# steineggerlab/folddisco

Hardware: AMD Instinct MI355X
Metric: structures/sec indexed (higher is better)
Workload: dtype f32+u32; 1 GPU; Swiss-Prot scale: 542000 synthetic AFDB-shaped structures (175035960 residues, 17705019118 postings, 26085150307 value bytes) index build, PDBTrRosetta default; 1 rank(s), contiguous id ranges, per rank 1 build call(s) of <= 542000 structures: one resident index, no merge; structures=542000, structures_per_gpu=542000, residues=175035960, postings=17705019118, parallelism=shard-by-structure x1, build_calls_per_rank=1

## Files before the change

### folddisco_amd/_lib.py

```python
from __future__ import annotations

import ctypes as C
import os

HERE = os.path.dirname(os.path.abspath(__file__))
LIB_PATH = os.path.join(HERE, "libfdgpu.so")

u8p = C.POINTER(C.c_uint8)
u32p = C.POINTER(C.c_uint32)
u64p = C.POINTER(C.c_uint64)
f32p = C.POINTER(C.c_float)
VP = C.c_void_p


class BatchDesc(C.Structure):
    _fields_ = [("n_struct", C.c_uint64), ("res_off", u64p), ("n_xyz", f32p), ("ca_xyz", f32p), ("cb_xyz", f32p),
                ("aa", u8p), ("cb_valid", u8p)]


class HashParams(C.Structure):
    _fields_ = [("nbin_dist", C.c_uint32), ("nbin_angle", C.c_uint32), ("dist_cutoff", C.c_float), ("hash_type", C.c_uint32),
                ("n_multiple_bins", C.c_uint32), ("multiple_bins", (C.c_uint32 * 2) * 8)]

    def __init__(self, nbin_dist=0, nbin_angle=0, dist_cutoff=20.0, hash_type=3, multiple_bins=None):
        super().__init__(int(nbin_dist), int(nbin_angle), float(dist_cutoff), int(hash_type))
        mb = list(multiple_bins or [])
        if len(mb) > 8:
            raise ValueError("at most 8 (dist, angle) bin pairs")
        self.n_multiple_bins = len(mb)
        for k, (d, a) in enumerate(mb):
            self.multiple_bins[k][0] = int(d)
            self.multiple_bins[k][1] = int(a)


def parse_multiple_bins(s):
    out = []
    for item in (s or "").split(","):
        parts = item.strip().split("-")
        if len(parts) == 2:
            try:
                out.append((int(parts[0]), int(parts[1])))
            except ValueError:
                pass
    return out


HASH_TYPE_NAMES = {0: "PDBMotif", 1: "PDBMotifSinCos", 2: "TrRosetta", 3: "PDBTrRosetta", 4: "PointPairFeature", 5: "TertiaryInteraction",
                   6: "Hybrid", 7: "FolddiscoAngle", 8: "FolddiscoDist"}
_HASH_TYPE_ALIASES = {"pyscomotif": 0, "orig_pdb": 0, "pdb": 1, "trrosetta": 2, "tr": 2, "pdbtr": 3, "default": 3, "folddisco": 3, "ppf": 4,
                      "tertiary": 5, "3di": 5, "hybrid": 6, "angle": 7, "folddisco_angle": 7, "distance": 8, "dist": 8, "folddisco_dist": 8}


def hash_type_index(name) -> int:
    if isinstance(name, int):
        return name
    s = str(name)
    if s.isdigit() and int(s) in HASH_TYPE_NAMES:
        return int(s)
    for k, v in HASH_TYPE_NAMES.items():
        if v == s:
            return k
    if s in _HASH_TYPE_ALIASES:
        return _HASH_TYPE_ALIASES[s]
    raise ValueError(f"unknown hash type {name!r}")


class CountRec(C.Structure):
    _fields_ = [("nid", C.c_uint32), ("total_match_count", C.c_uint32), ("node_count", C.c_uint32),
                ("edge_count", C.c_uint32), ("idf", C.c_float)]


class PairRec(C.Structure):
    _fields_ = [("cand", C.c_uint32), ("i", C.c_uint32), ("j", C.c_uint32), ("hash", C.c_uint32)]


class CandRec(C.Structure):
    _fields_ = [("cand", C.c_uint32), ("qi", C.c_uint32), ("i", C.c_uint32), ("j", C.c_uint32)]


class MatchQuery(C.Structure):
    _fields_ = [("hashes", u32p), ("n_hashes", C.c_uint64), ("aad_aa1", u8p), ("aad_aa2", u8p), ("aad_dist", f32p),
                ("aad_qi", u32p), ("n_aad", C.c_uint64), ("ca_distance_cutoff", C.c_float), ("use_aa_prefilter", C.c_int)]


class QueryMap(C.Structure):
    _fields_ = [("n", C.c_uint64), ("hash", u32p), ("qi", u32p), ("qj", u32p), ("is_primary", u8p), ("idf", f32p),
                ("n_indices", C.c_uint64), ("indices", u32p),
                ("n_aad", C.c_uint64), ("aad_aa1", u8p), ("aad_aa2", u8p), ("aad_dist", f32p), ("aad_qi", u32p), ("primary_hash", u32p),
                ("post_len", u64p), ("post_seg", u32p), ("post_index_uid", C.c_uint64), ("post_kidx", C.POINTER(C.c_longlong)),
                ("arena_bytes", C.c_uint64)]


class MatchRec(C.Structure):
    _fields_ = [("cand", C.c_uint32), ("same", C.c_uint32), ("idf", C.c_float), ("rmsd", C.c_float), ("rmsd_from_hash", C.c_float),
                ("rot", C.c_float * 9), ("tran", C.c_float * 3), ("metrics", C.c_float * 5),
                ("rot_from_hash", C.c_float * 9), ("tran_from_hash", C.c_float * 3), ("metrics_from_hash", C.c_float * 5)]


class FoldcompAtom(C.Structure):
    _fields_ = [("x", C.c_float), ("y", C.c_float), ("z", C.c_float), ("b", C.c_float), ("name", C.c_char * 4), ("res", C.c_char * 3),
                ("chain", C.c_uint8), ("rser", C.c_uint64)]


class VerifyReportC(C.Structure):
    _fields_ = [("ok", C.c_uint32), ("first_mask", C.c_uint32), ("n_bad", C.c_uint64), ("class_count", C.c_uint64 * 9), ("first_slot", C.c_uint64),
                ("first_offset", C.c_uint64), ("first_hash", C.c_uint32), ("list_stage", C.c_uint32), ("n_lists", C.c_uint64), ("n_postings", C.c_uint64),
                ("max_id", C.c_uint64), ("max_list_bytes", C.c_uint64)]


class Parsed(C.Structure):
    _fields_ = [("n_struct", C.c_uint64), ("n_res", C.c_uint64), ("res_off", u64p), ("n_xyz", f32p), ("ca_xyz", f32p), ("cb_xyz", f32p),
                ("aa", u8p), ("cb_valid", u8p), ("chain", u8p), ("resname_std", u8p), ("serial", u64p), ("bfac", f32p),
                ("resname", C.POINTER(C.c_char)), ("nres_raw", u64p), ("plddt", f32p), ("ok", u8p), ("first_chain", u8p)]


SYMBOLS = [
    ("fdgpu_create", C.c_int, [C.c_int, C.POINTER(VP)]),
    ("fdgpu_destroy", None, [VP]),
    ("fdgpu_set_stream", C.c_int, [VP, VP]),
    ("fdgpu_synchronize", C.c_int, [VP]),
    ("fdgpu_release_workspaces", C.c_int, [VP]),
    ("fdgpu_last_error", C.c_char_p, [VP]),
    ("fdgpu_free", None, [VP]),
    ("fdgpu_version", C.c_char_p, []),
    ("fdgpu_batch_upload", C.c_int, [VP, C.POINTER(BatchDesc), C.POINTER(VP)]),
    ("fdgpu_batch_wrap_device", C.c_int, [VP, C.POINTER(BatchDesc), C.c_uint64, C.POINTER(VP)]),
    ("fdgpu_batch_destroy", None, [VP]),
    ("fdgpu_batch_num_structures", C.c_uint64, [VP]),
    ("fdgpu_batch_num_residues", C.c_uint64, [VP]),
    ("fdgpu_batch_select", C.c_int, [VP, VP, u32p, C.c_uint64, C.POINTER(VP)]),
    ("fdgpu_batch_concat", C.c_int, [VP, C.POINTER(VP), C.c_uint64, C.POINTER(VP)]),
    ("fdgpu_batch_export", C.c_int, [VP, VP, C.POINTER(BatchDesc)]),
    ("fdgpu_hash_batch", C.c_int, [VP, VP, C.POINTER(HashParams), C.c_int, C.POINTER(u32p), C.POINTER(u64p)]),
    ("fdgpu_index_build", C.c_int, [VP, VP, C.POINTER(HashParams), C.c_uint64, C.POINTER(VP)]),
    ("fdgpu_index_export", C.c_int, [VP, VP, C.POINTER(u8p), u64p, C.POINTER(u32p), C.POINTER(u64p), u64p]),
    ("fdgpu_index_load", C.c_int, [VP, u32p, u64p, C.c_uint64, u8p, C.c_uint64, C.c_uint64, C.POINTER(VP)]),
    ("fdgpu_index_destroy", None, [VP]),
    ("fdgpu_index_num_hashes", C.c_uint64, [VP]),
    ("fdgpu_index_value_len", C.c_uint64, [VP]),
    ("fdgpu_index_num_postings", C.c_uint64, [VP]),
    ("fdgpu_index_num_structures", C.c_uint64, [VP]),
    ("fdgpu_index_save", C.c_int, [VP, VP, C.c_char_p]),
    ("fdgpu_posting_lengths", C.c_int, [VP, VP, u32p, C.c_uint64, u64p]),
    ("fdgpu_count_query", C.c_int, [VP, VP, u32p, u32p, u32p, f32p, C.c_uint64, f32p, C.POINTER(C.POINTER(CountRec)), u64p]),
    ("fdgpu_count_query_batch", C.c_int, [VP, VP, C.c_uint64, u64p, u32p, u32p, u32p, f32p, f32p, C.POINTER(C.POINTER(CountRec)), C.POINTER(u64p)]),
    ("fdgpu_spec_fallbacks", C.c_int, [VP, u64p]),
    ("fdgpu_parse_structures", C.c_int, [C.POINTER(C.c_char_p), C.c_uint64, C.c_uint32, C.c_uint64, C.POINTER(C.POINTER(Parsed))]),
    ("fdgpu_parsed_free", None, [C.POINTER(Parsed)]),
    ("fdgpu_foldcomp_decode", C.c_int, [C.c_char_p, C.c_uint64, C.POINTER(C.POINTER(FoldcompAtom)), u64p]),
    ("fdgpu_foldcomp_db_list", C.c_int, [C.c_char_p, C.POINTER(u64p), C.POINTER(C.c_void_p), u64p]),
    ("fdgpu_parse_foldcomp_db", C.c_int, [C.c_char_p, u64p, C.c_uint64, C.c_uint32, C.c_uint64, C.POINTER(C.POINTER(Parsed))]),
    ("fdgpu_get_entries", C.c_int, [VP, VP, u32p, C.c_uint64, C.POINTER(u32p), C.POINTER(u64p)]),
    ("fdgpu_count_query_batch_top", C.c_int, [VP, VP, C.c_uint64, u64p, u32p, u32p, u32p, f32p, f32p, C.c_uint32, C.POINTER(C.POINTER(CountRec)), C.POINTER(u64p)]),
    ("fdgpu_index_set_penalty", C.c_int, [VP, VP, f32p]),
    ("fdgpu_count_query_maps_top", C.c_int, [VP, VP, C.c_uint64, C.c_void_p, f32p, C.c_float, C.c_uint32, C.POINTER(C.POINTER(CountRec)), C.POINTER(u64p)]),
    ("fdgpu_match_pairs", C.c_int, [VP, VP, u8p, u32p, C.c_uint64, C.POINTER(MatchQuery), C.POINTER(HashParams),
                                    C.POINTER(C.POINTER(PairRec)), u64p, C.POINTER(C.POINTER(CandRec)), u64p]),
    ("fdgpu_kabsch_batch", C.c_int, [VP, f32p, f32p, u64p, C.c_uint64, f32p, f32p, f32p]),
    ("fdgpu_lms_qcp_batch", C.c_int, [VP, f32p, f32p, u64p, C.c_uint64, f32p, f32p, f32p, u32p, u32p]),
    ("fdgpu_last_timings", C.c_int, [VP, C.POINTER(C.c_char_p), f32p, u64p, C.c_int]),
    ("fdgpu_enable_timing", C.c_int, [VP, C.c_int]),
    ("fdgpu_pair_features", C.c_int, [VP, VP, C.c_uint64, u32p, u32p, C.c_uint64, C.POINTER(HashParams), f32p, u8p]),
    ("fdgpu_hash_features", C.c_int, [VP, f32p, C.c_uint64, C.POINTER(HashParams), u32p]),
    ("fdgpu_make_query_map_batch", C.c_int, [VP, VP, C.c_uint64, u32p, u64p, u32p, C.POINTER(u8p), u32p, f32p, C.c_uint64, f32p, C.c_uint64,
                                              C.POINTER(HashParams), VP, C.c_float, C.POINTER(C.POINTER(QueryMap))]),
    ("fdgpu_make_query_map", C.c_int, [VP, VP, u32p, C.c_uint64, C.POINTER(u8p), u32p, f32p, C.c_uint64, f32p, C.c_uint64,
                                       C.POINTER(HashParams), VP, C.c_float, C.POINTER(C.POINTER(QueryMap))]),
    ("fdgpu_query_map_free", None, [C.POINTER(QueryMap)]),
    ("fdgpu_retrieve_batch", C.c_int, [VP, VP, u8p, C.c_uint64, u32p, u64p, C.POINTER(C.POINTER(QueryMap)), VP, u32p, C.POINTER(HashParams),
                                        C.c_float, C.c_uint32, C.c_uint32, C.POINTER(C.POINTER(MatchRec)), C.POINTER(u64p), C.POINTER(C.POINTER(C.c_int32)),
                                        C.POINTER(u64p)]),
    ("fdgpu_query_batch", C.c_int, [VP, VP, VP, u8p, VP, C.c_uint64, u32p, u64p, u32p, C.POINTER(u8p), u32p, f32p, C.c_uint64, f32p, C.c_uint64,
                                    C.POINTER(HashParams), C.c_float, f32p, C.c_uint32, C.c_uint32, C.c_float, C.c_uint32, C.POINTER(C.POINTER(QueryMap)),
                                    C.POINTER(C.POINTER(CountRec)), C.POINTER(u64p), C.POINTER(C.POINTER(MatchRec)), C.POINTER(u64p),
                                    C.POINTER(C.POINTER(C.c_int32)), C.POINTER(u64p)]),
    ("fdgpu_query_batch_submit", C.c_int, [VP, VP, VP, u8p, VP, C.c_uint64, u32p, u64p, u32p, C.POINTER(u8p), u32p, f32p, C.c_uint64, f32p, C.c_uint64,
                                           C.POINTER(HashParams), C.c_float, f32p, C.c_uint32, C.c_uint32, C.c_float, C.c_uint32, C.POINTER(VP)]),
    ("fdgpu_query_batch_wait", C.c_int, [VP, VP, C.POINTER(C.POINTER(QueryMap)), C.POINTER(C.POINTER(CountRec)), C.POINTER(u64p), C.POINTER(C.POINTER(MatchRec)),
                                         C.POINTER(u64p), C.POINTER(C.POINTER(C.c_int32)), C.POINTER(u64p)]),
    ("fdgpu_query_lanes", C.c_int, [VP, C.c_uint32]),
    ("fdgpu_trim", None, []),
    ("fdgpu_reserve_staging", C.c_int, [VP]),
    ("fdgpu_write_lookup", C.c_int, [C.c_char_p, C.c_char_p, C.c_uint64, u64p, f32p, u64p]),
    ("fdgpu_format_f32_display", C.c_int, [f32p, C.c_uint64, C.c_char_p]),
    ("fdgpu_retrieve", C.c_int, [VP, VP, u8p, u32p, C.c_uint64, C.POINTER(QueryMap), VP, C.POINTER(HashParams), C.c_float, C.c_uint32, C.c_uint32,
                                 C.POINTER(C.POINTER(MatchRec)), u64p, C.POINTER(C.POINTER(C.c_int32))]),
    ("fdgpu_matches_free", None, [C.POINTER(MatchRec), C.POINTER(C.c_int32)]),
    ("fdgpu_merge_subindices", C.c_int, [C.c_uint64, C.POINTER(u8p), C.POINTER(u32p), C.POINTER(u64p), u64p, C.POINTER(u8p), u64p,
                                         C.POINTER(u32p), C.POINTER(u64p), u64p]),
    ("fdgpu_index_merge", C.c_int, [VP, C.POINTER(VP), C.c_uint64, C.POINTER(VP)]),
    ("fdgpu_index_remove", C.c_int, [VP, VP, u8p, C.c_uint64, C.POINTER(VP)]),
    ("fdgpu_index_split", C.c_int, [VP, VP, C.c_uint32, u64p, C.POINTER(VP)]),
    ("fdgpu_split_host", C.c_int, [u32p, u64p, C.c_uint64, u8p, C.c_uint64, C.c_uint64, C.c_uint32, u64p, C.c_uint32, C.POINTER(u8p), u64p,
                                   C.POINTER(u32p), C.POINTER(u64p), u64p]),
    ("fdgpu_index_rebase", C.c_int, [VP, VP, C.c_uint64, C.POINTER(VP)]),
    ("fdgpu_rebase_host", C.c_int, [u32p, u64p, C.c_uint64, u8p, C.c_uint64, C.c_uint64, C.c_uint64, C.c_uint64, C.c_uint32, C.POINTER(u8p), u64p,
                                    C.POINTER(u32p), C.POINTER(u64p)]),
    ("fdgpu_index_permute", C.c_int, [VP, VP, u32p, C.c_uint64, C.POINTER(VP)]),
    ("fdgpu_permute_host", C.c_int, [u32p, u64p, C.c_uint64, u8p, C.c_uint64, C.c_uint64, u32p, C.c_uint64, C.c_uint32, C.POINTER(u8p), u64p,
                                     C.POINTER(u32p), C.POINTER(u64p)]),
    ("fdgpu_index_rows", C.c_int, [VP, VP, C.c_uint64, C.c_uint64, C.POINTER(u32p), C.POINTER(u64p)]),
    ("fdgpu_rows_host", C.c_int, [u32p, u64p, C.c_uint64, u8p, C.c_uint64, C.c_uint64, C.c_uint64, C.c_uint64, C.c_uint64, C.c_uint32, C.POINTER(u32p),
                                  C.POINTER(u64p)]),
    ("fdgpu_index_signatures", C.c_int, [VP, VP, C.c_uint64, C.c_uint64, C.c_uint64, C.POINTER(VP)]),
    ("fdgpu_signatures_host", C.c_int, [u32p, u64p, C.c_uint64, u8p, C.c_uint64, C.c_uint64, C.c_uint64, C.c_uint64, C.c_uint64, C.c_uint32, C.POINTER(VP)]),
    ("fdgpu_signature_pairs", C.c_int, [VP, VP, C.c_uint64, VP, C.c_uint64, C.c_uint32, C.c_uint64, C.POINTER(VP), u64p]),
    ("fdgpu_signature_pairs_host", C.c_int, [VP, C.c_uint64, VP, C.c_uint64, C.c_uint32, C.c_uint64, C.c_uint32, C.POINTER(VP), u64p]),
    ("fdgpu_signature_neighbors", C.c_int, [VP, VP, C.c_uint64, VP, C.c_uint64, VP, C.c_uint32, C.c_uint32, C.POINTER(VP)]),
    ("fdgpu_signature_neighbors_host", C.c_int, [VP, C.c_uint64, VP, C.c_uint64, VP, C.c_uint32, C.c_uint32, C.c_uint32, C.POINTER(VP)]),
    ("fdgpu_signature_clusters", C.c_int, [VP, VP, C.c_uint64, VP, C.c_uint32, C.POINTER(VP)]),
    ("fdgpu_signature_clusters_host", C.c_int, [VP, C.c_uint64, VP, C.c_uint32, C.c_uint32, C.POINTER(VP)]),
    ("fdgpu_index_rowset", C.c_int, [VP, VP, u32p, C.c_uint64, C.c_uint64, C.c_uint64, C.POINTER(VP), u64p]),
    ("fdgpu_rowset_info", C.c_int, [VP, u64p, u64p]),
    ("fdgpu_rowset_lengths", C.c_int, [VP, C.POINTER(u32p)]),
    ("fdgpu_rowset_export", C.c_int, [VP, VP, C.POINTER(u32p), C.POINTER(u64p)]),
    ("fdgpu_rowset_intersect", C.c_int, [VP, VP, VP, u32p, u32p, C.c_uint64, C.POINTER(u32p)]),
    ("fdgpu_rowset_destroy", None, [VP]),
    ("fdgpu_rows_intersect_host", C.c_int, [u32p, u64p, C.c_uint64, u32p, u64p, C.c_uint64, u32p, u32p, C.c_uint64, C.c_uint32, C.POINTER(u32p)]),
    ("fdgpu_index_verify", C.c_int, [VP, VP, C.POINTER(VerifyReportC)]),
    ("fdgpu_verify_host", C.c_int, [u32p, u64p, C.c_uint64, u8p, C.c_uint64, C.c_uint64, C.c_uint64, C.c_uint32, C.POINTER(VerifyReportC)]),
    ("fdgpu_posting_bytes", C.c_int, [VP, VP, u32p, C.c_uint64, u64p]),
    ("fdgpu_index_set_first_id", C.c_int, [VP, C.c_uint64]),
    ("fdgpu_host_libm_matches", C.c_int, [VP]),
    ("fdgpu_metrics_batch", C.c_int, [VP, f32p, f32p, u64p, C.c_uint64, f32p, f32p, f32p]),
    ("fdgpu_hash_batch_rows", C.c_int, [VP, VP, C.POINTER(HashParams), C.POINTER(u32p), C.POINTER(u32p), C.POINTER(u64p)]),
    ("fdgpu_hypergeom_enrichment", C.c_int, [u64p, u64p, C.c_uint64, C.c_uint64, C.c_uint64, C.c_uint32, C.POINTER(C.c_double)]),
    ("fdgpu_comm_unique_id", C.c_int, [u8p]),
    ("fdgpu_comm_init", C.c_int, [VP, u8p, C.c_int, C.c_int, C.POINTER(VP)]),
    ("fdgpu_comm_destroy", None, [VP]),
    ("fdgpu_comm_rank", C.c_int, [VP]),
    ("fdgpu_comm_world", C.c_int, [VP]),
    ("fdgpu_allreduce_lengths", C.c_int, [VP, VP, u64p, C.c_uint64]),
    ("fdgpu_sharded_count_query", C.c_int, [VP, VP, VP, C.c_uint64, u64p, u32p, u32p, u32p, f32p, C.c_uint64, C.c_uint32,
                                            C.POINTER(C.POINTER(CountRec)), C.POINTER(u64p)]),
    ("fdgpu_comm_stats", C.c_int, [VP, u64p, u64p]),
    ("fdgpu_index_range_bounds", C.c_int, [VP, VP, C.c_uint32, u32p]),
    ("fdgpu_index_slice", C.c_int, [VP, VP, C.c_uint64, C.c_uint64, C.POINTER(VP)]),
    ("fdgpu_comm_single_index", C.c_int, [VP, VP, VP, C.POINTER(VP), u64p, u64p, u64p, u64p]),
    ("fdgpu_index_save_part", C.c_int, [VP, VP, C.c_char_p, C.c_uint64, C.c_uint64, C.c_uint64, C.c_uint64, C.c_int, C.c_int]),
    ("fdgpu_sharded_count_query_maps", C.c_int, [VP, VP, VP, C.c_uint64, C.c_void_p, f32p, C.c_uint64, C.c_uint32,
                                                 C.POINTER(C.POINTER(CountRec)), C.POINTER(u64p)]),
    ("fdgpu_sharded_retrieve", C.c_int, [VP, VP, VP, C.c_uint64, u8p, C.c_uint64, u32p, u64p, C.POINTER(C.POINTER(QueryMap)), VP, u32p,
                                         C.POINTER(HashParams), C.c_float, C.c_uint32, C.c_uint32, C.POINTER(C.POINTER(MatchRec)), C.POINTER(u64p),
                                         C.POINTER(C.POINTER(C.c_int32)), C.POINTER(u64p)]),
    ("fdgpu_query_maps_lengths", C.c_int, [VP, VP, C.c_uint64, C.c_void_p, u64p]),
    ("fdgpu_count_query_maps_top_global", C.c_int, [VP, VP, C.c_uint64, C.c_void_p, u64p, f32p, C.c_float, C.c_uint32,
                                                    C.POINTER(C.POINTER(CountRec)), C.POINTER(u64p)]),
    ("fdgpu_comm_message_bytes", C.c_uint64, [C.c_uint64, C.c_uint32]),
    ("fdgpu_debug_merge_gathered", C.c_int, [VP, C.c_uint32, C.c_uint64, C.c_uint32, u8p, C.POINTER(C.POINTER(CountRec)), C.POINTER(u64p)]),
    ("fdgpu_debug_libm", C.c_int, [VP, C.c_int, f32p, f32p, f32p, C.c_uint64]),
    ("fdgpu_debug_last_count_path", C.c_int, [VP, u32p]),
    ("fdgpu_debug_last_retrieve_path", C.c_int, [VP, u32p]),
    ("fdgpu_debug_last_query_map_path", C.c_int, [VP, u32p]),
    ("fdgpu_debug_qm_pairs", C.c_int, [C.c_uint64, u32p, u64p, u32p, u64p, C.POINTER(u32p), C.POINTER(u32p), u64p]),
    ("fdgpu_debug_qm_fields", C.c_int, [C.c_uint32, C.POINTER(C.c_int32)]),
    ("fdgpu_debug_qm_expand", C.c_int, [f32p, u8p, u32p, u32p, C.c_uint64, C.c_uint64, u32p, C.c_uint64, C.POINTER(u8p), u32p, C.c_uint32, f32p, C.c_uint64, f32p,
                                        C.c_uint64, C.POINTER(f32p), C.POINTER(u32p), u64p]),
    ("fdgpu_debug_qm_first_insertions", C.c_int, [u32p, C.c_uint64, C.c_uint32, C.c_uint64, C.c_uint64, C.POINTER(u32p), u64p]),
    ("fdgpu_debug_qm_arena", C.c_int, [C.c_uint64, C.c_uint64, C.c_uint64, C.c_uint32, u64p]),
    ("fdgpu_debug_qm_fill", C.c_int, [u32p, C.c_uint64, u32p, C.c_uint64, C.c_uint32, C.c_uint64, u32p, u32p, C.c_uint64, u32p, u32p, C.c_uint64, f32p, u32p, u64p, u32p,
                                      C.POINTER(C.c_longlong), C.c_uint64, u32p, C.c_uint64, u8p, u8p, f32p, u32p, C.c_uint64, C.c_uint32, C.POINTER(C.POINTER(QueryMap))]),
    ("fdgpu_debug_encode_stream", C.c_int, [VP, u32p, u32p, C.c_uint64, C.POINTER(VP)]),
    ("fdgpu_debug_encode_stream_b24", C.c_int, [VP, u32p, u32p, C.c_uint64, C.c_uint64, C.POINTER(VP)]),
    ("fdgpu_ingest_stats", None, [C.POINTER(C.c_double), C.c_int]),
    ("fdgpu_debug_gunzip", C.c_int, [u8p, C.c_uint64, C.POINTER(u8p), u64p]),
    ("fdgpu_debug_host_components", C.c_int, [u32p, u32p, C.c_uint64, C.c_uint32, C.POINTER(u32p), C.POINTER(u64p), u64p]),
    ("fdgpu_debug_hash_is_symmetric", C.c_int, [C.c_uint32, u32p, C.c_uint64, u8p]),
    ("fdgpu_debug_host_retrieve_slot", C.c_int, [u32p, u32p, u32p, C.c_uint64, u32p, u32p, u32p, C.c_uint64, C.c_uint32, C.POINTER(QueryMap), C.c_uint32, C.c_uint32,
                                                 C.c_uint32, C.c_uint32, u64p, C.POINTER(f32p), C.POINTER(u32p), C.POINTER(C.POINTER(C.c_int32))]),
    ("fdgpu_debug_match_tables", C.c_int, [C.c_uint64, C.POINTER(MatchQuery), u32p, u64p, u64p, C.c_uint64, C.c_uint32, C.c_uint32, C.c_uint32, C.POINTER(u32p), u64p, u64p,
                                           C.POINTER(C.c_char_p)]),
    ("fdgpu_debug_merge_retrieved", C.c_int, [VP, C.c_uint32, C.c_uint64, u64p, C.POINTER(C.POINTER(MatchRec)), C.POINTER(C.POINTER(C.c_int32)), u64p,
                                              C.POINTER(C.POINTER(MatchRec)), C.POINTER(u64p), C.POINTER(C.POINTER(C.c_int32)), C.POINTER(u64p)]),
]

_lib = None


def load() -> C.CDLL:
    global _lib
    if _lib is not None:
        return _lib
    if not os.path.exists(LIB_PATH):
        raise ImportError(
            f"{LIB_PATH} is missing: build it with `python -m folddisco_amd.build` (hipcc, gfx950). "
            "folddisco_amd has no CPU fallback.")
    try:
        import torch
    except Exception:
        pass
    L = C.CDLL(LIB_PATH)
    for name, res, args in SYMBOLS:
        fn = getattr(L, name)
        fn.restype = res
        fn.argtypes = args
    _lib = L
    return L


def owned_view(lib, ptr, nbytes, dtype):
    import weakref
    import numpy as _np
    addr = C.cast(ptr, C.c_void_p).value
    if not nbytes or not addr:
        if addr:
            lib.fdgpu_free(C.c_void_p(addr))
        return _np.zeros(0, _np.uint8).view(dtype)
    buf = (C.c_uint8 * nbytes).from_address(addr)
    weakref.finalize(buf, lib.fdgpu_free, C.c_void_p(addr))
    return _np.frombuffer(buf, dtype=_np.uint8).view(dtype)
```

### folddisco_amd/csrc/fd_api_build.hip

```cpp
#include <stdlib.h>
#include <algorithm>
#include <memory>
#include "fd_api_common.h"

struct ib_free { void operator()(void *p) const { free(p); } };
typedef std::unique_ptr<uint32_t, ib_free> ib_u32_ptr;
typedef std::unique_ptr<uint64_t, ib_free> ib_u64_ptr;

static int row_count_and_scan(fdgpu_ctx *c, const fdgpu_batch *b, const fd_hash_consts &C, float dist_cutoff, uint64_t *P, const char *stage = nullptr) {
    const uint64_t R = b->n_res;
    hipStream_t st = c->stream;
    HIPCHK(c, c->ws[WS_MISC0].ensure((R + 1) * 4));
    HIPCHK(c, c->ws[WS_MISC1].ensure((R + 2) * 8));
    HIPCHK(c, c->ws[WS_SCANTMP].ensure(fd_scan_tmp_elems(std::max<uint64_t>(b->n_struct, R)) * 8 + 64));
    HIPCHK(c, c->ws[WS_TOTAL].ensure(64));
    HIPCHK(c, hipMemsetAsync(c->ws[WS_MISC0].p, 0, (R + 1) * 4, st));
    {
        StageTimer t(stage ? c : nullptr, stage, R * 37);
        fd_launch_row_count(b->view(), C, c->ws[WS_MISC0].as<uint32_t>(), dist_cutoff, st);
        fd_exclusive_scan<uint32_t>(c->ws[WS_MISC0].as<uint32_t>(), R, c->ws[WS_MISC1].as<uint64_t>(), c->ws[WS_SCANTMP].as<uint64_t>(),
                                    c->ws[WS_TOTAL].as<uint64_t>(), st);
    }
    HIPCHK(c, hipGetLastError());
    return d2h_u64(c, c->ws[WS_TOTAL].as<uint64_t>(), P);
}

static int scan_counts(fdgpu_ctx *c, uint64_t n, uint64_t *P) {
    {
        StageTimer t(c, "segment_scan", n * 12);
        fd_exclusive_scan<uint32_t>(c->ws[WS_COUNTS].as<uint32_t>(), n, c->ws[WS_SEGOFF].as<uint64_t>(), c->ws[WS_SCANTMP].as<uint64_t>(),
                                    c->ws[WS_TOTAL].as<uint64_t>(), c->stream);
    }
    HIPCHK(c, hipGetLastError());
    return d2h_u64(c, c->ws[WS_TOTAL].as<uint64_t>(), P);
}
static int count_and_scan(fdgpu_ctx *c, const fdgpu_batch *b, const fd_hash_consts &C, uint64_t *P, bool unordered = false) {
    uint64_t S = b->n_struct;
    HIPCHK(c, c->ws[WS_COUNTS].ensure((S + 1) * 4));
    HIPCHK(c, c->ws[WS_CURSOR].ensure((S + 1) * 4));
    HIPCHK(c, c->ws[WS_SEGOFF].ensure((S + 2) * 8));
    HIPCHK(c, c->ws[WS_SCANTMP].ensure(fd_scan_tmp_elems(std::max<uint64_t>(S, b->n_res)) * 8 + 64));
    HIPCHK(c, c->ws[WS_TOTAL].ensure(64));
    HIPCHK(c, hipMemsetAsync(c->ws[WS_COUNTS].p, 0, (S + 1) * 4, c->stream));
    HIPCHK(c, hipMemsetAsync(c->ws[WS_CURSOR].p, 0, (S + 1) * 4, c->stream));
    {
        StageTimer t(c, "pair_count", b->n_res * 13);
        if (unordered) fd_launch_pair_count2(b->view(), C, c->ws[WS_COUNTS].as<uint32_t>(), c->stream);
        else fd_launch_pair_count(b->view(), C, c->ws[WS_COUNTS].as<uint32_t>(), c->stream);
    }
    return scan_counts(c, S, P);
}

struct ib_keys { uint32_t *ka, *kb; void *ia, *ib; };
static int reserve_keys(fdgpu_ctx *c, uint64_t P, uint64_t max_keys, const char *too_many, size_t id_bytes, ib_keys &K) {
    if (P >= max_keys) FAIL(c, FDGPU_ERANGE, too_many);
    size_t kb = std::max<uint64_t>(P, 1) * 4, ib = std::max<uint64_t>(P, 1) * id_bytes + 16;
    if (kb > c->ws[WS_KEYS_A].cap + ((size_t)1 << 30) || kb > c->ws[WS_KEYS_B].cap + ((size_t)1 << 30)) c->pool_drop();
    HIPCHK(c, c->ws[WS_KEYS_A].ensure(kb));
    HIPCHK(c, c->ws[WS_IDS_A].ensure(ib));
    HIPCHK(c, c->ws[WS_KEYS_B].ensure(kb));
    HIPCHK(c, c->ws[WS_IDS_B].ensure(ib));
    HIPCHK(c, c->ws[WS_GHIST].ensure((size_t)256 * std::max<uint32_t>(fd_rs_num_tiles(P), 1) * 4));
    HIPCHK(c, c->ws[WS_TOT].ensure((256 + (size_t)(fd_rs_num_tiles(P) / 128 + 2) * 256) * 8));
    K.ka = c->ws[WS_KEYS_A].as<uint32_t>(); K.kb = c->ws[WS_KEYS_B].as<uint32_t>();
    K.ia = c->ws[WS_IDS_A].p; K.ib = c->ws[WS_IDS_B].p;
    return FDGPU_OK;
}

extern "C" int fdgpu_hash_batch(fdgpu_ctx *c, const fdgpu_batch *b, const fd_hash_params *p, int sort_dedup, uint32_t **hashes,
                                uint64_t **hash_off) { FD_LOCK(c);
    if (!c || !b || !p || !hashes || !hash_off) return FDGPU_EINVAL;
    *hashes = nullptr; *hash_off = nullptr;
    if (p->n_multiple_bins) FAIL(c, FDGPU_EINVAL, "hash_batch: multiple_bins is honoured by the index build and the query calls only");
    if (!fd_hash_type_supported(p->hash_type)) FAIL(c, FDGPU_EINVAL, "hash_type: only the encodings over the (d_CA, d_CB, theta, tau1, tau2) descriptor are built (0, 1, 3, 7, 8)");
    reset_timings(c);
    fd_hash_consts C = make_consts(p);
    uint64_t S = b->n_struct, R = b->n_res;
    ib_u64_ptr h_off((uint64_t *)malloc((S + 1) * 8));
    if (!h_off) return FDGPU_ENOMEM;
    hipStream_t st = c->stream;
    int rc;
    if (!sort_dedup) {
        uint64_t P = 0;
        if ((rc = row_count_and_scan(c, b, C, p->dist_cutoff, &P))) return rc;
        HIPCHK(c, c->ws[WS_KEYS_A].ensure(std::max<uint64_t>(P, 1) * 4));
        fd_launch_row_emit(b->view(), C, c->ws[WS_MISC1].as<uint64_t>(), c->ws[WS_KEYS_A].as<uint32_t>(), p->dist_cutoff, nullptr, 0u, st);
        HIPCHK(c, hipGetLastError());
        ib_u32_ptr h((uint32_t *)malloc(std::max<uint64_t>(P, 1) * 4));
        std::vector<uint64_t> row_off(R + 1);
        if (!h) return FDGPU_ENOMEM;
        HIPCHK(c, hipMemcpyAsync(h.get(), c->ws[WS_KEYS_A].p, P * 4, hipMemcpyDeviceToHost, st));
        HIPCHK(c, hipMemcpyAsync(row_off.data(), c->ws[WS_MISC1].p, (R + 1) * 8, hipMemcpyDeviceToHost, st));
        HIPCHK(c, hipStreamSynchronize(st));
        for (uint64_t s = 0; s <= S; ++s) h_off.get()[s] = row_off[b->h_res_off[s]];
        *hashes = h.release(); *hash_off = h_off.release();
        return FDGPU_OK;
    }
    if (fd_own_descriptor(p->hash_type)) FAIL(c, FDGPU_EINVAL, "hash_batch: this encoding is served in the reference's raw order only (sort_dedup = 0)");
    uint64_t P = 0;
    if ((rc = count_and_scan(c, b, C, &P))) return rc;
    ib_keys K;
    if ((rc = reserve_keys(c, P, 0xffffffffull, "more than 2^32 residue pairs in one batch; split the batch", 4, K))) return rc;
    uint32_t *ka = K.ka, *ia = (uint32_t *)K.ia, *kb = K.kb, *ib = (uint32_t *)K.ib;
    fd_launch_pair_emit(b->view(), C, c->ws[WS_SEGOFF].as<uint64_t>(), c->ws[WS_CURSOR].as<uint32_t>(), ka, ia, 0u, st);
    int cur = sort_pairs(c, ka, ia, kb, ib, P, 32);
    uint32_t *k1 = cur ? kb : ka, *i1 = cur ? ib : ia, *k2 = cur ? ka : kb, *i2 = cur ? ia : ib;
    int id_bits = 1;
    while (id_bits < 32 && (1ull << id_bits) < std::max<uint64_t>(S, 2)) ++id_bits;
    int cur2 = sort_pairs(c, i1, k1, i2, k2, P, id_bits);
    uint32_t *ids_s = cur2 ? i2 : i1, *keys_s = cur2 ? k2 : k1, *spare = cur2 ? k1 : k2;
    HIPCHK(c, c->ws[WS_MISC0].ensure(std::max<uint64_t>(P, 1)));
    HIPCHK(c, c->ws[WS_MISC1].ensure((P + 2) * 8));
    HIPCHK(c, c->ws[WS_SCANTMP].ensure(fd_scan_tmp_elems(std::max<uint64_t>(P, S)) * 8 + 64));
    fd_launch_uniq_flags(keys_s, ids_s, P, c->ws[WS_MISC0].as<uint8_t>(), st);
    fd_exclusive_scan<uint8_t>(c->ws[WS_MISC0].as<uint8_t>(), P, c->ws[WS_MISC1].as<uint64_t>(), c->ws[WS_SCANTMP].as<uint64_t>(),
                               c->ws[WS_TOTAL].as<uint64_t>(), st);
    fd_launch_compact(keys_s, c->ws[WS_MISC0].as<uint8_t>(), c->ws[WS_MISC1].as<uint64_t>(), P, spare, st);
    HIPCHK(c, c->ws[WS_MISC2].ensure((S + 2) * 8));
    fd_launch_gather_u64(c->ws[WS_MISC1].as<uint64_t>(), c->ws[WS_SEGOFF].as<uint64_t>(), S + 1, c->ws[WS_MISC2].as<uint64_t>(), st);
    HIPCHK(c, hipGetLastError());
    uint64_t U = 0;
    if ((rc = d2h_u64(c, c->ws[WS_TOTAL].as<uint64_t>(), &U))) return rc;
    ib_u32_ptr h((uint32_t *)malloc(std::max<uint64_t>(U, 1) * 4));
    if (!h) return FDGPU_ENOMEM;
    HIPCHK(c, hipMemcpyAsync(h.get(), spare, U * 4, hipMemcpyDeviceToHost, st));
    HIPCHK(c, hipMemcpyAsync(h_off.get(), c->ws[WS_MISC2].p, (S + 1) * 8, hipMemcpyDeviceToHost, st));
    HIPCHK(c, hipStreamSynchronize(st));
    *hashes = h.release(); *hash_off = h_off.release();
    return FDGPU_OK;
}

extern "C" int fdgpu_hash_batch_rows(fdgpu_ctx *c, const fdgpu_batch *b, const fd_hash_params *p, uint32_t **hashes, uint32_t **partner, uint64_t **row_off) { FD_LOCK(c);
    if (!c || !b || !p || !hashes || !partner || !row_off) return FDGPU_EINVAL;
    *hashes = nullptr; *partner = nullptr; *row_off = nullptr;
    if (p->n_multiple_bins) FAIL(c, FDGPU_EINVAL, "hash_batch_rows: multiple_bins is honoured by the index build and the query calls only");
    if (!fd_hash_type_supported(p->hash_type)) FAIL(c, FDGPU_EINVAL, "hash_type: unknown encoding");
    reset_timings(c);
    const fd_hash_consts C = make_consts(p);
    const uint64_t R = b->n_res;
    hipStream_t st = c->stream;
    uint64_t P = 0;
    int rc = row_count_and_scan(c, b, C, p->dist_cutoff, &P);
    if (rc) return rc;
    HIPCHK(c, c->ws[WS_KEYS_A].ensure(std::max<uint64_t>(P, 1) * 4));
    HIPCHK(c, c->ws[WS_IDS_A].ensure(std::max<uint64_t>(P, 1) * 4));
    fd_launch_row_emit(b->view(), C, c->ws[WS_MISC1].as<uint64_t>(), c->ws[WS_KEYS_A].as<uint32_t>(), p->dist_cutoff, c->ws[WS_IDS_A].as<uint32_t>(), 0u, st, 1);
    HIPCHK(c, hipGetLastError());
    ib_u32_ptr h((uint32_t *)malloc(std::max<uint64_t>(P, 1) * 4)), pj((uint32_t *)malloc(std::max<uint64_t>(P, 1) * 4));
    ib_u64_ptr ro((uint64_t *)malloc((R + 1) * 8));
    if (!h || !pj || !ro) return FDGPU_ENOMEM;
    hipError_t e = hipMemcpyAsync(h.get(), c->ws[WS_KEYS_A].p, P * 4, hipMemcpyDeviceToHost, st);
    if (e == hipSuccess) e = hipMemcpyAsync(pj.get(), c->ws[WS_IDS_A].p, P * 4, hipMemcpyDeviceToHost, st);
    if (e == hipSuccess) e = hipMemcpyAsync(ro.get(), c->ws[WS_MISC1].p, (R + 1) * 8, hipMemcpyDeviceToHost, st);
    if (e == hipSuccess) e = hipStreamSynchronize(st);
    if (e != hipSuccess) { c->err = std::string("hash_batch_rows: ") + hipGetErrorString(e); return FDGPU_EHIP; }
    *hashes = h.release(); *partner = pj.release(); *row_off = ro.release();
    return FDGPU_OK;
}

#define FDGPU_RETRY_WIDE 1000
enum {
    IB_W_TOTALS = 0, IB_W_VALUE_BYTES = 0, IB_W_HASHES = 1, IB_W_POSTINGS = 2,
    IB_W_WIDE = 3,
    IB_W_SORT_OVERFLOW = 4,
    IB_W_READ = 5,
    IB_W_BUCKET_STARTS = 8,
};
static uint64_t *ib_word(fdgpu_ctx *c, int w) { return c->ws[WS_MISC3].as<uint64_t>() + w; }
static int ib_clear_words(fdgpu_ctx *c) {
    HIPCHK(c, c->ws[WS_MISC3].ensure(512));
    HIPCHK(c, hipMemsetAsync(c->ws[WS_MISC3].p, 0, IB_W_BUCKET_STARTS * 8, c->stream));
    return FDGPU_OK;
}
static int encode_sorted_stream(fdgpu_ctx *c, const uint32_t *ks, const void *is, int codec, uint64_t first_id, uint64_t P, uint64_t S, uint64_t seg_stride, fdgpu_index **out) {
    hipStream_t st = c->stream;
    const bool el6 = codec != 0;
    const uint32_t nt = std::max<uint32_t>(fd_enc_num_tiles(P), 1);
    for (int s : {WS_TILE_B, WS_TILE_H, WS_TILE_P}) HIPCHK(c, c->ws[s].ensure((size_t)(nt + 1) * 4));
    for (int s : {WS_TILE_BO, WS_TILE_HO, WS_TILE_PO}) HIPCHK(c, c->ws[s].ensure((size_t)(nt + 2) * 8));
    HIPCHK(c, c->ws[WS_SCANTMP].ensure(fd_scan_tmp_elems(std::max<uint64_t>(nt, S)) * 8 + 64));
    uint32_t *tile_bytes = c->ws[WS_TILE_B].as<uint32_t>(), *tile_hashes = c->ws[WS_TILE_H].as<uint32_t>(), *tile_posts = c->ws[WS_TILE_P].as<uint32_t>();
    uint64_t *bytes_off = c->ws[WS_TILE_BO].as<uint64_t>(), *hashes_off = c->ws[WS_TILE_HO].as<uint64_t>(), *posts_off = c->ws[WS_TILE_PO].as<uint64_t>();
    uint64_t *scan_tmp = c->ws[WS_SCANTMP].as<uint64_t>();
    const uint64_t *seg = c->ws[WS_SEGOFF].as<uint64_t>();
    uint64_t tot[IB_W_READ] = {0, 0, 0, 0, 0};
    const uint64_t nt_eff = P ? fd_enc_num_tiles(P) : 0;
    {
        StageTimer t(c, "encode_sizes", P * (el6 ? 6 : 8));
        for (uint32_t *tile : {tile_bytes, tile_hashes, tile_posts}) HIPCHK(c, hipMemsetAsync(tile, 0, (size_t)(nt + 1) * 4, st));
        fd_launch_enc_sizes(ks, is, codec, (uint32_t)first_id, P, tile_bytes, tile_hashes, tile_posts, seg, seg_stride, ib_word(c, IB_W_BUCKET_STARTS), st);
        fd_exclusive_scan<uint32_t>(tile_bytes, nt_eff, bytes_off, scan_tmp, ib_word(c, IB_W_VALUE_BYTES), st);
        fd_exclusive_scan<uint32_t>(tile_hashes, nt_eff, hashes_off, scan_tmp, ib_word(c, IB_W_HASHES), st);
        fd_exclusive_scan<uint32_t>(tile_posts, nt_eff, posts_off, scan_tmp, ib_word(c, IB_W_POSTINGS), st);
    }
    HIPCHK(c, hipGetLastError());
    HIPCHK(c, hipMemcpyAsync(tot, ib_word(c, IB_W_TOTALS), sizeof tot, hipMemcpyDeviceToHost, st));
    HIPCHK(c, hipStreamSynchronize(st));
    if (tot[IB_W_SORT_OVERFLOW]) FAIL(c, FDGPU_ERANGE, "index build: one (residue-pair bucket, key digit) group holds 2^32 keys or more; build the shard in several calls and merge");
    if (el6 && tot[IB_W_WIDE]) return FDGPU_RETRY_WIDE;
    fdgpu_index *ix = nullptr;
    const int rc = fd_index_new(c, true, tot[IB_W_HASHES], tot[IB_W_VALUE_BYTES], true, &ix);
    if (rc) return rc;
    ix->n_postings = tot[IB_W_POSTINGS]; ix->n_structures = S; ix->first_id = first_id;
    {
        StageTimer t(c, "encode_write", P * (el6 ? 6 : 8) + ix->value_len + ix->n_hashes * 12);
        fd_launch_enc_write(ks, is, codec, (uint32_t)first_id, P, bytes_off, hashes_off, ix->value, ix->hashes, ix->offsets, ix->last_ids, ib_word(c, IB_W_TOTALS), ix->n_hashes,
                            ib_word(c, IB_W_BUCKET_STARTS), st);
    }
    const hipError_t e = hipGetLastError();
    if (e != hipSuccess) { c->err = std::string("encode launch: ") + hipGetErrorString(e); fdgpu_index_destroy(ix); return FDGPU_EHIP; }
    *out = ix;
    return FDGPU_OK;
}

enum ib_kind { IB_OWN, IB_STRUCTURE_MAJOR, IB_MSD };
static const uint32_t IB_BUCKETS = 40;
struct ib_form {
    ib_kind kind; bool el6; int codec;
    uint32_t n_cfg; uint64_t seg_stride;
    uint64_t max_keys; const char *too_many;
};
static int ib_choose_form(fdgpu_ctx *c, const fdgpu_batch *b, const fd_hash_params *p, uint64_t first_id, bool force32, ib_form &F) {
    if (!fd_hash_type_supported(p->hash_type)) FAIL(c, FDGPU_EINVAL, "hash_type: only the encodings over the (d_CA, d_CB, theta, tau1, tau2) descriptor are built (0, 1, 3, 7, 8)");
    reset_timings(c);
    const uint64_t S = b->n_struct;
    if (first_id + S > 0xffffffffull) FAIL(c, FDGPU_ERANGE, "structure ids exceed 32 bits");
    if (!fd_multiple_bins_valid(p)) FAIL(c, FDGPU_EINVAL, "multiple_bins: at most 8 (dist, angle) bin pairs, no zero counts");
    F.n_cfg = fd_num_bin_configs(p);
    const bool own = fd_own_descriptor(p->hash_type);
    if (own && F.n_cfg > 1) FAIL(c, FDGPU_EINVAL, "multiple_bins is built for the encodings over the PDBTrRosetta descriptor only");
    const bool ids16 = !own && !force32 && S <= (1ull << 18);
    const bool msd_env = [] { const char *e = getenv("FDGPU_MSD"); return !(e && e[0] == '0'); }();
    const bool msd = msd_env && !own && !force32 && S <= (1ull << 24) && F.n_cfg == 1 && p->hash_type == FDGPU_HASH_PDBTR && S > 0;
    F.kind = own ? IB_OWN : msd ? IB_MSD : IB_STRUCTURE_MAJOR;
    F.el6 = ids16 || msd;
    F.codec = msd ? 2 : ids16 ? 1 : 0;
    F.seg_stride = msd ? b->n_work : 0;
    F.max_keys = msd ? 1ull << 35 : 0xffffffffull;
    F.too_many = msd ? "more than 2^35 residue pairs in one build call; split the shard" : "more than 2^32 residue pairs in one build call; split the shard";
    return FDGPU_OK;
}
static void ib_frames(fdgpu_ctx *c, const fdgpu_batch *b) {
    StageTimer t(c, "frames", b->n_res * (37 + sizeof(fd_frame)));
    fd_launch_frames(b->view(), b->n_res, c->ws[WS_FRAMES].p, c->stream);
}
static int ib_count_msd(fdgpu_ctx *c, const fdgpu_batch *b, const fd_hash_consts &C, fd_batch_view &V, uint64_t *P1) {
    hipStream_t st = c->stream;
    const uint64_t R1 = std::max<uint64_t>(b->n_res, 1), NS = (uint64_t)IB_BUCKETS * b->n_work;
    HIPCHK(c, c->ws[WS_CA_PERM].ensure(R1 * 12));
    HIPCHK(c, c->ws[WS_OK_PERM].ensure(R1));
    HIPCHK(c, c->ws[WS_AA_PERM].ensure(R1));
    HIPCHK(c, c->ws[WS_SRC_PERM].ensure(R1 * 4));
    V = b->view();
    {
        StageTimer t(c, "frames", b->n_res * (2 + 14 + 18));
        fd_launch_frames_perm(V, c->ws[WS_CA_PERM].as<float>(), c->ws[WS_OK_PERM].as<uint8_t>(), c->ws[WS_AA_PERM].as<uint8_t>(), c->ws[WS_SRC_PERM].as<uint32_t>(),
                              C.wide_flag, st);
    }
    V.ca_xyz = c->ws[WS_CA_PERM].as<float>(); V.hash_ok = c->ws[WS_OK_PERM].as<uint8_t>(); V.aa = c->ws[WS_AA_PERM].as<uint8_t>();
    V.n_xyz = nullptr; V.cb_xyz = nullptr;
    HIPCHK(c, c->ws[WS_COUNTS].ensure((NS + 1) * 4));
    HIPCHK(c, c->ws[WS_SEGOFF].ensure((NS + 2) * 8));
    HIPCHK(c, c->ws[WS_SCANTMP].ensure(fd_scan_tmp_elems(std::max<uint64_t>(NS, b->n_res)) * 8 + 64));
    HIPCHK(c, c->ws[WS_TOTAL].ensure(64));
    {
        StageTimer t(c, "pair_count", b->n_res * (14 + 28 + sizeof(fd_frame)) + NS * 4);
        fd_launch_pair_count_msd(V, C, b->n_xyz, b->cb_xyz, c->ws[WS_SRC_PERM].as<uint32_t>(), c->ws[WS_FRAMES].p, c->ws[WS_COUNTS].as<uint32_t>(), st);
    }
    int rc = scan_counts(c, NS, P1);
    uint64_t odd = 0;
    if (!rc) rc = d2h_u64(c, (const uint64_t *)C.wide_flag, &odd);
    return !rc && odd ? FDGPU_RETRY_WIDE : rc;
}
static int ib_reserve_keys(fdgpu_ctx *c, const ib_form &F, uint64_t P, ib_keys &K) { return reserve_keys(c, P, F.max_keys, F.too_many, F.el6 ? 2 : 4, K); }
static void ib_emit_rows(fdgpu_ctx *c, const fdgpu_batch *b, const fd_hash_params *p, const fd_hash_consts &C, const ib_keys &K, uint64_t P, uint64_t first_id) {
    StageTimer t(c, "pair_emit", b->n_res * 37 + P * 8);
    fd_launch_row_emit(b->view(), C, c->ws[WS_MISC1].as<uint64_t>(), K.ka, p->dist_cutoff, (uint32_t *)K.ia, (uint32_t)first_id, c->stream);
}
static void ib_emit_msd(fdgpu_ctx *c, const fdgpu_batch *b, const fd_batch_view &V, const fd_hash_consts &C, const ib_keys &K, uint64_t P) {
    StageTimer t(c, "pair_emit", b->n_res * 37 + P * 6);
    fd_launch_pair_emit_msd(V, c->ws[WS_FRAMES].p, C, c->ws[WS_SEGOFF].as<uint64_t>(), K.ka, (uint16_t *)K.ia, c->stream);
}
static int ib_emit_structure_major(fdgpu_ctx *c, const fdgpu_batch *b, const fd_hash_params *p, const ib_form &F, const fd_hash_consts &C, const ib_keys &K, uint64_t P,
                                   uint64_t first_id) {
    StageTimer t(c, "pair_emit", b->n_res * 37 + P * (F.el6 ? 6 : 8));
    for (uint32_t k = 0; k < F.n_cfg; ++k) {
        fd_hash_consts Ck = fd_make_consts_cfg(p, k);
        Ck.spec_miss = C.spec_miss; Ck.wide_flag = C.wide_flag; Ck.seg_mul = F.n_cfg; Ck.seg_cfg = k;
        if (k) HIPCHK(c, hipMemsetAsync(c->ws[WS_CURSOR].p, 0, (b->n_struct + 1) * 4, c->stream));
        fd_launch_pair_emit2(b->view(), c->ws[WS_FRAMES].p, Ck, c->ws[WS_SEGOFF].as<uint64_t>(), c->ws[WS_CURSOR].as<uint32_t>(), K.ka, K.ia, F.el6, (uint32_t)first_id,
                             c->stream);
    }
    return FDGPU_OK;
}
static int ib_sort(fdgpu_ctx *c, const ib_form &F, const ib_keys &K, uint64_t P) {
    if (F.el6) return fd_radix_sort_pairs16(K.ka, (uint16_t *)K.ia, K.kb, (uint16_t *)K.ib, P, 32, c->ws[WS_GHIST].as<uint32_t>(), c->ws[WS_TOT].as<uint64_t>(), c->stream, c);
    return sort_pairs(c, K.ka, (uint32_t *)K.ia, K.kb, (uint32_t *)K.ib, P, 32);
}
static int ib_sort_msd(fdgpu_ctx *c, const fdgpu_batch *b, const ib_keys &K, uint64_t P, int *cur) {
    static const fd_rs_digit digits[3] = {{0, 24}, {1, 0}, {1, 8}};
    HIPCHK(c, c->ws[WS_GHIST].ensure((size_t)256 * fd_rs_seg_num_tiles(P, IB_BUCKETS) * 4));
    HIPCHK(c, c->ws[WS_TOT].ensure(fd_rs_seg_tot_words(P, IB_BUCKETS) * 8));
    HIPCHK(c, c->ws[WS_SEG_TAB].ensure(fd_rs_seg_tab_bytes(P, IB_BUCKETS)));
    *cur = fd_radix_sort_pairs16_seg(K.ka, (uint16_t *)K.ia, K.kb, (uint16_t *)K.ib, P, c->ws[WS_SEGOFF].as<uint64_t>(), b->n_work, IB_BUCKETS, digits, 3,
                                     c->ws[WS_GHIST].as<uint32_t>(), c->ws[WS_TOT].as<uint64_t>(), c->ws[WS_SEG_TAB].p, c->stream, c,
                                     (unsigned long long *)ib_word(c, IB_W_SORT_OVERFLOW));
    return FDGPU_OK;
}

static int index_build_impl(fdgpu_ctx *c, const fdgpu_batch *b, const fd_hash_params *p, uint64_t first_id, fdgpu_index **out, bool force32) {
    if (!c || !b || !p || !out) return FDGPU_EINVAL;
    *out = nullptr;
    ib_form F;
    int rc = ib_choose_form(c, b, p, first_id, force32, F);
    if (rc) return rc;
    HIPCHK(c, c->ws[WS_FRAMES].ensure(std::max<uint64_t>(b->n_res, 1) * sizeof(fd_frame)));
    if ((rc = ib_clear_words(c))) return rc;
    fd_hash_consts C = fd_make_consts_cfg(p, 0);
    C.spec_miss = c->spec_miss;
    C.wide_flag = (unsigned long long *)ib_word(c, IB_W_WIDE);
    uint64_t P = 0;
    ib_keys K;
    fd_batch_view V;
    int cur = 0;
    switch (F.kind) {
    case IB_OWN:
        ib_frames(c, b);
        if ((rc = row_count_and_scan(c, b, C, p->dist_cutoff, &P, "pair_count")) || (rc = ib_reserve_keys(c, F, P, K))) return rc;
        ib_emit_rows(c, b, p, C, K, P, first_id);
        cur = ib_sort(c, F, K, P);
        break;
    case IB_STRUCTURE_MAJOR:
        ib_frames(c, b);
        if ((rc = count_and_scan(c, b, C, &P, true))) return rc;
        P *= F.n_cfg;
        if ((rc = ib_reserve_keys(c, F, P, K)) || (rc = ib_emit_structure_major(c, b, p, F, C, K, P, first_id))) return rc;
        cur = ib_sort(c, F, K, P);
        break;
    case IB_MSD:
        if ((rc = ib_count_msd(c, b, C, V, &P)) || (rc = ib_reserve_keys(c, F, P, K))) return rc;
        ib_emit_msd(c, b, V, C, K, P);
        if ((rc = ib_sort_msd(c, b, K, P, &cur))) return rc;
        break;
    }
    return encode_sorted_stream(c, cur ? K.kb : K.ka, cur ? K.ib : K.ia, F.codec, first_id, P, b->n_struct, F.seg_stride, out);
}

extern "C" int fdgpu_index_build(fdgpu_ctx *c, const fdgpu_batch *b, const fd_hash_params *p, uint64_t first_id, fdgpu_index **out) { FD_LOCK(c);
    const char *e32 = getenv("FDGPU_IDS32");
    int rc = index_build_impl(c, b, p, first_id, out, e32 && e32[0] == '1');
    if (rc == FDGPU_RETRY_WIDE) rc = index_build_impl(c, b, p, first_id, out, true);
    return rc;
}

static int debug_upload_stream(fdgpu_ctx *c, const uint32_t *keys, const void *ids, size_t id_bytes, uint64_t n) {
    reset_timings(c);
    const int rc = ib_clear_words(c);
    if (rc) return rc;
    HIPCHK(c, c->ws[WS_KEYS_A].ensure(std::max<uint64_t>(n, 1) * 4));
    HIPCHK(c, c->ws[WS_IDS_A].ensure(std::max<uint64_t>(n, 1) * id_bytes));
    if (n) {
        HIPCHK(c, hipMemcpyAsync(c->ws[WS_KEYS_A].p, keys, n * 4, hipMemcpyHostToDevice, c->stream));
        HIPCHK(c, hipMemcpyAsync(c->ws[WS_IDS_A].p, ids, n * id_bytes, hipMemcpyHostToDevice, c->stream));
    }
    return FDGPU_OK;
}
extern "C" int fdgpu_debug_encode_stream(fdgpu_ctx *c, const uint32_t *hashes, const uint32_t *ids, uint64_t n, fdgpu_index **out) { FD_LOCK(c);
    if (!c || !out || (n && (!hashes || !ids))) return FDGPU_EINVAL;
    *out = nullptr;
    if (n >= 0xffffffffull) FAIL(c, FDGPU_ERANGE, "encode_stream: 2^32 elements or more");
    uint64_t S = 0;
    for (uint64_t p = 0; p < n; ++p) {
        if (p && (hashes[p - 1] > hashes[p] || (hashes[p - 1] == hashes[p] && ids[p - 1] > ids[p]))) FAIL(c, FDGPU_EINVAL, "encode_stream: the stream is not sorted by (hash, id)");
        S = std::max<uint64_t>(S, (uint64_t)ids[p] + 1);
    }
    const int rc = debug_upload_stream(c, hashes, ids, 4, n);
    if (rc) return rc;
    return encode_sorted_stream(c, c->ws[WS_KEYS_A].as<uint32_t>(), c->ws[WS_IDS_A].p, 0, 0, n, S, 0, out);
}
extern "C" int fdgpu_debug_encode_stream_b24(fdgpu_ctx *c, const uint32_t *hashes, const uint32_t *local_ids, uint64_t n, uint64_t first_id, fdgpu_index **out) { FD_LOCK(c);
    if (!out || (n && (!hashes || !local_ids))) return FDGPU_EINVAL;
    *out = nullptr;
    const uint32_t NB = IB_BUCKETS;
    uint64_t S = 0;
    const char *why = n >= 0xffffffffull ? "encode_stream_b24: 2^32 elements or more" : nullptr;
    for (uint64_t p = 0; p < n && !why; ++p) {
        const uint32_t h = hashes[p], id = local_ids[p];
        if (h >= (1u << 30) || (h >> 24) >= NB) why = "encode_stream_b24: a hash of 2^30 or more, or in a bucket (hash >> 24) of 40 or more";
        else if (id >= (1u << 24)) why = "encode_stream_b24: a local id of 2^24 or more";
        else if (p && (hashes[p - 1] > h || (hashes[p - 1] == h && local_ids[p - 1] > id))) why = "encode_stream_b24: the stream is not sorted by (hash, id)";
        S = std::max<uint64_t>(S, (uint64_t)id + 1);
    }
    if (!why && first_id + S > 0xffffffffull) why = "encode_stream_b24: structure ids exceed 32 bits";
    if (why) { if (c) c->err = why; return FDGPU_EINVAL; }
    if (!c) return FDGPU_OK;
    std::vector<uint32_t> k32(std::max<uint64_t>(n, 1));
    std::vector<uint16_t> v16(std::max<uint64_t>(n, 1));
    std::vector<uint64_t> seg(NB + 2, 0);
    for (uint64_t p = 0; p < n; ++p) {
        const uint32_t h = hashes[p];
        k32[p] = (h & 0xffu) << 24 | local_ids[p];
        v16[p] = (uint16_t)(h >> 8);
        ++seg[(h >> 24) + 1];
    }
    for (uint32_t b = 0; b < NB; ++b) seg[b + 1] += seg[b];
    const int rc = debug_upload_stream(c, k32.data(), v16.data(), 2, n);
    if (rc) return rc;
    HIPCHK(c, c->ws[WS_SEGOFF].ensure((NB + 2) * 8));
    HIPCHK(c, hipMemcpyAsync(c->ws[WS_SEGOFF].p, seg.data(), (NB + 1) * 8, hipMemcpyHostToDevice, c->stream));
    HIPCHK(c, hipStreamSynchronize(c->stream));
    return encode_sorted_stream(c, c->ws[WS_KEYS_A].as<uint32_t>(), c->ws[WS_IDS_A].p, 2, first_id, n, S, 1, out);
}
```

### folddisco_amd/csrc/fd_device.h

```cpp
#pragma once
#include <hip/hip_runtime.h>
#include <stdint.h>
#include "fd_geom.h"

#define FD_WAVE 64

struct fd_batch_view {
    const float *n_xyz, *ca_xyz, *cb_xyz;
    const uint8_t *aa;
    const uint8_t *hash_ok;
    const uint32_t *res_off;
    const uint32_t *wi_struct;
    const uint32_t *wi_i0;
    uint32_t n_struct;
    uint32_t n_work;
};

struct fd_hash_consts {
    uint32_t seg_mul, seg_cfg;
    fd_quant q;
    float d2_max;
    int use_tab;
    unsigned long long *spec_miss;
    unsigned long long *wide_flag;
};

__device__ __forceinline__ fd_v3 fd_load3(const float *p, uint32_t r) {
    const float *q = p + 3ull * r;
    return {q[0], q[1], q[2]};
}

__device__ __forceinline__ uint32_t fd_xcd_remap(uint32_t b, uint32_t n) {
    uint32_t per = (n + 7u) / 8u;
    uint32_t w = (b & 7u) * per + (b >> 3);
    return w;
}

__device__ __forceinline__ void fd_wave_lds_fence() {
    __builtin_amdgcn_fence(__ATOMIC_ACQ_REL, "wavefront");
    __builtin_amdgcn_wave_barrier();
}

__device__ __forceinline__ uint32_t fd_lane() { return __builtin_amdgcn_mbcnt_hi(~0u, __builtin_amdgcn_mbcnt_lo(~0u, 0u)); }
__device__ __forceinline__ uint32_t fd_mbcnt(uint64_t m) {
    return __builtin_amdgcn_mbcnt_hi((uint32_t)(m >> 32), __builtin_amdgcn_mbcnt_lo((uint32_t)m, 0u));
}
```

### folddisco_amd/csrc/fdgpu_api.hip

```cpp
#include <math.h>
#include <stdio.h>
#include <stdlib.h>
#include <string.h>
#include <algorithm>
#include <chrono>
#include <sys/mman.h>
#include <atomic>
#include <thread>
#include "fdgpu_internal.h"
#include <fcntl.h>
#include <unistd.h>
#include <cerrno>
#include <cstring>

#include "fd_api_common.h"
#include "fd_postings.h"

__global__ void k_uniq_flags(const uint32_t *__restrict__ keys, const uint32_t *__restrict__ ids, uint64_t n, uint8_t *__restrict__ flags) {
    uint64_t p = (uint64_t)blockIdx.x * blockDim.x + threadIdx.x;
    if (p < n) flags[p] = (p == 0 || keys[p] != keys[p - 1] || ids[p] != ids[p - 1]) ? 1 : 0;
}
__global__ void k_compact(const uint32_t *__restrict__ keys, const uint8_t *__restrict__ flags, const uint64_t *__restrict__ pos, uint64_t n,
                          uint32_t *__restrict__ out) {
    uint64_t p = (uint64_t)blockIdx.x * blockDim.x + threadIdx.x;
    if (p < n && flags[p]) out[pos[p]] = keys[p];
}
__global__ void k_gather_u64(const uint64_t *__restrict__ src, const uint64_t *__restrict__ idx, uint64_t n, uint64_t *__restrict__ dst) {
    uint64_t p = (uint64_t)blockIdx.x * blockDim.x + threadIdx.x;
    if (p < n) dst[p] = src[idx[p]];
}
void fd_launch_uniq_flags(const uint32_t *keys, const uint32_t *ids, uint64_t n, uint8_t *flags, hipStream_t st) {
    if (n) hipLaunchKernelGGL(k_uniq_flags, dim3((unsigned)((n + 255) / 256)), dim3(256), 0, st, keys, ids, n, flags);
}
void fd_launch_compact(const uint32_t *keys, const uint8_t *flags, const uint64_t *pos, uint64_t n, uint32_t *out, hipStream_t st) {
    if (n) hipLaunchKernelGGL(k_compact, dim3((unsigned)((n + 255) / 256)), dim3(256), 0, st, keys, flags, pos, n, out);
}
void fd_launch_gather_u64(const uint64_t *src, const uint64_t *idx, uint64_t n, uint64_t *dst, hipStream_t st) {
    if (n) hipLaunchKernelGGL(k_gather_u64, dim3((unsigned)((n + 255) / 256)), dim3(256), 0, st, src, idx, n, dst);
}

__global__ __launch_bounds__(256) void k_count_postings(const uint8_t *__restrict__ value, uint64_t n, unsigned long long *__restrict__ out) {
    unsigned long long acc = 0;
    for (uint64_t p = ((uint64_t)blockIdx.x * 256 + threadIdx.x) * 16; p < n; p += (uint64_t)gridDim.x * 256 * 16)
        for (uint64_t k = p; k < n && k < p + 16; ++k) acc += !(value[k] & 0x80u);
    for (int o = 32; o > 0; o >>= 1) acc += __shfl_down(acc, o);
    if ((threadIdx.x & 63) == 0 && acc) atomicAdd(out, acc);
}
hipError_t fd_count_postings(fdgpu_ctx *c, const uint8_t *value, uint64_t n, uint64_t *out) {
    unsigned long long np = 0;
    hipError_t e = hipSuccess;
    if (n) {
        e = c->ws[WS_TOTAL].ensure(64);
        if (e == hipSuccess) e = hipMemsetAsync(c->ws[WS_TOTAL].p, 0, 8, c->stream);
        if (e == hipSuccess) { hipLaunchKernelGGL(k_count_postings, dim3(2048), dim3(256), 0, c->stream, value, n, c->ws[WS_TOTAL].as<unsigned long long>()); e = hipGetLastError(); }
        if (e == hipSuccess) e = hipMemcpyAsync(&np, c->ws[WS_TOTAL].p, 8, hipMemcpyDeviceToHost, c->stream);
    }
    if (e == hipSuccess) e = hipStreamSynchronize(c->stream);
    *out = np;
    return e;
}

extern "C" const char *fdgpu_version(void) { return "folddisco_amd 0.1 (gfx950)"; }

static int fd_selfcheck(fdgpu_ctx *c) {
    const char *e = getenv("FDGPU_SELFCHECK");
    if (e && e[0] == '0') return FDGPU_OK;
    fd_hash_params p;
    memset(&p, 0, sizeof p);
    p.dist_cutoff = 20.0f; p.hash_type = FDGPU_HASH_PDBTR;
    const fd_hash_consts C = make_consts(&p);
    uint32_t *d = nullptr, h[24];
    HIPCHK(c, hipMalloc((void **)&d, sizeof h));
    fd_launch_selfcheck(C.q, d, c->stream);
    hipError_t he = hipGetLastError();
    if (he == hipSuccess) he = hipMemcpyAsync(h, d, sizeof h, hipMemcpyDeviceToHost, c->stream);
    if (he == hipSuccess) he = hipStreamSynchronize(c->stream);
    (void)hipFree(d);
    if (he != hipSuccess) { c->err = std::string("self-check launch: ") + hipGetErrorString(he); return FDGPU_EHIP; }
    static const uint32_t want[6] = {109329223u, 116878724u, 271858548u, 284511716u, 506948936u, 512052558u};
    for (int k = 0; k < 24; ++k)
        if (h[k] != want[k % 6]) {
            char b[256];
            snprintf(b, sizeof b, "self-check failed: 4CHA triad hash %d (%s evaluation) is %u, the reference's literal is %u (controller/graph.rs:71-79)", k % 6,
                     k < 6 ? "generic" : k < 12 ? "table" : k < 18 ? "speculative" : "speculative + squared-distance table", h[k], want[k % 6]);
            c->err = b;
            return FDGPU_EHIP;
        }
    int ok = 1;
    auto same = [](float a, float b) { uint32_t x, y; memcpy(&x, &a, 4); memcpy(&y, &b, 4); return x == y || (a != a && b != b); };
    for (int k = 1; k < FD_THETA_NSEG && ok; ++k) {
        float t;
        memcpy(&t, &fd_theta_thr_bits[k], 4);
        for (int u = -64; u <= 64 && ok; ++u) {
            uint32_t bits = fd_theta_thr_bits[k] + (uint32_t)u;
            float x;
            memcpy(&x, &bits, 4);
            if (!(x >= -1.0f && x <= 1.0f)) continue;
            const float a = acosf(x);
            ok = same(fd_acosf(x), a) && same(fd_sinf(a), sinf(a)) && same(fd_cosf(a), cosf(a));
        }
    }
    for (int m = 0; m < 4 && ok; ++m)
        for (int k = 1; k < FD_TOR_MAXSEG && ok; ++k)
            for (int u = -64; u <= 64 && ok; ++u) {
                uint32_t bits = fd_tor_thr_bits[m][k] + (uint32_t)u;
                float r;
                memcpy(&r, &bits, 4);
                if (!(r == r) || r > 3.0e38f) continue;
                const float y = (m & 1) ? -r : r, x = (m & 2) ? -1.0f : 1.0f;
                const float a = -atan2f(y, x);
                ok = same(-fd_atan2f(y, x), a) && same(fd_sinf(a), sinf(a)) && same(fd_cosf(a), cosf(a));
            }
    c->host_libm_matches = ok;
    if (!ok) {
        static bool warned = false;
        if (!warned) {
            warned = true;
            fprintf(stderr, "[fdgpu] warning: this host's libm (sinf/cosf/acosf/atan2f) differs from the glibc 2.35 generation the device arithmetic restates; a "
                            "reference build on this host can hash residue pairs at bin edges differently (rerun tools/gen_bin_tables.c + tools/check_libm.c)\n");
        }
    }
    return FDGPU_OK;
}
extern "C" int fdgpu_host_libm_matches(const fdgpu_ctx *c) { return c ? c->host_libm_matches : -1; }

static std::atomic<int> fd_live_contexts{0};
extern "C" void fdgpu_trim(void);
extern "C" int fdgpu_create(int device, fdgpu_ctx **out) {
    if (!out) return FDGPU_EINVAL;
    *out = nullptr;
    fdgpu_ctx *c = new (std::nothrow) fdgpu_ctx();
    if (!c) return FDGPU_ENOMEM;
    c->device = device;
    int n = 0;
    hipError_t e = hipGetDeviceCount(&n);
    if (e != hipSuccess || n <= 0 || device < 0 || device >= n) {
        c->err = e != hipSuccess ? std::string("hipGetDeviceCount: ") + hipGetErrorString(e) : "no such HIP device";
        *out = c;
        return FDGPU_EHIP;
    }
    if ((e = hipSetDevice(device)) != hipSuccess || (e = hipStreamCreate(&c->stream)) != hipSuccess) {
        c->err = std::string("hipSetDevice/hipStreamCreate: ") + hipGetErrorString(e);
        *out = c;
        return FDGPU_EHIP;
    }
    c->own_stream = true;
    c->counted = true;
    fd_live_contexts.fetch_add(1);
    if (hipMalloc((void **)&c->spec_miss, 8) == hipSuccess) (void)hipMemset(c->spec_miss, 0, 8);
    else c->spec_miss = nullptr;
    *out = c;
    return fd_selfcheck(c);
}
extern "C" int fdgpu_spec_fallbacks(fdgpu_ctx *c, uint64_t *out) { FD_LOCK(c);
    if (!c || !out) return FDGPU_EINVAL;
    *out = 0;
    if (!c->spec_miss) return FDGPU_OK;
    HIPCHK(c, hipStreamSynchronize(c->stream));
    HIPCHK(c, hipMemcpy(out, c->spec_miss, 8, hipMemcpyDeviceToHost));
    HIPCHK(c, hipMemset(c->spec_miss, 0, 8));
    return FDGPU_OK;
}
extern "C" void fdgpu_destroy(fdgpu_ctx *c) {
    if (!c) return;
    fd_lanes_destroy(c);
    if (c->spec_miss) (void)hipFree(c->spec_miss);
    for (auto &b : c->ws) b.release();
    for (auto &b : c->pool) (void)hipFree(b.p);
    for (auto e : c->event_pool) (void)hipEventDestroy(e);
    for (int k = 0; k < 16; ++k) { if (c->pin[k]) (void)hipHostFree(c->pin[k]); if (c->pin_ev[k]) (void)hipEventDestroy(c->pin_ev[k]); }
    for (int k = 0; k < FD_HP_SLOTS; ++k) if (c->hbuf[k]) (void)hipHostFree(c->hbuf[k]);
    if (c->side_stream) (void)hipStreamDestroy(c->side_stream);
    if (c->own_stream && c->stream) (void)hipStreamDestroy(c->stream);
    const bool last = c->counted && fd_live_contexts.fetch_sub(1) == 1;
    delete c;
    if (last) fdgpu_trim();
}
extern "C" int fdgpu_release_workspaces(fdgpu_ctx *c) { FD_LOCK(c);
    if (!c) return FDGPU_EINVAL;
    HIPCHK(c, hipStreamSynchronize(c->stream));
    for (auto &b : c->ws) b.release();
    c->pool_drop();
    (void)hipGetLastError();
    return FDGPU_OK;
}
extern "C" int fdgpu_set_stream(fdgpu_ctx *c, void *s) { FD_LOCK(c);
    if (!c) return FDGPU_EINVAL;
    if (c->own_stream && c->stream) { (void)hipStreamSynchronize(c->stream); (void)hipStreamDestroy(c->stream); c->own_stream = false; }
    if (s) { c->stream = (hipStream_t)s; return FDGPU_OK; }
    HIPCHK(c, hipStreamCreate(&c->stream));
    c->own_stream = true;
    return FDGPU_OK;
}
extern "C" int fdgpu_synchronize(fdgpu_ctx *c) { FD_LOCK(c);
    if (!c) return FDGPU_EINVAL;
    HIPCHK(c, hipStreamSynchronize(c->stream));
    return FDGPU_OK;
}
extern "C" const char *fdgpu_last_error(const fdgpu_ctx *c) { return c ? c->err.c_str() : "null context"; }
#include <mutex>
#include <unordered_map>
namespace {
struct fd_out_blk { size_t cap; bool pinned; };
struct fd_out_pool {
    std::mutex mu;
    std::unordered_map<void *, fd_out_blk> live;
    std::vector<std::pair<fd_out_blk, void *>> idle;
    size_t idle_bytes = 0;
};
fd_out_pool &out_pool() { static fd_out_pool *p = new fd_out_pool(); return *p; }
const size_t FD_OUT_POOL_MIN = (size_t)64 << 10;
size_t fd_out_pool_cap() {
    static const size_t cap = [] { const char *e = getenv("FDGPU_OUT_POOL_MB"); return e ? (size_t)std::max(0L, atol(e)) << 20 : (size_t)256 << 20; }();
    return cap;
}
}
extern "C" void fdgpu_trim(void) {
    fd_out_pool &P = out_pool();
    std::vector<std::pair<fd_out_blk, void *>> drop;
    {
        std::lock_guard<std::mutex> lk(P.mu);
        drop.swap(P.idle);
        P.idle_bytes = 0;
    }
    for (auto &b : drop) { if (b.first.pinned) (void)hipHostFree(b.second); else free(b.second); }
}
void *fd_out_alloc(size_t bytes, bool pinned) {
    if (bytes < FD_OUT_POOL_MIN) return malloc(bytes ? bytes : 1);
    fd_out_pool &P = out_pool();
    {
        std::lock_guard<std::mutex> lk(P.mu);
        size_t best = (size_t)-1;
        for (size_t k = 0; k < P.idle.size(); ++k)
            if (P.idle[k].first.pinned == pinned && P.idle[k].first.cap >= bytes && P.idle[k].first.cap <= 2 * bytes + (1u << 20) &&
                (best == (size_t)-1 || P.idle[k].first.cap < P.idle[best].first.cap)) best = k;
        if (best != (size_t)-1) {
            void *p = P.idle[best].second;
            const fd_out_blk b = P.idle[best].first;
            P.idle.erase(P.idle.begin() + best);
            P.idle_bytes -= b.cap;
            P.live[p] = b;
            return p;
        }
    }
    const size_t cap = bytes + bytes / 4;
    void *p = nullptr;
    bool got_pinned = false;
    if (pinned && hipHostMalloc(&p, cap, hipHostMallocPortable) == hipSuccess && p) got_pinned = true;
    else { (void)hipGetLastError(); p = malloc(cap); }
    if (!p) return nullptr;
    std::lock_guard<std::mutex> lk(P.mu);
    P.live[p] = fd_out_blk{cap, got_pinned};
    return p;
}
extern "C" void fdgpu_free(void *p) {
    if (!p) return;
    fd_out_pool &P = out_pool();
    fd_out_blk b;
    {
        std::lock_guard<std::mutex> lk(P.mu);
        auto it = P.live.find(p);
        if (it == P.live.end()) { free(p); return; }
        b = it->second;
        P.live.erase(it);
        if (P.idle_bytes + b.cap <= fd_out_pool_cap()) { P.idle.emplace_back(b, p); P.idle_bytes += b.cap; return; }
    }
    if (b.pinned) (void)hipHostFree(p); else free(p);
}
extern "C" int fdgpu_enable_timing(fdgpu_ctx *c, int on) { FD_LOCK(c); if (!c) return FDGPU_EINVAL; c->timing = on != 0; return FDGPU_OK; }
extern "C" int fdgpu_last_timings(const fdgpu_ctx *c, const char **names, float *ms, uint64_t *bytes, int cap) { FD_LOCK(c);
    if (!c) return FDGPU_EINVAL;
    int n = 0;
    for (auto &t : c->timings) {
        if (n >= cap) break;
        float m = 0.f;
        if (hipEventElapsedTime(&m, t.ev0, t.ev1) != hipSuccess) m = -1.f;
        if (names) names[n] = t.name;
        if (ms) ms[n] = m;
        if (bytes) bytes[n] = t.bytes;
        ++n;
    }
    return n;
}

int fd_build_work_items(fdgpu_ctx *c, fdgpu_batch *b, bool with_hash_ok) {
    std::vector<uint32_t> ws, wi;
    std::vector<uint32_t> ro(b->n_struct + 1);
    for (uint64_t s = 0; s <= b->n_struct; ++s) ro[s] = (uint32_t)b->h_res_off[s];
    for (uint64_t s = 0; s < b->n_struct; ++s) {
        uint64_t R = b->h_res_off[s + 1] - b->h_res_off[s];
        if (R > 65535) FAIL(c, FDGPU_ERANGE, "structure with more than 65535 residues (reference max_residue, controller/mod.rs:40)");
        for (uint64_t t = 0; t < R; t += FD_WAVE) { ws.push_back((uint32_t)s); wi.push_back((uint32_t)(b->h_res_off[s] + t)); }
    }
    if (ws.size() > 0xfffffff0ull) FAIL(c, FDGPU_ERANGE, "too many tiles in one batch");
    b->n_work = (uint32_t)ws.size();
    HIPCHK(c, hipMalloc((void **)&b->res_off, ro.size() * 4));
    HIPCHK(c, hipMalloc((void **)&b->wi_struct, std::max<size_t>(ws.size(), 1) * 4));
    HIPCHK(c, hipMalloc((void **)&b->wi_i0, std::max<size_t>(wi.size(), 1) * 4));
    HIPCHK(c, hipMemcpyAsync(b->res_off, ro.data(), ro.size() * 4, hipMemcpyHostToDevice, c->stream));
    if (!ws.empty()) {
        HIPCHK(c, hipMemcpyAsync(b->wi_struct, ws.data(), ws.size() * 4, hipMemcpyHostToDevice, c->stream));
        HIPCHK(c, hipMemcpyAsync(b->wi_i0, wi.data(), wi.size() * 4, hipMemcpyHostToDevice, c->stream));
    }
    HIPCHK(c, hipMalloc((void **)&b->hash_ok, std::max<uint64_t>(b->n_res, 1)));
    if (with_hash_ok) fd_launch_hash_ok(b->aa, b->cb_valid, b->hash_ok, b->n_res, c->stream);
    HIPCHK(c, hipGetLastError());
    HIPCHK(c, hipStreamSynchronize(c->stream));
    return FDGPU_OK;
}

extern "C" int fdgpu_batch_upload(fdgpu_ctx *c, const fd_batch_desc *h, fdgpu_batch **out) { FD_LOCK(c);
    if (!c || !h || !out || !h->res_off || (h->n_struct && (!h->n_xyz || !h->ca_xyz || !h->cb_xyz || !h->aa))) return FDGPU_EINVAL;
    *out = nullptr;
    if (h->n_struct >= 0xffffffffull) FAIL(c, FDGPU_ERANGE, "too many structures in one batch");
    uint64_t R = h->res_off[h->n_struct];
    if (R >= 0xffffffffull) FAIL(c, FDGPU_ERANGE, "more than 2^32 residues in one batch");
    fdgpu_batch *b = new (std::nothrow) fdgpu_batch();
    if (!b) return FDGPU_ENOMEM;
    b->ctx = c; b->owns = true; b->n_struct = h->n_struct; b->n_res = R;
    b->h_res_off.assign(h->res_off, h->res_off + h->n_struct + 1);
    size_t rb = std::max<uint64_t>(R, 1);
    int rc = FDGPU_OK;
    auto up = [&](void **d, const void *src, size_t bytes) -> int {
        HIPCHK(c, hipMalloc(d, std::max<size_t>(bytes, 4)));
        if (bytes) HIPCHK(c, hipMemcpyAsync(*d, src, bytes, hipMemcpyHostToDevice, c->stream));
        return FDGPU_OK;
    };
    if ((rc = up((void **)&b->n_xyz, h->n_xyz, R * 12)) || (rc = up((void **)&b->ca_xyz, h->ca_xyz, R * 12)) ||
        (rc = up((void **)&b->cb_xyz, h->cb_xyz, R * 12)) || (rc = up((void **)&b->aa, h->aa, R))) { fdgpu_batch_destroy(b); return rc; }
    if (h->cb_valid && (rc = up((void **)&b->cb_valid, h->cb_valid, R))) { fdgpu_batch_destroy(b); return rc; }
    (void)rb;
    if ((rc = fd_build_work_items(c, b))) { fdgpu_batch_destroy(b); return rc; }
    *out = b;
    return FDGPU_OK;
}

extern "C" int fdgpu_batch_wrap_device(fdgpu_ctx *c, const fd_batch_desc *d, uint64_t total_residues, fdgpu_batch **out) { FD_LOCK(c);
    if (!c || !d || !out || !d->res_off) return FDGPU_EINVAL;
    *out = nullptr;
    fdgpu_batch *b = new (std::nothrow) fdgpu_batch();
    if (!b) return FDGPU_ENOMEM;
    b->ctx = c; b->owns = false; b->n_struct = d->n_struct; b->n_res = total_residues;
    b->n_xyz = (float *)d->n_xyz; b->ca_xyz = (float *)d->ca_xyz; b->cb_xyz = (float *)d->cb_xyz;
    b->aa = (uint8_t *)d->aa; b->cb_valid = (uint8_t *)d->cb_valid;
    b->h_res_off.resize(d->n_struct + 1);
    hipError_t e = hipMemcpy(b->h_res_off.data(), d->res_off, (d->n_struct + 1) * 8, hipMemcpyDeviceToHost);
    if (e != hipSuccess) { c->err = std::string("wrap_device: ") + hipGetErrorString(e); delete b; return FDGPU_EHIP; }
    if (b->h_res_off[d->n_struct] != total_residues) { c->err = "wrap_device: res_off[n] != total_residues"; delete b; return FDGPU_EINVAL; }
    int rc = fd_build_work_items(c, b);
    if (rc) { fdgpu_batch_destroy(b); return rc; }
    *out = b;
    return FDGPU_OK;
}

extern "C" void fdgpu_batch_destroy(fdgpu_batch *b) {
    if (!b) return;
    if (b->owns) { (void)hipFree(b->n_xyz); (void)hipFree(b->ca_xyz); (void)hipFree(b->cb_xyz); (void)hipFree(b->aa); (void)hipFree(b->cb_valid); }
    (void)hipFree(b->hash_ok); (void)hipFree(b->res_off); (void)hipFree(b->wi_struct); (void)hipFree(b->wi_i0);
    delete b;
}
extern "C" uint64_t fdgpu_batch_num_structures(const fdgpu_batch *b) { return b ? b->n_struct : 0; }
extern "C" uint64_t fdgpu_batch_num_residues(const fdgpu_batch *b) { return b ? b->n_res : 0; }

bool fd_hash_type_supported(uint32_t t) { return t <= 8u; }
fd_hash_consts make_consts_bins(const fd_hash_params *p, uint32_t nbd_req, uint32_t nba_req, bool either_zero_defaults) {
    const uint32_t type = p->hash_type;
    uint32_t cap_d = 16, def_d = 16, cap_a = 4, def_a = 4;
    if (type == FD_HASH_PDBMOTIF) { cap_d = 32; def_d = 18; cap_a = 32; def_a = 9; }
    else if (type == FD_HASH_PDBMOTIF_SINCOS) { cap_d = 16; def_d = 8; cap_a = 16; def_a = 3; }
    else if (type == FD_HASH_FD_ANGLE) { cap_d = 8; def_d = 8; cap_a = 32; def_a = 32; }
    else if (type == FD_HASH_FD_DIST) { cap_d = 32; def_d = 32; cap_a = 16; def_a = 16; }
    else if (type == FD_HASH_TRROSETTA) { cap_d = 8; def_d = 8; cap_a = 4; def_a = 3; }
    else if (type == FD_HASH_PPF || type == FD_HASH_TERTIARY) { cap_d = 16; def_d = 8; cap_a = 8; def_a = 3; }
    else if (type == FD_HASH_HYBRID) { cap_d = 16; def_d = 16; cap_a = 4; def_a = 4; }
    const bool dflt = either_zero_defaults && (nbd_req == 0 || nba_req == 0);
    float nd = (dflt || nbd_req == 0) ? (float)def_d : (nbd_req > cap_d ? (float)cap_d : (float)nbd_req);
    float na = (dflt || nba_req == 0) ? (float)def_a : (nba_req > cap_a ? (float)cap_a : (float)nba_req);
    fd_hash_consts C;
    C.seg_mul = 1; C.seg_cfg = 0;
    const float PI_F = 3.14159274f;
    float a_min = -1.0f, a_max = 1.0f;
    if (type == FD_HASH_PDBMOTIF) { a_min = 0.0f; a_max = 180.0f; }
    else if (type == FD_HASH_FD_ANGLE || type == FD_HASH_FD_DIST) { a_min = -PI_F; a_max = PI_F; }
    volatile float cont_d = (20.0f - 2.0f) / (nd - 1.0f);
    volatile float cont_a = (a_max - a_min) / (na - 1.0f);
    float n180 = type == FD_HASH_FD_ANGLE ? fminf(na, 32.0f) : fminf(na, 8.0f);
    volatile float cont_t = (PI_F - 0.0f) / (n180 - 1.0f);
    C.q.dist_disc = 1.0f / cont_d;
    C.q.ang_disc = 1.0f / cont_a;
    C.q.ang2_disc = 1.0f / cont_t;
    C.q.type = type;
    float cut = p->dist_cutoff;
    float d2 = cut * cut;
    while (sqrtf(d2) > cut) d2 = nextafterf(d2, 0.0f);
    while (sqrtf(nextafterf(d2, INFINITY)) <= cut) d2 = nextafterf(d2, INFINITY);
    C.d2_max = d2;
    const char *ex = getenv("FDGPU_EXACT");
    const bool exact_only = ex && ex[0] == '1';
    C.use_tab = (type == FD_HASH_PDBTR && na == 4.0f) ? (exact_only ? 1 : 2) : 0;
    const char *dt = getenv("FDGPU_DTAB");
    if (C.use_tab == 2 && nd == 16.0f && !(dt && dt[0] == '0')) C.use_tab = 3;
    C.spec_miss = nullptr;
    return C;
}

fd_hash_consts make_consts(const fd_hash_params *p) { return make_consts_bins(p, p->nbin_dist, p->nbin_angle, true); }
fd_hash_consts fd_make_consts(const fd_hash_params *p) { return make_consts(p); }
uint32_t fd_num_bin_configs(const fd_hash_params *p) { return p->n_multiple_bins ? p->n_multiple_bins : 1u; }
fd_hash_consts fd_make_consts_cfg(const fd_hash_params *p, uint32_t k) {
    if (!p->n_multiple_bins) return make_consts(p);
    return make_consts_bins(p, p->multiple_bins[k][0], p->multiple_bins[k][1], false);
}
bool fd_multiple_bins_valid(const fd_hash_params *p) {
    if (p->n_multiple_bins > FDGPU_MAX_MULTIPLE_BINS) return false;
    for (uint32_t k = 0; k < p->n_multiple_bins; ++k)
        if (p->multiple_bins[k][0] == 0 || p->multiple_bins[k][1] == 0) return false;
    return true;
}

int d2h_u64(fdgpu_ctx *c, const uint64_t *dev, uint64_t *host) {
    HIPCHK(c, hipMemcpyAsync(host, dev, 8, hipMemcpyDeviceToHost, c->stream));
    HIPCHK(c, hipStreamSynchronize(c->stream));
    return FDGPU_OK;
}

int sort_pairs(fdgpu_ctx *c, uint32_t *ka, uint32_t *va, uint32_t *kb, uint32_t *vb, uint64_t n, int key_bits) {
    return fd_radix_sort_pairs(ka, va, kb, vb, n, key_bits, c->ws[WS_GHIST].as<uint32_t>(), c->ws[WS_TOT].as<uint64_t>(), c->stream, c);
}

hipError_t fd_index_block(fdgpu_ctx *pool, size_t bytes, void **p, size_t *cap) {
    if (!pool) return hipMalloc(p, bytes);
    hipError_t e;
    *p = pool->pool_alloc(bytes, &e);
    *cap = pool->last_cap;
    return e;
}
int fd_index_new(fdgpu_ctx *c, bool pooled, uint64_t H, uint64_t value_len, bool with_last, fdgpu_index **out) {
    *out = nullptr;
    fdgpu_index *ix = new (std::nothrow) fdgpu_index();
    if (!ix) FAIL(c, FDGPU_ENOMEM, "index alloc: out of memory");
    ix->ctx = pooled ? c : nullptr; ix->n_hashes = H;
    hipError_t e = hipSuccess;
    if (value_len != FD_VALUE_LATER) { ix->value_len = value_len; e = fd_index_block(ix->ctx, value_len + FD_VALUE_SLACK, (void **)&ix->value, &ix->cap_value); }
    if (e == hipSuccess) e = fd_index_block(ix->ctx, std::max<uint64_t>(H, 1) * 4, (void **)&ix->hashes, &ix->cap_hashes);
    if (e == hipSuccess) e = fd_index_block(ix->ctx, (H + 1) * 8, (void **)&ix->offsets, &ix->cap_offsets);
    if (e == hipSuccess && with_last) e = fd_index_block(ix->ctx, std::max<uint64_t>(H, 1) * 4, (void **)&ix->last_ids, &ix->cap_last);
    if (e != hipSuccess) { c->err = std::string("index alloc: ") + hipGetErrorString(e); fdgpu_index_destroy(ix); return FDGPU_EHIP; }
    *out = ix;
    return FDGPU_OK;
}
__global__ void k_ix_order(const uint8_t *__restrict__ sel, const uint8_t *__restrict__ is_long, const uint64_t *__restrict__ sel_pre,
                           const uint64_t *__restrict__ long_pre, uint64_t H, uint32_t *__restrict__ order, uint32_t *__restrict__ place) {
    const uint64_t t = (uint64_t)blockIdx.x * blockDim.x + threadIdx.x;
    if (t >= H || (sel && !sel[t])) return;
    const uint64_t n_long = long_pre[H];
    const uint64_t g = is_long[t] ? long_pre[t] : n_long + ((sel ? sel_pre[t] : t) - long_pre[t]);
    order[g] = (uint32_t)t;
    if (place) place[t] = (uint32_t)g;
}
void fd_order_long_first(const uint8_t *sel, const uint8_t *is_long, uint64_t H, uint64_t *sel_pre, uint64_t *long_pre, uint64_t *scan_tmp,
                         uint64_t *total_dev, uint32_t *order, uint32_t *place, hipStream_t st) {
    if (sel) fd_exclusive_scan<uint8_t>(sel, H, sel_pre, scan_tmp, total_dev, st);
    fd_exclusive_scan<uint8_t>(is_long, H, long_pre, scan_tmp, total_dev, st);
    hipLaunchKernelGGL(k_ix_order, dim3(fd_grid(H, 256)), dim3(256), 0, st, sel, is_long, sel_pre, long_pre, H, order, place);
}
extern "C" void fdgpu_index_destroy(fdgpu_index *ix) {
    if (!ix) return;
    FD_LOCK(ix->ctx);
    if (ix->ctx) {
        ix->ctx->pool_free(ix->hashes, ix->cap_hashes); ix->ctx->pool_free(ix->offsets, ix->cap_offsets); ix->ctx->pool_free(ix->value, ix->cap_value);
    } else { (void)hipFree(ix->hashes); (void)hipFree(ix->offsets); (void)hipFree(ix->value); }
    if (ix->ctx && ix->cap_last) ix->ctx->pool_free(ix->last_ids, ix->cap_last);
    else (void)hipFree(ix->last_ids);
    if (ix->penalty) (void)hipFree(ix->penalty);
    if (ix->lens) (void)hipFree(ix->lens);
    if (ix->ck_meta) (void)hipFree(ix->ck_meta);
    if (ix->ck_ent) (void)hipFree(ix->ck_ent);
    delete ix;
}
extern "C" int fdgpu_index_set_first_id(fdgpu_index *ix, uint64_t first_id) { if (!ix || first_id + ix->n_structures > 0xffffffffull) return FDGPU_EINVAL; ix->first_id = first_id; return FDGPU_OK; }
extern "C" uint64_t fdgpu_index_num_hashes(const fdgpu_index *ix) { return ix ? ix->n_hashes : 0; }
extern "C" uint64_t fdgpu_index_value_len(const fdgpu_index *ix) { return ix ? ix->value_len : 0; }
extern "C" uint64_t fdgpu_index_num_postings(const fdgpu_index *ix) { return ix ? ix->n_postings : 0; }
extern "C" uint64_t fdgpu_index_num_structures(const fdgpu_index *ix) { return ix ? ix->n_structures : 0; }

#define FD_PIN_SLOTS 16
#define FD_PIN_BYTES ((size_t)16 << 20)
hipError_t fd_d2h_big(fdgpu_ctx *c, void *dst, const void *src, size_t bytes) {
    if (bytes < 4 * FD_PIN_BYTES) return bytes ? hipMemcpyAsync(dst, src, bytes, hipMemcpyDeviceToHost, c->stream) : hipSuccess;
    for (int k = 0; k < FD_PIN_SLOTS; ++k) {
        hipError_t e = hipSuccess;
        if (!c->pin[k]) e = hipHostMalloc(&c->pin[k], FD_PIN_BYTES, hipHostMallocDefault);
        if (e == hipSuccess && !c->pin_ev[k]) e = hipEventCreateWithFlags(&c->pin_ev[k], hipEventDisableTiming);
        if (e != hipSuccess) return hipMemcpyAsync(dst, src, bytes, hipMemcpyDeviceToHost, c->stream);
    }
    {
        const uintptr_t a = ((uintptr_t)dst + 0x1fffff) & ~(uintptr_t)0x1fffff, b = ((uintptr_t)dst + bytes) & ~(uintptr_t)0x1fffff;
        if (b > a) (void)madvise((void *)a, b - a, MADV_HUGEPAGE);
    }
    const size_t n_chunks = (bytes + FD_PIN_BYTES - 1) / FD_PIN_BYTES;
    std::vector<std::thread> drain(FD_PIN_SLOTS);
    hipError_t err = hipSuccess;
    const int dev = c->device;
    for (size_t i = 0; i < n_chunks && err == hipSuccess; ++i) {
        const int k = (int)(i % FD_PIN_SLOTS);
        if (drain[k].joinable()) drain[k].join();
        const size_t off = i * FD_PIN_BYTES, n = std::min(FD_PIN_BYTES, bytes - off);
        err = hipMemcpyAsync(c->pin[k], (const uint8_t *)src + off, n, hipMemcpyDeviceToHost, c->stream);
        if (err == hipSuccess) err = hipEventRecord(c->pin_ev[k], c->stream);
        if (err != hipSuccess) break;
        void *pin = c->pin[k];
        hipEvent_t ev = c->pin_ev[k];
        drain[k] = std::thread([=]() { (void)hipSetDevice(dev); (void)hipEventSynchronize(ev); memcpy((uint8_t *)dst + off, pin, n); });
    }
    for (auto &t : drain) if (t.joinable()) t.join();
    return err;
}

extern "C" int fdgpu_index_export(fdgpu_ctx *c, const fdgpu_index *ix, uint8_t **value, uint64_t *value_len, uint32_t **hashes,
                                  uint64_t **offsets, uint64_t *n_hashes) { FD_LOCK(c);
    if (!c || !ix || !value || !value_len || !hashes || !offsets || !n_hashes) return FDGPU_EINVAL;
    uint8_t *v = (uint8_t *)malloc(std::max<uint64_t>(ix->value_len, 1));
    uint32_t *h = (uint32_t *)malloc(std::max<uint64_t>(ix->n_hashes, 1) * 4);
    uint64_t *o = (uint64_t *)malloc((ix->n_hashes + 1) * 8);
    if (!v || !h || !o) { free(v); free(h); free(o); return FDGPU_ENOMEM; }
    hipError_t e = fd_d2h_big(c, v, ix->value, ix->value_len);
    if (e == hipSuccess) e = fd_d2h_big(c, h, ix->hashes, ix->n_hashes * 4);
    if (e == hipSuccess) e = fd_d2h_big(c, o, ix->offsets, (ix->n_hashes + 1) * 8);
    if (e == hipSuccess) e = hipStreamSynchronize(c->stream);
    if (e != hipSuccess) { free(v); free(h); free(o); c->err = std::string("index export: ") + hipGetErrorString(e); return FDGPU_EHIP; }
    *value = v; *value_len = ix->value_len; *hashes = h; *offsets = o; *n_hashes = ix->n_hashes;
    return FDGPU_OK;
}

extern "C" int fdgpu_index_load(fdgpu_ctx *c, const uint32_t *hashes, const uint64_t *offsets, uint64_t H, const uint8_t *value,
                                uint64_t vlen, uint64_t n_structures, fdgpu_index **out) { FD_LOCK(c);
    if (!c || !out || (H && (!hashes || !offsets)) || (vlen && !value)) return FDGPU_EINVAL;
    *out = nullptr;
    fdgpu_index *ix = nullptr;
    int rc = fd_index_new(c, false, H, vlen, false, &ix);
    if (rc) return rc;
    ix->n_structures = n_structures;
    hipError_t e = hipSuccess;
    uint64_t zero = 0;
    if ((vlen && (e = hipMemcpyAsync(ix->value, value, vlen, hipMemcpyHostToDevice, c->stream)) != hipSuccess) ||
        (H && (e = hipMemcpyAsync(ix->hashes, hashes, H * 4, hipMemcpyHostToDevice, c->stream)) != hipSuccess) ||
        (e = hipMemcpyAsync(ix->offsets, H ? offsets : &zero, (H + 1) * 8, hipMemcpyHostToDevice, c->stream)) != hipSuccess ||
        (e = hipStreamSynchronize(c->stream)) != hipSuccess) {
        c->err = std::string("index load: ") + hipGetErrorString(e);
        fdgpu_index_destroy(ix);
        return FDGPU_EHIP;
    }
    if ((e = fd_count_postings(c, ix->value, vlen, &ix->n_postings)) != hipSuccess) {
        (void)hipGetLastError();
        c->err = std::string("index load: counting the postings: ") + hipGetErrorString(e);
        fdgpu_index_destroy(ix);
        return FDGPU_EHIP;
    }
    *out = ix;
    return FDGPU_OK;
}

hipError_t fd_d2h_to_file(fdgpu_ctx *c, int fd, uint64_t file_off, const void *src, size_t bytes, std::atomic<int> *io_err) {
    if (!bytes) return hipSuccess;
    for (int k = 0; k < FD_PIN_SLOTS; ++k) {
        hipError_t e = hipSuccess;
        if (!c->pin[k]) e = hipHostMalloc(&c->pin[k], FD_PIN_BYTES, hipHostMallocDefault);
        if (e == hipSuccess && !c->pin_ev[k]) e = hipEventCreateWithFlags(&c->pin_ev[k], hipEventDisableTiming);
        if (e != hipSuccess) return e;
    }
    const size_t n_chunks = (bytes + FD_PIN_BYTES - 1) / FD_PIN_BYTES;
    std::vector<std::thread> drain(FD_PIN_SLOTS);
    hipError_t err = hipSuccess;
    const int dev = c->device;
    for (size_t i = 0; i < n_chunks && err == hipSuccess; ++i) {
        const int k = (int)(i % FD_PIN_SLOTS);
        if (drain[k].joinable()) drain[k].join();
        const size_t off = i * FD_PIN_BYTES, n = std::min(FD_PIN_BYTES, bytes - off);
        err = hipMemcpyAsync(c->pin[k], (const uint8_t *)src + off, n, hipMemcpyDeviceToHost, c->stream);
        if (err == hipSuccess) err = hipEventRecord(c->pin_ev[k], c->stream);
        if (err != hipSuccess) break;
        const uint8_t *pin = (const uint8_t *)c->pin[k];
        hipEvent_t ev = c->pin_ev[k];
        drain[k] = std::thread([=]() {
            (void)hipSetDevice(dev);
            if (hipEventSynchronize(ev) != hipSuccess) { int z = 0; io_err->compare_exchange_strong(z, EIO); return; }
            size_t done = 0;
            while (done < n) {
                const ssize_t w = pwrite(fd, pin + done, n - done, (off_t)(file_off + off + done));
                if (w < 0) { if (errno == EINTR) continue; int z = 0; io_err->compare_exchange_strong(z, errno ? errno : EIO); return; }
                done += (size_t)w;
            }
        });
    }
    for (auto &t : drain) if (t.joinable()) t.join();
    return err;
}

extern "C" int fdgpu_reserve_staging(fdgpu_ctx *c) { FD_LOCK(c);
    if (!c) return FDGPU_EINVAL;
    for (int k = 0; k < FD_PIN_SLOTS; ++k) {
        if (!c->pin[k]) HIPCHK(c, hipHostMalloc(&c->pin[k], FD_PIN_BYTES, hipHostMallocDefault));
        if (!c->pin_ev[k]) HIPCHK(c, hipEventCreateWithFlags(&c->pin_ev[k], hipEventDisableTiming));
    }
    return FDGPU_OK;
}

extern "C" int fdgpu_index_save(fdgpu_ctx *c, const fdgpu_index *ix, const char *prefix) { FD_LOCK(c);
    if (!c || !ix || !prefix) return FDGPU_EINVAL;
    const std::string p(prefix);
    const uint64_t H = ix->n_hashes;
    std::atomic<int> io_err{0};
    hipError_t e = hipSuccess;
    const int fv = open(p.c_str(), O_WRONLY | O_CREAT | O_TRUNC, 0644);
    const int fo = fv >= 0 ? open((p + ".offset").c_str(), O_WRONLY | O_CREAT | O_TRUNC, 0644) : -1;
    if (fv < 0 || fo < 0) { if (fv >= 0) close(fv); FAIL(c, FDGPU_EINVAL, "index save: cannot write " + p); }
    if (pwrite(fo, &H, 8, 0) != 8) io_err = errno ? errno : EIO;
    const bool trace = getenv("FDGPU_TRACE") != nullptr;
    const auto t0 = std::chrono::steady_clock::now();
    auto ms = [&]() { return std::chrono::duration<double, std::milli>(std::chrono::steady_clock::now() - t0).count(); };
    if (trace) {
        for (int k = 0; k < FD_PIN_SLOTS && e == hipSuccess; ++k) if (!c->pin[k]) e = hipHostMalloc(&c->pin[k], FD_PIN_BYTES, hipHostMallocDefault);
        fprintf(stderr, "[index_save] staging slots page-locked at %.3f ms\n", ms());
    }
    if (e == hipSuccess) e = fd_d2h_to_file(c, fv, 0, ix->value, ix->value_len, &io_err);
    if (trace) fprintf(stderr, "[index_save] %llu value bytes streamed at %.3f ms\n", (unsigned long long)ix->value_len, ms());
    if (e == hipSuccess) e = fd_d2h_to_file(c, fo, 8, ix->hashes, H * 4, &io_err);
    if (e == hipSuccess) e = fd_d2h_to_file(c, fo, 8 + H * 4, ix->offsets, (H + 1) * 8, &io_err);
    if (e == hipSuccess) e = hipStreamSynchronize(c->stream);
    if (trace) fprintf(stderr, "[index_save] offset file streamed at %.3f ms\n", ms());
    if (close(fv) != 0 && !io_err) io_err = errno ? errno : EIO;
    if (close(fo) != 0 && !io_err) io_err = errno ? errno : EIO;
    if (trace) fprintf(stderr, "[index_save] files closed at %.3f ms\n", ms());
    if (e != hipSuccess) { c->err = std::string("index save: ") + hipGetErrorString(e); return FDGPU_EHIP; }
    if (io_err) FAIL(c, FDGPU_EINVAL, "index save: cannot write " + p + " (" + strerror(io_err) + ")");
    return FDGPU_OK;
}

__global__ void k_debug_libm(int op, const float *__restrict__ a, const float *__restrict__ b, float *__restrict__ out, uint64_t n) {
    uint64_t k = (uint64_t)blockIdx.x * blockDim.x + threadIdx.x;
    if (k >= n) return;
    float x = a[k], s, c;
    switch (op) {
        case 0: fdd_sincosf(x, &s, &c); out[k] = s; break;
        case 1: fdd_sincosf(x, &s, &c); out[k] = c; break;
        case 2: out[k] = fdd_acosf(x); break;
        case 3: out[k] = fdd_atanf(x); break;
        default: out[k] = fdd_atan2f(x, b[k]); break;
    }
}
extern "C" int fdgpu_debug_libm(fdgpu_ctx *c, int op, const float *a, const float *b, float *out, uint64_t n) { FD_LOCK(c);
    if (!c || !a || !out || (op == 4 && !b) || op < 0 || op > 4) return FDGPU_EINVAL;
    if (!n) return FDGPU_OK;
    hipStream_t st = c->stream;
    HIPCHK(c, c->ws[WS_MISC0].ensure(n * 4));
    HIPCHK(c, c->ws[WS_MISC1].ensure(n * 4));
    HIPCHK(c, c->ws[WS_MISC2].ensure(n * 4));
    HIPCHK(c, hipMemcpyAsync(c->ws[WS_MISC0].p, a, n * 4, hipMemcpyHostToDevice, st));
    if (b) HIPCHK(c, hipMemcpyAsync(c->ws[WS_MISC1].p, b, n * 4, hipMemcpyHostToDevice, st));
    hipLaunchKernelGGL(k_debug_libm, dim3((unsigned)((n + 255) / 256)), dim3(256), 0, st, op, c->ws[WS_MISC0].as<float>(),
                       c->ws[WS_MISC1].as<float>(), c->ws[WS_MISC2].as<float>(), n);
    HIPCHK(c, hipGetLastError());
    HIPCHK(c, hipMemcpyAsync(out, c->ws[WS_MISC2].p, n * 4, hipMemcpyDeviceToHost, st));
    HIPCHK(c, hipStreamSynchronize(st));
    return FDGPU_OK;
}
```

### folddisco_amd/csrc/fdgpu_internal.h

```cpp
#pragma once
#include <hip/hip_runtime.h>
#include <stdint.h>
#include <functional>
#include <mutex>
#include <string>
#include <vector>
#include "../../include/fdgpu.h"
#include "../../include/fdgpu_debug.h"
#include "fd_device.h"
#include "fd_geom_other.h"
#include "fd_retrieve_host.h"

#include "fd_host_pool.h"
#include "fd_match_tables.h"

struct fd_devbuf {
    void *p = nullptr;
    size_t cap = 0;
    hipError_t ensure(size_t bytes) {
        if (bytes <= cap) return hipSuccess;
        size_t want = bytes + (bytes < ((size_t)4 << 30) ? bytes / 16 : (size_t)0) + 256;
        if (cap && cap < (64u << 20) && want < cap + cap / 2) want = cap + cap / 2;
        if (p) { hipError_t e = hipFree(p); p = nullptr; cap = 0; if (e != hipSuccess) return e; }
        hipError_t e = hipMalloc(&p, want);
        if (e != hipSuccess) { p = nullptr; return e; }
        cap = want;
        return hipSuccess;
    }
    void release() { if (p) (void)hipFree(p); p = nullptr; cap = 0; }
    template <typename T> T *as() const { return reinterpret_cast<T *>(p); }
};

struct fd_timing_entry { const char *name; hipEvent_t ev0, ev1; uint64_t bytes; };

enum {
    WS_COUNTS, WS_CURSOR, WS_SEGOFF, WS_SCANTMP, WS_TOTAL, WS_KEYS_A, WS_IDS_A, WS_KEYS_B, WS_IDS_B, WS_GHIST, WS_TOT,
    WS_TILE_B, WS_TILE_H, WS_TILE_P, WS_TILE_BO, WS_TILE_HO , WS_TILE_PO, WS_MISC0, WS_MISC1, WS_MISC2, WS_MISC3, WS_MISC4, WS_MISC5, WS_FRAMES,
    WS_CQ_KIDX, WS_CQ_NSEG, WS_CQ_WSTART, WS_CQ_SEGSUM, WS_CQ_TOPN,
    WS_QT_RANGES, WS_QT_COMPACT, WS_QT_COUNT, WS_QT_AUX, WS_RS_PLAN, WS_RS_REC, WS_RS_RECRES, WS_QT_PARTIAL, WS_QT_SURV, WS_QT_ROWBITS, WS_QT_STREAM, WS_QT_STAB, WS_QT_PIECEP, WS_QT_WIN, WS_QT_HEAD, WS_RS_SPLIT, WS_MP_QSET,
    WS_CA_PERM, WS_OK_PERM, WS_AA_PERM, WS_SRC_PERM , WS_SEG_TAB,
    WS_RS_TAB, WS_RS_SEG, WS_RS_OUT, WS_RS_RES, WS_RS_KX, WS_RS_KY, WS_RS_KOFF, WS_RS_SOL, WS_RS_CNT, WS_RS_GQ, WS_MP_ACT, WS_MP_Q,
    WS_SG_TAB , WS_SG_TAB_B, WS_SG_PAIRS, WS_SG_CURSOR,
    WS_SG_NB_PART , WS_SG_NB_OUT ,
    WS_SG_CL_TAB , WS_SG_CL_REPS ,
    WS_SG_CL_OUT , WS_SG_CL_PART , WS_SG_CL_COUNT ,
    WS_COUNT
};

enum fd_hp_slot {
    FD_HP_SCAN_A,
    FD_HP_SCAN_B,
    FD_HP_LAND,
    FD_HP_UP,
    FD_HP_FEAT,
    FD_HP_PAIRS,
    FD_HP_SLOTS
};

struct fdgpu_ctx {
    int device = 0;
    hipStream_t stream = nullptr;
    bool own_stream = false;
    std::string err;
    uint32_t last_retrieve_path = 0;
    uint32_t last_count_path = 0;
    uint32_t last_query_map_path = 0;
    fd_devbuf ws[WS_COUNT];
    bool timing = false;
    mutable std::recursive_mutex mu;
    int host_libm_matches = -1;
    unsigned long long *spec_miss = nullptr;
    std::vector<fd_timing_entry> timings;
    std::vector<hipEvent_t> event_pool;
    size_t event_used = 0;
    hipStream_t side_stream = nullptr;
    void *hbuf[FD_HP_SLOTS] = {};
    size_t hbuf_cap[FD_HP_SLOTS] = {};
    void *host_pinned(fd_hp_slot k, size_t bytes) {
        if (hbuf_cap[k] >= bytes) return hbuf[k];
        if (hbuf[k]) (void)hipHostFree(hbuf[k]);
        hbuf[k] = nullptr; hbuf_cap[k] = 0;
        const size_t want = bytes + bytes / 4 + 4096;
        if (hipHostMalloc(&hbuf[k], want, hipHostMallocDefault) != hipSuccess) { hbuf[k] = nullptr; return nullptr; }
        hbuf_cap[k] = want;
        return hbuf[k];
    }
    void *pin[16] = {};
    hipEvent_t pin_ev[16] = {};
    struct pooled { void *p; size_t cap; };
    std::vector<pooled> pool;
    void *pool_alloc(size_t bytes, hipError_t *err) {
        *err = hipSuccess;
        size_t best = (size_t)-1;
        for (size_t k = 0; k < pool.size(); ++k)
            if (pool[k].cap >= bytes && pool[k].cap <= bytes + bytes / 4 + 4096 && (best == (size_t)-1 || pool[k].cap < pool[best].cap)) best = k;
        if (best != (size_t)-1) { void *p = pool[best].p; last_cap = pool[best].cap; pool.erase(pool.begin() + best); return p; }
        void *p = nullptr;
        size_t want = bytes + bytes / 32 + 256;
        *err = hipMalloc(&p, want);
        if (*err != hipSuccess) {
            pool_drop();
            (void)hipGetLastError();
            *err = hipMalloc(&p, want);
            if (*err != hipSuccess) return nullptr;
        }
        last_cap = want;
        return p;
    }
    void pool_drop() { for (auto &b : pool) (void)hipFree(b.p); pool.clear(); }
    void pool_free(void *p, size_t cap) {
        if (!p) return;
        if (pool.size() >= 96) { (void)hipFree(p); return; }
        pool.push_back({p, cap});
    }
    size_t last_cap = 0;
    bool counted = false;
    const void *mp_bintab_at = nullptr; size_t mp_bintab_cap = 0;
    fd_host_pool host_pool;
    bool is_lane = false;
    unsigned small_par(unsigned n) const { return is_lane ? 1u : std::min(n, std::max(1u, std::thread::hardware_concurrency())); }
    void *lanes = nullptr;
};
void fd_lanes_destroy(fdgpu_ctx *c);

static inline hipEvent_t fd_next_event(fdgpu_ctx *c) {
    if (c->event_used == c->event_pool.size()) {
        hipEvent_t e;
        if (hipEventCreate(&e) != hipSuccess) return nullptr;
        c->event_pool.push_back(e);
    }
    return c->event_pool[c->event_used++];
}
struct StageTimer {
    fdgpu_ctx *c;
    size_t idx = (size_t)-1;
    StageTimer(fdgpu_ctx *ctx, const char *name, uint64_t bytes) : c(ctx) {
        if (!c || !c->timing) return;
        fd_timing_entry t;
        t.name = name; t.bytes = bytes; t.ev0 = fd_next_event(c); t.ev1 = fd_next_event(c);
        if (!t.ev0 || !t.ev1) return;
        (void)hipEventRecord(t.ev0, c->stream);
        c->timings.push_back(t);
        idx = c->timings.size() - 1;
    }
    ~StageTimer() { if (idx != (size_t)-1) (void)hipEventRecord(c->timings[idx].ev1, c->stream); }
};

#define FD_LOCK(c) std::unique_lock<std::recursive_mutex> _fd_lk; if (c) { _fd_lk = std::unique_lock<std::recursive_mutex>((c)->mu); (void)hipSetDevice((c)->device); }

struct fdgpu_batch {
    fdgpu_ctx *ctx = nullptr;
    bool owns = false;
    uint64_t n_struct = 0, n_res = 0;
    uint32_t n_work = 0;
    float *n_xyz = nullptr, *ca_xyz = nullptr, *cb_xyz = nullptr;
    uint8_t *aa = nullptr, *cb_valid = nullptr, *hash_ok = nullptr;
    uint32_t *res_off = nullptr, *wi_struct = nullptr, *wi_i0 = nullptr;
    std::vector<uint64_t> h_res_off;
    fd_batch_view view() const {
        fd_batch_view v;
        v.n_xyz = n_xyz; v.ca_xyz = ca_xyz; v.cb_xyz = cb_xyz; v.aa = aa; v.hash_ok = hash_ok; v.res_off = res_off;
        v.wi_struct = wi_struct; v.wi_i0 = wi_i0; v.n_struct = (uint32_t)n_struct; v.n_work = n_work;
        return v;
    }
};

int fd_build_work_items(fdgpu_ctx *c, fdgpu_batch *b, bool with_hash_ok = true);

#include <atomic>
static inline uint64_t fd_next_index_uid() { static std::atomic<uint64_t> n{1}; return n.fetch_add(1); }
struct fdgpu_index {
    fdgpu_ctx *ctx = nullptr;
    uint64_t n_hashes = 0, value_len = 0, n_postings = 0, n_structures = 0, first_id = 0;
    uint32_t *hashes = nullptr;
    uint64_t *offsets = nullptr;
    uint8_t *value = nullptr;
    mutable uint32_t *last_ids = nullptr;
    size_t cap_hashes = 0, cap_offsets = 0, cap_value = 0, cap_last = 0;
    mutable uint32_t *lens = nullptr;
    mutable std::mutex lens_mu;
    uint64_t uid = fd_next_index_uid();
    float *penalty = nullptr;
    mutable unsigned long long *ck_meta = nullptr;
    mutable void *ck_ent = nullptr;
    mutable uint64_t ck_n = 0, ck_first = 0, ck_S = 0;
    mutable bool ck_failed = false;
    mutable uint32_t ck_fail_skips = 0;
};

#define FD_VALUE_LATER (~0ull)
int fd_index_new(fdgpu_ctx *c, bool pooled, uint64_t H, uint64_t value_len, bool with_last, fdgpu_index **out);
hipError_t fd_index_block(fdgpu_ctx *pool, size_t bytes, void **p, size_t *cap);
int fd_index_last_ids(fdgpu_ctx *c, const fdgpu_index *ix);
hipError_t fd_count_postings(fdgpu_ctx *c, const uint8_t *value, uint64_t n, uint64_t *out);
static inline unsigned fd_grid(uint64_t n, uint64_t per) { return (unsigned)((n + per - 1) / per); }

#define FD_IXERR_DAMAGED 1u
#define FD_IXERR_LONG 2u
#define FD_LONG_LIST_BYTES 16384u
void fd_order_long_first(const uint8_t *sel, const uint8_t *is_long, uint64_t H, uint64_t *sel_pre, uint64_t *long_pre, uint64_t *scan_tmp,
                         uint64_t *total_dev, uint32_t *order, uint32_t *place, hipStream_t st);
static inline int fd_index_last_ids_staged(fdgpu_ctx *c, const fdgpu_index *ix, const char *stage) {
    if (ix->last_ids || !ix->n_hashes) return FDGPU_OK;
    StageTimer t(c, stage, ix->value_len + ix->n_hashes * 12);
    return fd_index_last_ids(c, ix);
}
struct fd_rows_dev { const uint32_t *val; const uint64_t *row_off; uint64_t n; };
int fd_rows_device(fdgpu_ctx *c, const fdgpu_index *ix, uint64_t id_lo, uint64_t id_hi, const char *what, fd_rows_dev *out);
static inline int fd_index_op_failed(fdgpu_ctx *c, int rc, fdgpu_index *const *made, size_t n = 1) {
    (void)hipStreamSynchronize(c->stream);
    for (size_t k = 0; k < n; ++k) fdgpu_index_destroy(made[k]);
    return rc;
}

struct fd_cq_dev_out {
    bool got = false, overflow = false; const void *recs = nullptr; const void *state = nullptr; uint32_t top_n = 0, cap = 0;
    std::vector<uint32_t> counts;
    const std::function<void()> *while_running = nullptr;
    uint32_t head_n = 0;
    const fd_count_rec *head = nullptr;
};
int fd_count_query_batch_impl(fdgpu_ctx *c, const fdgpu_index *ix, uint64_t n_queries, const uint64_t *q_off, const uint32_t *q_hash,
                              const uint32_t *q_node, const uint32_t *q_edge_j, const float *q_idf, const float *penalty, uint32_t top_n,
                              fd_count_rec **out, uint64_t **out_off, bool allow_dense, fd_cq_dev_out *dev, int64_t known_segments = -1,
                              const long long *known_kidx = nullptr, const uint64_t *known_len = nullptr);
int fd_posting_lengths_dev(fdgpu_ctx *c, const fdgpu_index *ix, const uint32_t *q_hash, uint64_t nq, uint64_t **dev_lengths);
uint64_t fd_maps_hashes(uint64_t n_queries, const fd_query_map *const *qms, std::vector<uint32_t> &h);
int fd_count_query_maps_len(fdgpu_ctx *c, const fdgpu_index *ix, uint64_t n_queries, const fd_query_map *const *qms, const uint64_t *len,
                            const uint64_t *primary_len, const float *penalty, float total_structures, uint32_t top_n, fd_count_rec **out,
                            uint64_t **out_off, fd_cq_dev_out *dev, const uint32_t *seg = nullptr, const long long *kidx = nullptr, bool allow_dense = true);
int fd_posting_lengths_segs(fdgpu_ctx *c, const fdgpu_index *ix, const uint32_t *q_hash, uint64_t nq, uint64_t *lengths, uint32_t *segs, long long *kidx = nullptr,
                            const uint8_t **land_out = nullptr);
int fd_count_query_maps_top_impl(fdgpu_ctx *c, const fdgpu_index *ix, uint64_t n_queries, const fd_query_map *const *qms, const float *penalty, float total_structures,
                                 uint32_t top_n, fd_count_rec **out, uint64_t **out_off, fd_cq_dev_out *dev, bool allow_dense = true);

struct fd_rb_dev_out { bool got = false; const void *recs = nullptr; const int32_t *residues = nullptr; uint64_t n_recs = 0, n_res = 0; };
int fd_retrieve_batch_dev(fdgpu_ctx *c, const fdgpu_batch *db, const uint8_t *resname_std, uint64_t n_queries, const uint32_t *cand, const uint64_t *cand_off,
                          const fd_query_map *const *qms, const fdgpu_batch *qb, const uint32_t *q_struct, const fd_hash_params *p, float ca_distance_cutoff,
                          uint32_t node_count, uint32_t partial_fit, fd_match_rec **matches, uint64_t **match_off, int32_t **residues, uint64_t **res_off, fd_rb_dev_out *dev);
hipError_t fd_d2h_to_file(fdgpu_ctx *c, int fd, uint64_t file_off, const void *src, size_t bytes, std::atomic<int> *io_err);
hipError_t fd_d2h_big(fdgpu_ctx *c, void *dst, const void *src, size_t bytes);
void *fd_out_alloc(size_t bytes, bool pinned = false);

void fd_launch_selfcheck(const fd_quant &q, uint32_t *out, hipStream_t st);
void fd_launch_hash_ok(const uint8_t *aa, const uint8_t *cb_valid, uint8_t *ok, uint64_t n, hipStream_t st);
void fd_launch_pair_count(const fd_batch_view &B, const fd_hash_consts &C, uint32_t *counts, hipStream_t st);
void fd_launch_pair_emit(const fd_batch_view &B, const fd_hash_consts &C, const uint64_t *seg_off, uint32_t *cursor, uint32_t *keys,
                         uint32_t *ids, uint32_t first_id, hipStream_t st);
void fd_launch_frames(const fd_batch_view &B, uint64_t n_res, void *frames, hipStream_t st);
void fd_launch_pair_count2(const fd_batch_view &B, const fd_hash_consts &C, uint32_t *counts, hipStream_t st);
void fd_launch_pair_emit2(const fd_batch_view &B, const void *frames, const fd_hash_consts &C, const uint64_t *seg_off, uint32_t *cursor,
                          uint32_t *keys, void *ids, bool ids16, uint32_t first_id, hipStream_t st);
int fd_radix_sort_pairs16(uint32_t *keys_a, uint16_t *vals_a, uint32_t *keys_b, uint16_t *vals_b, uint64_t n, int key_bits, uint32_t *ghist,
                          uint64_t *tot, hipStream_t st, fdgpu_ctx *timing_ctx = nullptr);
void fd_launch_frames_perm(const fd_batch_view &B, float *ca_perm, uint8_t *ok_perm, uint8_t *aa_perm, uint32_t *src_perm, unsigned long long *wide_flag, hipStream_t st);
void fd_launch_pair_count_msd(const fd_batch_view &B, const fd_hash_consts &C, const float *n_xyz, const float *cb_xyz, const uint32_t *src_perm, void *frames,
                              uint32_t *counts, hipStream_t st);
void fd_launch_pair_emit_msd(const fd_batch_view &B, const void *frames, const fd_hash_consts &C, const uint64_t *seg_off, uint32_t *keys,
                             uint16_t *ids, hipStream_t st);
uint32_t fd_rs_seg_num_tiles(uint64_t n, uint32_t n_seg);
uint64_t fd_rs_seg_tot_words(uint64_t n, uint32_t n_seg);
size_t fd_rs_seg_tab_bytes(uint64_t n, uint32_t n_seg);
struct fd_rs_digit { uint32_t plane, shift; };
int fd_radix_sort_pairs16_seg(uint32_t *keys_a, uint16_t *vals_a, uint32_t *keys_b, uint16_t *vals_b, uint64_t n, const uint64_t *seg_off, uint64_t stride,
                              uint32_t n_seg, const fd_rs_digit *digits, int passes, uint32_t *ghist, uint64_t *tot, void *seg_tab, hipStream_t st, fdgpu_ctx *timing_ctx = nullptr,
                              unsigned long long *overflow = nullptr);
void fd_launch_row_count(const fd_batch_view &B, const fd_hash_consts &C, uint32_t *row_cnt, float cutoff, hipStream_t st);
void fd_launch_row_emit(const fd_batch_view &B, const fd_hash_consts &C, const uint64_t *row_off, uint32_t *keys, float cutoff, uint32_t *ids,
                        uint32_t first_id, hipStream_t st, int ids_partner = 0);
template <typename TIn>
void fd_exclusive_scan(const TIn *in, uint64_t n, uint64_t *out, uint64_t *chunk_tmp, uint64_t *total_dev, hipStream_t st);
uint64_t fd_scan_tmp_elems(uint64_t n);
uint32_t fd_rs_num_tiles(uint64_t n);
int fd_radix_sort_pairs(uint32_t *keys_a, uint32_t *vals_a, uint32_t *keys_b, uint32_t *vals_b, uint64_t n, int key_bits, uint32_t *ghist,
                        uint64_t *tot, hipStream_t st, fdgpu_ctx *timing_ctx = nullptr);
uint32_t fd_enc_num_tiles(uint64_t n);
void fd_launch_enc_sizes(const uint32_t *keys, const void *ids, int codec, uint32_t first_id, uint64_t n, uint32_t *tb, uint32_t *th, uint32_t *tp,
                         const uint64_t *seg_off, uint64_t S, uint64_t *bo, hipStream_t st);
void fd_launch_enc_write(const uint32_t *keys, const void *ids, int codec, uint32_t first_id, uint64_t n, const uint64_t *tbo, const uint64_t *tho,
                         uint8_t *value, uint32_t *hashes, uint64_t *offsets, uint32_t *last_ids, const uint64_t *total_bytes_dev, uint64_t H,
                         const uint64_t *bo, hipStream_t st);
void fd_launch_uniq_flags(const uint32_t *keys, const uint32_t *ids, uint64_t n, uint8_t *flags, hipStream_t st);
void fd_launch_compact(const uint32_t *keys, const uint8_t *flags, const uint64_t *pos, uint64_t n, uint32_t *out, hipStream_t st);
void fd_launch_gather_u64(const uint64_t *src, const uint64_t *idx, uint64_t n, uint64_t *dst, hipStream_t st);

struct cq_args {
    const uint32_t *hashes; const uint64_t *offsets; const uint8_t *value; uint64_t H;
    const uint32_t *q_hash; uint64_t nq;
    uint32_t *hash_bits;
    const unsigned long long *row_meta;
    uint32_t *match;
    unsigned long long *idf;
    int packed;
    uint32_t words; uint32_t first_id; uint32_t S;
};

#define QT_CELL_LOG2 11
#define QT_BINS 2048
#define QT_MAX_ROWS 1024
#define QT_MAXB 16
struct qt_state { uint32_t thr_bin, above, thr_key, count; };
struct qt_aux { uint32_t need_l2, shift2, edge, pad; };
struct qt_args {
    const uint8_t *value; const uint64_t *offsets;
    const unsigned long long *ck_meta; const uint2 *ck_ent;
    const long long *kidx;
    const unsigned long long *row_meta;
    const uint64_t *q_rows;
    const float *penalty;
    uint32_t nq, n_queries, S, first_id, NT, NC, tile_log2, plan_log2;
    uint4 *ranges;
    uint32_t *c_nid, *c_key;
    uint32_t *ccount;
    uint32_t *ghist;
    qt_state *state; qt_aux *aux;
    void *out; uint32_t cap;
    void *stream_ids; uint16_t *stream_row;
    uint2 *stream_tab;
    uint32_t *stream_used; uint32_t stream_cap;
    uint4 *pieces;
    uint32_t *piece_p;
    uint32_t *win;
    uint4 *heads;
    uint32_t win_per_row, top_n;
    uint32_t max_rows;
    const uint64_t *slices; uint32_t n_slices;
    unsigned long long *partial;
    uint32_t *g_bm, *g_rank, *g_tcount, *g_nid;
    uint32_t *g_rowbits; uint32_t g_wpr;
    const uint32_t *g_eend, *g_nend;
};
void fd_launch_ck_count(const uint64_t *offsets, uint64_t H, uint32_t NC, uint32_t *cnt, hipStream_t st);
void fd_launch_ck_fill(const uint64_t *offsets, const uint8_t *value, uint64_t H, uint32_t NC, uint32_t S, uint32_t first_id, const uint64_t *ent_off,
                       unsigned long long *meta, void *ent, hipStream_t st);
void fd_launch_qt_plan(const qt_args &A, hipStream_t st);
void fd_launch_qt_score(const qt_args &A, hipStream_t st);
void fd_launch_qt_big_score(const qt_args &A, hipStream_t st);
void fd_launch_qt_big_select(const qt_args &A, uint32_t top_n, void *sorted, hipStream_t st);
void fd_launch_qt_select(const qt_args &A, uint32_t top_n, void *sorted, hipStream_t st);
#define QT_WIN_CONT 0x80000000u
void fd_launch_qt_layout(const qt_args &A, hipStream_t st);
void fd_launch_qt_score32(const qt_args &A, hipStream_t st);

void fd_launch_index_lens(const uint64_t *offsets, const uint8_t *value, uint64_t H, uint32_t *lens, hipStream_t st);
void fd_launch_posting_lookup(const uint32_t *hashes, const uint64_t *offsets, const uint32_t *lens, uint64_t H, const uint32_t *q_hash, uint64_t nq, uint64_t *lengths,
                              uint32_t *nseg, long long *kidx, hipStream_t st);
void fd_launch_cq_plan(const cq_args &A, long long *kidx, uint32_t *nseg, hipStream_t st);
void fd_launch_cq_seg(const cq_args &A, const long long *kidx, const uint64_t *wstart, uint32_t *segsum, uint64_t n_items, bool split,
                      hipStream_t st);
void fd_launch_cq_rows_finalize(const cq_args &A, const uint64_t *q_rows, uint32_t n_queries, const uint64_t *slices, uint32_t n_slices, uint32_t *node_cnt,
                                uint32_t *edge_cnt, uint8_t *flags, uint64_t max_rows_per_query, hipStream_t st);

enum : uint32_t {
    MP_FOUND = 1u,
    MP_CANDS = 2u,
    MP_CANDS_UNORDERED = 4u,
    MP_CANDS_PACKED = 8u,
    MP_ON_DEVICE = 16u,
    MP_VOTES = 32u
};
#define MP_QH_LDS 1024
#define MP_SUBQ_STRIDE 16u
struct mp_args {
    fd_batch_view B;
    fd_hash_consts C;
    float cutoff;
    const uint32_t *cand; uint32_t n_cand;
    const uint32_t *wi_cand; const uint32_t *wi_i0; const uint32_t *wi_query; uint32_t n_work;
    const uint32_t *wi_j0; uint32_t j_span;
    const mp_query_dev *qtab;
    const uint32_t *qset;
    const uint8_t *resname_std;
    uint32_t aa1_mask, aa2_mask;
    int use_prefilter;
    const uint32_t *q_hashes; uint32_t n_hashes;
    const uint32_t *aad_start;
    const float *aad_dist; const uint32_t *aad_qi; uint32_t n_aad;
    const uint32_t *iv_start; const float2 *iv;
    const uint32_t *iv_grp;
    float ca_window;
    unsigned long long *n_found, *n_cands;
    const uint4 *cinfo; const uint32_t *act;
    unsigned long long *q_cnt; uint4 *chunk_hdr; uint32_t *chunk_ij; uint32_t cap_subq;
    uint32_t *res_h, *res_meta; float *res_d; uint2 *chunk_cnt; ulonglong2 *chunk_base;
    const uint32_t *bintab;
    int compact;
    fd_pair_rec *found; fd_cand_rec *cands;
    unsigned long long cap_found, cap_cands;
    uint32_t n_cfg;
    fd_quant qk[8];
    uint32_t mode;
    const uint32_t *cj_mask;
    const uint32_t *mask_off;
    uint32_t *votes; const uint64_t *vt_off; const uint32_t *vt_qs; const uint8_t *cj_comp;
    const float *sd_dist; const uint32_t *sd_qi;
};
void fd_launch_mp_items(const uint32_t *db_res_off, const uint32_t *cand, uint32_t n_cand, const uint32_t *wbase, const uint32_t *cq, uint32_t j_span, uint32_t *wc,
                        uint32_t *wi, uint32_t *wq, uint32_t *wj, hipStream_t st, const uint8_t *aa, const uint8_t *hash_ok, const uint8_t *resname_std, int tert,
                        const struct mp_query_dev *qtab, void *cinfo , uint32_t *act );
struct fd_vote_plan {
    const uint8_t *cj_comp; uint64_t n_bits;
    const uint64_t *vt_off; const uint32_t *vt_qs; uint64_t n_counters;
    const uint64_t *row_off; const uint32_t *row_len; uint64_t n_rows;
    fd_vote_row *rows;
    const float *sd_dist; const uint32_t *sd_qi; uint64_t n_sd;
};
struct fd_mp_request {
    uint32_t mode = MP_FOUND | MP_CANDS;
    const uint32_t *cj_mask = nullptr, *mask_off = nullptr; uint64_t mask_words = 0;
    uint32_t **pk_key = nullptr, **pk_val = nullptr;
    fd_vote_plan *votes = nullptr;
    fd_mp_tables *tables = nullptr;
    const std::function<void()> *while_scanning = nullptr;
};
void fd_launch_vote_rows(const uint32_t *votes, const uint64_t *row_off, const uint32_t *row_len, uint64_t n_rows, fd_vote_row *out, hipStream_t st);
void fd_launch_match_pairs(const mp_args &A, hipStream_t st);
void fd_launch_mp_qset_build(const mp_query_dev *qtab, uint32_t n_queries, uint32_t max_hashes, const uint32_t *q_hashes, uint32_t *qset, hipStream_t st);
void fd_launch_found_key_ij(const fd_pair_rec *f, uint64_t n, uint32_t *key, uint32_t *val, hipStream_t st);
void fd_launch_found_key_slot(const fd_pair_rec *f, const uint32_t *val, uint64_t n, uint32_t *key, hipStream_t st);
void fd_launch_found_gather(const fd_pair_rec *f, const uint32_t *val, uint64_t n, fd_pair_rec *out, hipStream_t st);
void fd_launch_pack_cands(const fd_cand_rec *c, uint64_t n, uint32_t *key, uint32_t *val, hipStream_t st);
void fd_launch_kabsch(const float *x, const float *y, const uint64_t *off, uint64_t n, float *rmsd, float *rot, float *tran, hipStream_t st, uint64_t n_points = 0);
void fd_launch_metrics(const float *ref, const float *mov, const uint64_t *off, uint64_t n, const float *rot, const float *tran, const float *d0, float *out,
                       hipStream_t st, uint64_t n_points = 0);
void fd_launch_lms_qcp(const float *x, const float *y, const uint64_t *off, uint64_t n, float *rmsd, float *rot, float *tran, uint32_t *core_len,
                       uint8_t *flags, uint32_t *order, hipStream_t st);
void fd_launch_cq_compact_batch(const cq_args &A, const uint32_t *node_cnt, const uint32_t *edge_cnt, const uint8_t *flags, const uint64_t *pos,
                                const float *penalty, uint64_t total, void *out, hipStream_t st);
void fd_launch_cq_topn(const void *recs, const uint64_t *off, uint32_t n_queries, uint32_t top_n, uint32_t cap, void *out, void *state, uint32_t *ghist,
                       hipStream_t st);
void fd_launch_cq_topn_acc(const cq_args &A, const float *penalty, const uint32_t *node_cnt, const uint32_t *edge_cnt, uint32_t n_queries, uint32_t top_n,
                           uint32_t cap, void *out, void *state, uint32_t *ghist, hipStream_t st);
void fd_launch_cq_topn_dense(const cq_args &A, const uint64_t *q_rows, const float *penalty, uint32_t *keys, uint32_t n_queries, uint32_t top_n, uint32_t cap,
                             void *out, void *state, uint32_t *ghist, hipStream_t st);
void fd_launch_cq_topn_sort(const void *sel, uint32_t cap, const void *state, uint32_t n_queries, uint32_t top_n, void *out, hipStream_t st);
void fd_launch_get_entries(const uint32_t *hashes, const uint64_t *offsets, const uint8_t *value, uint64_t H, const uint32_t *q_hash, uint64_t nq,
                           const uint64_t *out_off, uint32_t *out, hipStream_t st);
struct rs_query_dev {
    uint32_t qh_off, n_hashes;
    uint32_t map_off;
    uint32_t idx_off, n_idx;
    uint32_t q_size;
    uint32_t q_res0;
    uint32_t pad;
};
struct rs_match_dev { uint32_t slot, ci, same, res_pos, prob0, prob1; float idf; uint32_t ord; };
#define RS_CNT_STRIDE 512
struct rs_args {
    const fd_pair_rec *found; const fd_cand_rec *cands;
    const uint32_t *seg_f, *seg_c, *perm_f, *perm_c;
    const uint32_t *cand, *slot_q;
    const uint32_t *order;
    uint32_t *slot_matches;
    const uint32_t *db_res_off; const float *db_ca, *db_cb, *q_ca, *q_cb;
    const rs_query_dev *qt;
    const uint32_t *hashes, *kfirst; const uint8_t *sym;
    const uint32_t *map_qi, *map_qj; const float *map_idf;
    const uint32_t *indices;
    const float *d0tab;
    uint32_t node_count;
    uint32_t node_cap;
    unsigned long long *counters;
    uint32_t *flags;
    rs_match_dev *matches; int32_t *residues; float *kx, *ky; uint64_t *koff; float *d0;
    uint32_t *gq, *gr;
    uint64_t cap_matches, cap_res, cap_prob, cap_pts;
    uint4 *sp_edges;
    uint32_t *sp_nodes;
    unsigned long long *sp_comps;
    uint4 *sp_head;
    uint2 *sp_work;
    uint4 *sp_np;
    uint32_t *sp_gq, *sp_gr;
    uint32_t *sp_big, *sp_big_n;
    const uint32_t *n_listed;
};
void fd_launch_rs_group(const fd_pair_rec *found, uint64_t nf, const fd_cand_rec *cands, uint64_t nc, uint32_t n_cand, uint32_t *cnt, uint32_t *seg, uint32_t *cur,
                        uint32_t *perm_f, uint32_t *perm_c, hipStream_t st);
void fd_launch_rs_slots(const rs_args &A, uint32_t n_cand, hipStream_t st);
void fd_launch_rs_points(const rs_args &A, uint64_t n_prob, uint64_t n_points, hipStream_t st);
void fd_launch_rs_records_dev(const void *matches, uint64_t n, const uint32_t *slot_matches, uint32_t n_cand, const uint64_t *cand_off, const uint32_t *slot_q,
                              const rs_query_dev *qt, uint32_t n_queries, uint32_t *scratch, uint64_t *match_off, uint64_t *res_off, const float *rmsd,
                              const float *rot, const float *tran, const float *met, const int32_t *residues, void *out, int32_t *out_res, hipStream_t st);
int fd_match_pairs_multi(fdgpu_ctx *c, const fdgpu_batch *db, const uint8_t *resname_std, uint64_t n_queries, const fd_match_query *qs,
                         const uint32_t *cand, const uint64_t *cand_off, const fd_hash_params *p, fd_pair_rec **found, uint64_t *n_found,
                         fd_cand_rec **cands, uint64_t *n_cands, const fd_mp_request &rq = fd_mp_request());
```

### folddisco_amd/csrc/k_hash.hip

```cpp
#include "fd_device.h"
#include "fd_geom_other.h"
#ifndef FD_EMIT_WAVES
#define FD_EMIT_WAVES 5
#endif
#define FD_MSD_BUCKETS 40u

__global__ __launch_bounds__(FD_WAVE) void k_pair_count(fd_batch_view B, fd_hash_consts C, uint32_t *__restrict__ counts) {
    uint32_t w = fd_xcd_remap(blockIdx.x, B.n_work);
    if (w >= B.n_work) return;
    const uint32_t s = B.wi_struct[w];
    const uint32_t r0 = B.res_off[s], r1 = B.res_off[s + 1];
    const uint32_t i = B.wi_i0[w] + threadIdx.x;
    const bool vi = i < r1 && B.hash_ok[i];
    fd_v3 cai = {0.f, 0.f, 0.f};
    if (vi) cai = fd_load3(B.ca_xyz, i);
    uint32_t cnt = 0;
    for (uint32_t j = r0; j < r1; ++j) {
        if (!B.hash_ok[j]) continue;
        fd_v3 caj = fd_load3(B.ca_xyz, j);
        float d2 = fd_dist2(cai, caj);
        cnt += (vi && i != j && !(d2 > C.d2_max)) ? 1u : 0u;
    }
    for (int off = 32; off > 0; off >>= 1) cnt += __shfl_down(cnt, off, FD_WAVE);
    if (threadIdx.x == 0 && cnt) atomicAdd(&counts[s], cnt);
}

template <bool WRITE_IDS>
__device__ __forceinline__ void drain(const fd_batch_view &B, const fd_hash_consts &C, const uint32_t *q, uint32_t n,
                                      uint32_t i0, uint32_t r0, uint32_t s, uint32_t id, const uint64_t *seg_off,
                                      uint32_t *cursor, uint32_t *keys, uint32_t *ids) {
    const uint32_t lane = threadIdx.x;
    uint32_t base = 0;
    if (lane == 0) base = atomicAdd(&cursor[s], n);
    base = __shfl(base, 0, FD_WAVE);
    if (lane < n) {
        uint32_t e = q[lane];
        uint32_t i = i0 + (e >> 16), j = r0 + (e & 0xffffu);
        fd_v3 n1 = fd_load3(B.n_xyz, i), ca1 = fd_load3(B.ca_xyz, i), cb1 = fd_load3(B.cb_xyz, i);
        fd_v3 n2 = fd_load3(B.n_xyz, j), ca2 = fd_load3(B.ca_xyz, j), cb2 = fd_load3(B.cb_xyz, j);
        fd_feature f = fd_pair_feature(n1, ca1, cb1, n2, ca2, cb2);
        uint32_t h = fd_hash_enc(B.aa[i], B.aa[j], f, C.q);
        uint64_t pos = seg_off[s] + base + lane;
        keys[pos] = h;
        if (WRITE_IDS) ids[pos] = id;
    }
}

template <bool WRITE_IDS>
__global__ __launch_bounds__(FD_WAVE) void k_pair_emit(fd_batch_view B, fd_hash_consts C, const uint64_t *__restrict__ seg_off,
                                                       uint32_t *__restrict__ cursor, uint32_t *__restrict__ keys,
                                                       uint32_t *__restrict__ ids, uint32_t first_id) {
    __shared__ uint32_t q[2 * FD_WAVE];
    uint32_t w = fd_xcd_remap(blockIdx.x, B.n_work);
    if (w >= B.n_work) return;
    const uint32_t s = B.wi_struct[w];
    const uint32_t r0 = B.res_off[s], r1 = B.res_off[s + 1];
    const uint32_t i0 = B.wi_i0[w];
    const uint32_t lane = threadIdx.x;
    const uint32_t i = i0 + lane;
    const bool vi = i < r1 && B.hash_ok[i];
    fd_v3 cai = {0.f, 0.f, 0.f};
    if (vi) cai = fd_load3(B.ca_xyz, i);
    uint32_t qn = 0;
    for (uint32_t j = r0; j < r1; ++j) {
        if (!B.hash_ok[j]) continue;
        fd_v3 caj = fd_load3(B.ca_xyz, j);
        float d2 = fd_dist2(cai, caj);
        bool pass = vi && i != j && !(d2 > C.d2_max);
        uint64_t m = __ballot(pass);
        if (m == 0) continue;
        if (pass) q[qn + fd_mbcnt(m)] = (lane << 16) | (j - r0);
        qn += (uint32_t)__popcll(m);
        if (qn >= FD_WAVE) {
            __syncthreads();
            qn -= FD_WAVE;
            drain<WRITE_IDS>(B, C, q + qn, FD_WAVE, i0, r0, s, first_id + s, seg_off, cursor, keys, ids);
            __syncthreads();
        }
    }
    if (qn) {
        __syncthreads();
        drain<WRITE_IDS>(B, C, q, qn, i0, r0, s, first_id + s, seg_off, cursor, keys, ids);
    }
}

__global__ __launch_bounds__(256) void k_frames(fd_batch_view B, uint32_t n_res, fd_frame *__restrict__ frames) {
    uint32_t r = blockIdx.x * blockDim.x + threadIdx.x;
    if (r >= n_res) return;
    fd_frame F;
    if (B.hash_ok[r]) F = fd_make_frame(fd_load3(B.n_xyz, r), fd_load3(B.ca_xyz, r), fd_load3(B.cb_xyz, r));
    else { F = fd_frame{}; F.ca = fd_load3(B.ca_xyz, r); }
    F.pad = __uint_as_float((uint32_t)B.aa[r]);
    frames[r] = F;
}

typedef float fd_f2 __attribute__((ext_vector_type(2)));
#define FD_NOT_HASHABLE 0x100u

__device__ __forceinline__ bool fd_lane_of(uint64_t m) { return __builtin_amdgcn_inverse_ballot_w64(m); }

template <bool TYPES, class Step, class RunEnd>
__device__ __forceinline__ void fd_filter_block(const fd_batch_view &B, float d2_max, const fd_v3 &cai, uint64_t vim, uint32_t i0, uint32_t jb, uint32_t r1,
                                                float *s_cj, Step &&step, RunEnd &&run_end) {
    const uint32_t lane = threadIdx.x;
    const uint32_t jl = jb + lane;
    fd_v3 cj = {0.f, 0.f, 0.f};
    uint32_t kind = FD_NOT_HASHABLE;
    if (jl < r1) {
        cj = fd_load3(B.ca_xyz, jl);
        if (B.hash_ok[jl]) kind = TYPES ? (uint32_t)B.aa[jl] : 0u;
    }
    fd_wave_lds_fence();
    s_cj[lane] = cj.x; s_cj[FD_WAVE + lane] = cj.y; s_cj[2 * FD_WAVE + lane] = cj.z;
    fd_wave_lds_fence();
    const uint64_t okm = __ballot(kind != FD_NOT_HASHABLE);
    const uint64_t starts = __ballot(kind != (uint32_t)__shfl_up((int)kind, 1, FD_WAVE)) | 1ull;
    const bool last_block = jb + FD_WAVE >= r1;
    const uint32_t nk = okm ? 64u - (uint32_t)__builtin_clzll(okm) : 0u;
    const uint32_t nkf = (last_block && nk == 0) ? 1u : nk;
    const bool first = jb == i0;
    const fd_f2 ax = {cai.x, cai.x}, ay = {cai.y, cai.y}, az = {cai.z, cai.z};
    uint32_t k = 0;
    while (k < nkf) {
        const uint32_t t = (uint32_t)__builtin_amdgcn_readlane((int)kind, (int)k);
        const uint64_t rest = (starts >> k) >> 1;
        uint32_t ke = rest ? k + 1u + (uint32_t)__builtin_ctzll(rest) : (uint32_t)FD_WAVE;
        ke = ke < nkf ? ke : nkf;
        const bool run_last = last_block && ke >= nkf;
        const bool dead = t == FD_NOT_HASHABLE;
        if (dead && !run_last) { k = ke; continue; }
        const uint64_t vr = dead ? 0ull : vim;
        uint64_t gt = first ? (1ull << k) - 1ull : ~0ull;
        do {
            const fd_f2 xj = {s_cj[k], s_cj[k + 1]}, yj = {s_cj[FD_WAVE + k], s_cj[FD_WAVE + k + 1]}, zj = {s_cj[2 * FD_WAVE + k], s_cj[2 * FD_WAVE + k + 1]};
            const fd_f2 dx = ax - xj, dy = ay - yj, dz = az - zj;
            const fd_f2 d2 = (dx * dx + dy * dy) + dz * dz;
            const uint64_t gt1 = gt << 1 | 1ull;
            const uint64_t m0 = __ballot(!(d2.x > d2_max)) & vr & gt;
            const uint64_t m1 = (k + 1u < ke) ? (__ballot(!(d2.y > d2_max)) & vr & gt1) : 0ull;
            gt = gt1 << 1 | 1ull;
            const uint32_t k0 = k;
            k += 2;
            step(k0, t, m0, m1, run_last && k >= ke);
        } while (k < ke);
        k = ke;
        run_end(t);
    }
}

__global__ __launch_bounds__(FD_WAVE) void k_pair_count2(fd_batch_view B, fd_hash_consts C, uint32_t *__restrict__ counts) {
    __shared__ float s_cj[3 * FD_WAVE + 1];
    uint32_t w = fd_xcd_remap(blockIdx.x, B.n_work);
    if (w >= B.n_work) return;
    const uint32_t s = B.wi_struct[w];
    const uint32_t r1 = B.res_off[s + 1];
    const uint32_t i0 = B.wi_i0[w];
    const uint32_t i = i0 + threadIdx.x;
    const bool vi = i < r1 && B.hash_ok[i];
    fd_v3 cai = {0.f, 0.f, 0.f};
    if (vi) cai = fd_load3(B.ca_xyz, i);
    const uint64_t vim = __ballot(vi);
    uint32_t cnt = 0;
    for (uint32_t jb = i0; jb < r1; jb += FD_WAVE)
        fd_filter_block<false>(B, C.d2_max, cai, vim, i0, jb, r1, s_cj,
                               [&](uint32_t, uint32_t, uint64_t m0, uint64_t m1, bool) { cnt += (fd_lane_of(m0) ? 1u : 0u) + (fd_lane_of(m1) ? 1u : 0u); },
                               [](uint32_t) {});
    cnt *= 2u;
    for (int off = 32; off > 0; off >>= 1) cnt += __shfl_down(cnt, off, FD_WAVE);
    if (threadIdx.x == 0 && cnt) atomicAdd(&counts[s], cnt);
}

__global__ __launch_bounds__(256) void k_frames_perm(fd_batch_view B, float *__restrict__ ca_perm, uint8_t *__restrict__ ok_perm, uint8_t *__restrict__ aa_perm,
                                                     uint32_t *__restrict__ src_perm, unsigned long long *__restrict__ wide_flag) {
    __shared__ uint32_t cnt[32], cur[32], wcnt[4][32];
    const uint32_t s = blockIdx.x, lane = threadIdx.x & (FD_WAVE - 1u), wave = threadIdx.x / FD_WAVE;
    const uint32_t r0 = B.res_off[s], r1 = B.res_off[s + 1];
    if (threadIdx.x < 32) cnt[threadIdx.x] = 0;
    __syncthreads();
    for (uint32_t r = r0 + threadIdx.x; r < r1; r += 256) {
        const uint32_t a = B.aa[r];
        atomicAdd(&cnt[(B.hash_ok[r] && a < 20u) ? a : 20u], 1u);
    }
    __syncthreads();
    if (threadIdx.x == 0) { uint32_t run = 0; for (int k = 0; k < 21; ++k) { cur[k] = run; run += cnt[k]; } }
    __syncthreads();
    for (uint32_t rb = r0; rb < r1; rb += 256) {
        const uint32_t r = rb + threadIdx.x;
        uint32_t a = 0, cls = 21u;
        bool ok = false;
        if (r < r1) {
            a = B.aa[r];
            ok = B.hash_ok[r] != 0;
            if (ok && a >= 20u) {
                ok = false;
                if (wide_flag) atomicOr(wide_flag, 1ull);
            }
            cls = ok ? a : 20u;
        }
        uint64_t mine = 0;
        uint32_t wc = 0;
#pragma unroll 1
        for (uint32_t k = 0; k < 21u; ++k) {
            const uint64_t m = __ballot(cls == k);
            if (cls == k) mine = m;
            if (lane == k) wc = (uint32_t)__popcll(m);
        }
        if (lane < 21u) wcnt[wave][lane] = wc;
        __syncthreads();
        if (r < r1) {
            uint32_t p = r0 + cur[cls] + fd_mbcnt(mine);
            for (uint32_t v = 0; v < wave; ++v) p += wcnt[v][cls];
            const fd_v3 ca = fd_load3(B.ca_xyz, r);
            ca_perm[3ull * p] = ca.x; ca_perm[3ull * p + 1] = ca.y; ca_perm[3ull * p + 2] = ca.z;
            ok_perm[p] = ok ? 1 : 0;
            aa_perm[p] = (uint8_t)a;
            src_perm[p] = r;
        }
        __syncthreads();
        if (threadIdx.x < 21u) cur[threadIdx.x] += wcnt[0][threadIdx.x] + wcnt[1][threadIdx.x] + wcnt[2][threadIdx.x] + wcnt[3][threadIdx.x];
        __syncthreads();
    }
}

__global__ __launch_bounds__(FD_WAVE) void k_pair_count_msd(fd_batch_view B, fd_hash_consts C, const float *__restrict__ n_xyz, const float *__restrict__ cb_xyz,
                                                            const uint32_t *__restrict__ src_perm, fd_frame *__restrict__ frames, uint32_t *__restrict__ counts) {
    __shared__ uint32_t s_cnt[FD_WAVE];
    __shared__ float s_cj[3 * FD_WAVE + 1];
    uint32_t w = fd_xcd_remap(blockIdx.x, B.n_work);
    if (w >= B.n_work) return;
    const uint32_t s = B.wi_struct[w];
    const uint32_t r1 = B.res_off[s + 1];
    const uint32_t i0 = B.wi_i0[w];
    const uint32_t lane = threadIdx.x;
    const uint32_t i = i0 + lane;
    const bool vi = i < r1 && B.hash_ok[i];
    fd_v3 cai = {0.f, 0.f, 0.f};
    uint32_t aai = 0;
    if (vi) { cai = fd_load3(B.ca_xyz, i); aai = B.aa[i]; }
    if (i < r1) {
        fd_frame F;
        if (vi) { const uint32_t src = src_perm[i]; F = fd_make_frame(fd_load3(n_xyz, src), cai, fd_load3(cb_xyz, src)); }
        else { F = fd_frame{}; F.ca = fd_load3(B.ca_xyz, i); }
        F.pad = __uint_as_float((uint32_t)B.aa[i]);
        frames[i] = F;
    }
    s_cnt[lane] = 0;
    __syncthreads();
    const uint64_t vim = __ballot(vi);
    uint32_t c_lo = 0, c_hi = 0, run = 0;
    const uint32_t hi_i = aai >> 4;
    for (uint32_t jb = i0; jb < r1; jb += FD_WAVE)
        fd_filter_block<true>(B, C.d2_max, cai, vim, i0, jb, r1, s_cj,
                              [&](uint32_t, uint32_t, uint64_t m0, uint64_t m1, bool) { run += (fd_lane_of(m0) ? 1u : 0u) + (fd_lane_of(m1) ? 1u : 0u); },
                              [&](uint32_t t) {
                                  if (t >= 16u) c_hi += run; else c_lo += run;
                                  if (run) atomicAdd(&s_cnt[(t * 2u + hi_i) & (FD_WAVE - 1u)], run);
                                  run = 0;
                              });
    if (c_lo) atomicAdd(&s_cnt[aai * 2u], c_lo);
    if (c_hi) atomicAdd(&s_cnt[aai * 2u + 1u], c_hi);
    __syncthreads();
    if (lane < FD_MSD_BUCKETS) counts[(uint64_t)lane * B.n_work + w] = s_cnt[lane];
}

__device__ __forceinline__ fd_frame load_frame(const fd_frame *__restrict__ frames, uint32_t r) {
    const float4 *p = reinterpret_cast<const float4 *>(frames + r);
    float4 a = p[0], b = p[1], c = p[2], d = p[3], e = p[4];
    fd_frame F;
    F.ca = {a.x, a.y, a.z}; F.cb = {a.w, b.x, b.y}; F.r1 = {b.z, b.w, c.x}; F.t1 = {c.y, c.z, c.w};
    F.len = d.x; F.pad = d.y; F.s2 = {d.z, d.w, e.x}; F.nv2 = {e.y, e.z, e.w};
    return F;
}
__device__ __forceinline__ fd_frame hot_frame(const float4 &a, const float4 &b, const float4 &c, const float4 &d) {
    fd_frame F{};
    F.ca = {a.x, a.y, a.z}; F.cb = {a.w, b.x, b.y}; F.r1 = {b.z, b.w, c.x}; F.t1 = {c.y, c.z, c.w};
    F.len = d.x; F.pad = d.y;
    return F;
}

__device__ __attribute__((noinline)) uint2 pair_both_tab_exact(const fd_frame *__restrict__ frames, uint32_t i, uint32_t j, uint32_t aai,
                                                               uint32_t aaj, float dist_disc, float ang_disc, const uint32_t *tab) {
    fd_frame Fi = load_frame(frames, i), Fj = load_frame(frames, j);
    fd_quant q;
    q.dist_disc = dist_disc; q.ang_disc = ang_disc; q.ang2_disc = 0.0f; q.type = FD_HASH_PDBTR;
    uint32_t a, b;
    fd_pair_both_tab(Fi, Fj, aai, aaj, q, tab, &a, &b);
    return make_uint2(a, b);
}

template <int TAB, bool IDS16, bool MSD, bool DT = false>
__device__ __forceinline__ void drain2(const fd_batch_view &B, const fd_frame *__restrict__ frames, const fd_hash_consts &C,
                                       const uint32_t *tab, const uint32_t *q, uint32_t n, uint32_t i0, uint32_t r0, uint32_t s, uint32_t id,
                                       const uint64_t *seg_off, uint32_t *cursor, uint32_t *keys, void *ids, const float4 *s_fi,
                                       uint32_t *s_bc, uint64_t *s_boff) {
    const uint32_t lane = threadIdx.x;
    uint32_t base = 0, slots = 0;
    if (!MSD) {
        if (lane == 0) base = atomicAdd(&cursor[s], 2u * n);
        base = __shfl(base, 0, FD_WAVE);
    } else {
        s_bc[lane] = 0;
        fd_wave_lds_fence();
        if (lane < n) {
            const uint32_t e = q[lane], il = (e >> 16) & 63u, aj = e >> 22;
            const uint32_t ai = TAB == 2 ? __float_as_uint(s_fi[192 + il].y) : (uint32_t)B.aa[i0 + il];
            const uint32_t bf = ai * 2u + (aj >> 4), br = aj * 2u + (ai >> 4);
            slots = atomicAdd(&s_bc[bf], 1u) | atomicAdd(&s_bc[br], 1u) << 8 | bf << 16 | br << 24;
        }
    }
    uint32_t h_ij = 0, h_ji = 0, aai = 0, aaj = 0;
    if (lane < n) {
        uint32_t e = q[lane];
        uint32_t i = i0 + ((e >> 16) & 63u), j = r0 + (e & 0xffffu);
        if (TAB == 2) {
            const uint32_t il = (e >> 16) & 63u;
            const fd_frame Fi = hot_frame(s_fi[il], s_fi[64 + il], s_fi[128 + il], s_fi[192 + il]);
            const float4 *pj = reinterpret_cast<const float4 *>(frames + j);
            const fd_frame Fj = hot_frame(pj[0], pj[1], pj[2], pj[3]);
            aai = __float_as_uint(Fi.pad); aaj = __float_as_uint(Fj.pad);
#if defined(FD_EMIT_STUB) && FD_EMIT_STUB == 1
            h_ij = aai << 25 | aaj << 20 | (__float_as_uint(Fj.ca.x) & 0xfffffu); h_ji = aaj << 25 | aai << 20 | (__float_as_uint(Fi.ca.x) & 0xfffffu);
            if (false)
#endif
            if (!fd_pair_both_spec<DT>(Fi, Fj, aai, aaj, C.q, tab, tab + 32, &h_ij, &h_ji, tab + 64)) {
                uint2 h = pair_both_tab_exact(frames, i, j, B.aa[i], B.aa[j], C.q.dist_disc, C.q.ang_disc, tab);
                h_ij = h.x; h_ji = h.y;
                if (C.spec_miss) atomicAdd(C.spec_miss, 1ull);
            }
        } else if (TAB == 1) {
            uint2 h = pair_both_tab_exact(frames, i, j, B.aa[i], B.aa[j], C.q.dist_disc, C.q.ang_disc, tab);
            h_ij = h.x; h_ji = h.y;
        } else {
            fd_frame Fi = load_frame(frames, i), Fj = load_frame(frames, j);
            fd_pair_both(Fi, Fj, B.aa[i], B.aa[j], C.q, &h_ij, &h_ji);
        }
    }
    if (MSD) {
        if (lane < n) {
            const uint32_t sf = slots & 255u, sr = (slots >> 8) & 255u, bf = (slots >> 16) & 255u, br = slots >> 24;
            if ((((h_ij | h_ji) >> 30) || (h_ij >> 24) != bf || (h_ji >> 24) != br) && C.wide_flag) atomicOr(C.wide_flag, 1ull);
            const uint64_t pf = s_boff[bf] + sf, pr = s_boff[br] + sr;
            keys[pf] = (h_ij << 24) | s;
            keys[pr] = (h_ji << 24) | s;
            ((uint16_t *)ids)[pf] = (uint16_t)(h_ij >> 8);
            ((uint16_t *)ids)[pr] = (uint16_t)(h_ji >> 8);
        }
        fd_wave_lds_fence();
        if (lane < FD_MSD_BUCKETS) s_boff[lane] += s_bc[lane];
        return;
    }
    if (lane < n) {
        const uint64_t so = seg_off[s];
        uint64_t pos = so * C.seg_mul + (uint64_t)C.seg_cfg * (seg_off[s + 1] - so) + base + lane;
        if (IDS16) {
            if (((h_ij | h_ji) >> 30) && C.wide_flag) atomicOr(C.wide_flag, 1ull);
            uint32_t hi = s >> 16;
            uint16_t lo = (uint16_t)(s & 0xffffu);
            keys[pos] = (h_ij << 2) | hi;
            keys[pos + n] = (h_ji << 2) | hi;
            ((uint16_t *)ids)[pos] = lo;
            ((uint16_t *)ids)[pos + n] = lo;
        } else {
            keys[pos] = h_ij;
            keys[pos + n] = h_ji;
            ((uint32_t *)ids)[pos] = id;
            ((uint32_t *)ids)[pos + n] = id;
        }
    }
}

template <int TAB, bool IDS16, bool MSD, bool DT = false>
__global__ __launch_bounds__(FD_WAVE, FD_EMIT_WAVES) void k_pair_emit2(fd_batch_view B, const fd_frame *__restrict__ frames, fd_hash_consts C,
                                                        const uint64_t *__restrict__ seg_off, uint32_t *__restrict__ cursor,
                                                        uint32_t *__restrict__ keys, void *__restrict__ ids, uint32_t first_id) {
    __shared__ uint32_t q[3 * FD_WAVE];
    __shared__ float s_cj[3 * FD_WAVE + 1];
    __shared__ uint32_t tab[DT ? 64 + FD_DIST_NTHR + 1 : 64];
    uint32_t w = fd_xcd_remap(blockIdx.x, B.n_work);
    if (w >= B.n_work) return;
    if (TAB) {
        if (DT && threadIdx.x < FD_DIST_NTHR) tab[64 + threadIdx.x] = fd_dist_thr_bits[threadIdx.x];
        if (threadIdx.x == 0) {
            fd_fill_bintab(tab);
            for (int k = 0; k < FD_BINTAB_WORDS; ++k) tab[32 + k] = tab[k];
            for (int m = 0; m < 4; ++m)
                for (int k = 0; k < 4; ++k) { uint32_t v = tab[32 + 7 + 5 * m + k]; tab[32 + 7 + 5 * m + k] = v > 0x7f7fffffu ? 0x7f7fffffu : v; }
        }
        __syncthreads();
    }
    const uint32_t s = B.wi_struct[w];
    const uint32_t r0 = B.res_off[s], r1 = B.res_off[s + 1];
    const uint32_t i0 = B.wi_i0[w];
    const uint32_t lane = threadIdx.x;
    const uint32_t i = i0 + lane;
    const bool vi = i < r1 && B.hash_ok[i];
    fd_v3 cai = {0.f, 0.f, 0.f};
    if (vi) cai = fd_load3(B.ca_xyz, i);
    __shared__ float4 s_fi[4 * FD_WAVE];
    if (TAB == 2 && i < r1) {
        const float4 *fp = reinterpret_cast<const float4 *>(frames + i);
#pragma unroll
        for (int k = 0; k < 4; ++k) s_fi[k * FD_WAVE + lane] = fp[k];
    }
    __shared__ uint32_t s_bc[MSD ? FD_WAVE : 1];
    __shared__ uint64_t s_boff[MSD ? FD_MSD_BUCKETS : 1];
    if (MSD && lane < FD_MSD_BUCKETS) s_boff[lane] = seg_off[(uint64_t)lane * B.n_work + w];
    __syncthreads();
    const uint64_t vim = __ballot(vi);
    const uint32_t lane16 = lane << 16;
    uint32_t qn = 0;
    for (uint32_t jb = i0; jb < r1; jb += FD_WAVE) {
        const uint32_t jrel = jb - r0;
        fd_filter_block<MSD>(B, C.d2_max, cai, vim, i0, jb, r1, s_cj,
            [&](uint32_t k, uint32_t t, uint64_t m0, uint64_t m1, bool last) {
                const uint32_t tag = (MSD ? t << 22 : 0u) | (jrel + k);
                if (m0) {
                    if (fd_lane_of(m0)) q[__builtin_amdgcn_mbcnt_hi((uint32_t)(m0 >> 32), __builtin_amdgcn_mbcnt_lo((uint32_t)m0, qn))] = lane16 | tag;
                    qn += (uint32_t)__popcll(m0);
                }
                if (m1) {
                    if (fd_lane_of(m1)) q[__builtin_amdgcn_mbcnt_hi((uint32_t)(m1 >> 32), __builtin_amdgcn_mbcnt_lo((uint32_t)m1, qn))] = lane16 | (tag + 1u);
                    qn += (uint32_t)__popcll(m1);
                }
                while (qn >= FD_WAVE || (last && qn)) {
                    fd_wave_lds_fence();
                    uint32_t n = qn < FD_WAVE ? qn : FD_WAVE;
                    qn -= n;
                    drain2<TAB, IDS16, MSD, DT>(B, frames, C, tab, q + qn, n, i0, r0, s, first_id + s, seg_off, cursor, keys, ids, s_fi, s_bc, s_boff);
                    fd_wave_lds_fence();
                }
            },
            [](uint32_t) {});
    }
}

__global__ __launch_bounds__(FD_WAVE) void k_row_count(fd_batch_view B, fd_hash_consts C, uint32_t *__restrict__ row_cnt, float cutoff) {
    uint32_t w = fd_xcd_remap(blockIdx.x, B.n_work);
    if (w >= B.n_work) return;
    const uint32_t s = B.wi_struct[w];
    const uint32_t r0 = B.res_off[s], r1 = B.res_off[s + 1];
    const uint32_t i = B.wi_i0[w] + threadIdx.x;
    if (i >= r1) return;
    if (fd_own_descriptor(C.q.type)) {
        uint32_t cnt = 0;
        if (B.aa[i] != 255)
            for (uint32_t j = r0; j < r1; ++j)
                cnt += (j != i && B.aa[j] != 255 && fd_accept_other(C.q.type, B, r0, r1, i, j, cutoff)) ? 1u : 0u;
        row_cnt[i] = cnt;
        return;
    }
    const bool vi = B.hash_ok[i];
    fd_v3 cai = fd_load3(B.ca_xyz, i);
    uint32_t cnt = 0;
    for (uint32_t j = r0; j < r1; ++j) {
        if (!B.hash_ok[j]) continue;
        float d2 = fd_dist2(cai, fd_load3(B.ca_xyz, j));
        cnt += (vi && i != j && !(d2 > C.d2_max)) ? 1u : 0u;
    }
    row_cnt[i] = cnt;
}

__global__ __launch_bounds__(FD_WAVE) void k_row_emit(fd_batch_view B, fd_hash_consts C, const uint64_t *__restrict__ row_off,
                                                      uint32_t *__restrict__ keys, float cutoff, uint32_t *__restrict__ ids, uint32_t first_id, int ids_partner) {
    uint32_t w = fd_xcd_remap(blockIdx.x, B.n_work);
    if (w >= B.n_work) return;
    const uint32_t s = B.wi_struct[w];
    const uint32_t r0 = B.res_off[s], r1 = B.res_off[s + 1];
    const uint32_t i = B.wi_i0[w] + threadIdx.x;
    if (i >= r1) return;
    if (fd_own_descriptor(C.q.type)) {
        if (B.aa[i] == 255) return;
        uint64_t pos = row_off[i];
        float f[FD_NFEAT];
        for (uint32_t j = r0; j < r1; ++j) {
            if (j == i || B.aa[j] == 255 || !fd_feature_other(C.q.type, B, r0, r1, i, j, cutoff, f)) continue;
            if (ids) ids[pos] = ids_partner ? j : first_id + s;
            keys[pos++] = fd_hash_other(C.q.type, f, C.q);
        }
        return;
    }
    if (!B.hash_ok[i]) return;
    fd_v3 n1 = fd_load3(B.n_xyz, i), ca1 = fd_load3(B.ca_xyz, i), cb1 = fd_load3(B.cb_xyz, i);
    uint32_t aa1 = B.aa[i];
    uint64_t pos = row_off[i];
    for (uint32_t j = r0; j < r1; ++j) {
        if (!B.hash_ok[j] || i == j) continue;
        fd_v3 ca2 = fd_load3(B.ca_xyz, j);
        if (fd_dist2(ca1, ca2) > C.d2_max) continue;
        fd_v3 n2 = fd_load3(B.n_xyz, j), cb2 = fd_load3(B.cb_xyz, j);
        fd_feature f = fd_pair_feature(n1, ca1, cb1, n2, ca2, cb2);
        if (ids) ids[pos] = ids_partner ? j : first_id + s;
        keys[pos++] = fd_hash_enc(aa1, B.aa[j], f, C.q);
    }
}

__global__ void k_hash_ok(const uint8_t *__restrict__ aa, const uint8_t *__restrict__ cb_valid, uint8_t *__restrict__ ok, uint64_t n) {
    uint64_t k = (uint64_t)blockIdx.x * blockDim.x + threadIdx.x;
    if (k < n) ok[k] = (aa[k] != 255 && (cb_valid == nullptr || cb_valid[k])) ? 1 : 0;
}

__global__ void k_selfcheck(fd_quant q, uint32_t *__restrict__ out ) {
    if (threadIdx.x != 0 || blockIdx.x != 0) return;
    const fd_v3 N[3] = {{6.661f, 8.291f, 43.860f}, {10.483f, 7.756f, 49.260f}, {5.260f, -1.068f, 41.296f}};
    const fd_v3 CA[3] = {{6.994f, 8.354f, 42.405f}, {9.429f, 7.479f, 48.266f}, {5.547f, 0.158f, 42.050f}};
    const fd_v3 CB[3] = {{8.251f, 7.488f, 42.026f}, {10.033f, 6.489f, 47.255f}, {5.773f, 1.360f, 41.130f}};
    const uint32_t AA[3] = {8u, 3u, 15u};
    const int PI[6] = {1, 1, 0, 0, 2, 2}, PJ[6] = {0, 2, 1, 2, 1, 0};
    uint32_t tab[64 + FD_DIST_NTHR + 1];
    fd_fill_bintab(tab);
    for (int k = 0; k < FD_BINTAB_WORDS; ++k) tab[32 + k] = tab[k];
    for (int m = 0; m < 4; ++m)
        for (int k = 0; k < 4; ++k) { uint32_t v = tab[32 + 7 + 5 * m + k]; tab[32 + 7 + 5 * m + k] = v > 0x7f7fffffu ? 0x7f7fffffu : v; }
    for (int k = 0; k < FD_DIST_NTHR; ++k) tab[64 + k] = fd_dist_thr_bits[k];
    fd_frame F[3];
    for (int r = 0; r < 3; ++r) F[r] = fd_make_frame(N[r], CA[r], CB[r]);
    for (int k = 0; k < 6; ++k) {
        const int i = PI[k], j = PJ[k];
        out[k] = fd_hash_pdbtr(AA[i], AA[j], fd_pair_feature(N[i], CA[i], CB[i], N[j], CA[j], CB[j]), q);
        uint32_t a, b;
        fd_pair_both_tab(F[i], F[j], AA[i], AA[j], q, tab, &a, &b);
        out[6 + k] = a;
        if (!fd_pair_both_spec(F[i], F[j], AA[i], AA[j], q, tab, tab + 32, &a, &b)) fd_pair_both_tab(F[i], F[j], AA[i], AA[j], q, tab, &a, &b);
        out[12 + k] = a;
        if (!fd_pair_both_spec<true>(F[i], F[j], AA[i], AA[j], q, tab, tab + 32, &a, &b, tab + 64)) fd_pair_both_tab(F[i], F[j], AA[i], AA[j], q, tab, &a, &b);
        out[18 + k] = a;
    }
}

extern "C++" {
void fd_launch_selfcheck(const fd_quant &q, uint32_t *out, hipStream_t st) { hipLaunchKernelGGL(k_selfcheck, dim3(1), dim3(64), 0, st, q, out); }
void fd_launch_hash_ok(const uint8_t *aa, const uint8_t *cb_valid, uint8_t *ok, uint64_t n, hipStream_t st) {
    if (!n) return;
    hipLaunchKernelGGL(k_hash_ok, dim3((unsigned)((n + 255) / 256)), dim3(256), 0, st, aa, cb_valid, ok, n);
}
static inline unsigned grid_for(uint32_t n_work) { return ((n_work + 7u) / 8u) * 8u; }
void fd_launch_pair_count(const fd_batch_view &B, const fd_hash_consts &C, uint32_t *counts, hipStream_t st) {
    if (!B.n_work) return;
    hipLaunchKernelGGL(k_pair_count, dim3(grid_for(B.n_work)), dim3(FD_WAVE), 0, st, B, C, counts);
}
void fd_launch_pair_emit(const fd_batch_view &B, const fd_hash_consts &C, const uint64_t *seg_off, uint32_t *cursor,
                         uint32_t *keys, uint32_t *ids, uint32_t first_id, hipStream_t st) {
    if (!B.n_work) return;
    if (ids)
        hipLaunchKernelGGL(k_pair_emit<true>, dim3(grid_for(B.n_work)), dim3(FD_WAVE), 0, st, B, C, seg_off, cursor, keys, ids, first_id);
    else
        hipLaunchKernelGGL(k_pair_emit<false>, dim3(grid_for(B.n_work)), dim3(FD_WAVE), 0, st, B, C, seg_off, cursor, keys, ids, first_id);
}
void fd_launch_frames(const fd_batch_view &B, uint64_t n_res, void *frames, hipStream_t st) {
    if (!n_res) return;
    hipLaunchKernelGGL(k_frames, dim3((unsigned)((n_res + 255) / 256)), dim3(256), 0, st, B, (uint32_t)n_res, (fd_frame *)frames);
}
void fd_launch_pair_count2(const fd_batch_view &B, const fd_hash_consts &C, uint32_t *counts, hipStream_t st) {
    if (!B.n_work) return;
    hipLaunchKernelGGL(k_pair_count2, dim3(grid_for(B.n_work)), dim3(FD_WAVE), 0, st, B, C, counts);
}
void fd_launch_pair_emit2(const fd_batch_view &B, const void *frames, const fd_hash_consts &C, const uint64_t *seg_off, uint32_t *cursor,
                          uint32_t *keys, void *ids, bool ids16, uint32_t first_id, hipStream_t st) {
    if (!B.n_work) return;
    dim3 g(grid_for(B.n_work)), b(FD_WAVE);
    const fd_frame *F = (const fd_frame *)frames;
    if (C.use_tab >= 2 && ids16) hipLaunchKernelGGL((k_pair_emit2<2, true, false>), g, b, 0, st, B, F, C, seg_off, cursor, keys, ids, first_id);
    else if (C.use_tab >= 2) hipLaunchKernelGGL((k_pair_emit2<2, false, false>), g, b, 0, st, B, F, C, seg_off, cursor, keys, ids, first_id);
    else if (C.use_tab && ids16) hipLaunchKernelGGL((k_pair_emit2<1, true, false>), g, b, 0, st, B, F, C, seg_off, cursor, keys, ids, first_id);
    else if (C.use_tab) hipLaunchKernelGGL((k_pair_emit2<1, false, false>), g, b, 0, st, B, F, C, seg_off, cursor, keys, ids, first_id);
    else if (ids16) hipLaunchKernelGGL((k_pair_emit2<0, true, false>), g, b, 0, st, B, F, C, seg_off, cursor, keys, ids, first_id);
    else hipLaunchKernelGGL((k_pair_emit2<0, false, false>), g, b, 0, st, B, F, C, seg_off, cursor, keys, ids, first_id);
}
void fd_launch_frames_perm(const fd_batch_view &B, float *ca_perm, uint8_t *ok_perm, uint8_t *aa_perm, uint32_t *src_perm, unsigned long long *wide_flag, hipStream_t st) {
    if (!B.n_struct) return;
    hipLaunchKernelGGL(k_frames_perm, dim3(B.n_struct), dim3(256), 0, st, B, ca_perm, ok_perm, aa_perm, src_perm, wide_flag);
}
void fd_launch_pair_count_msd(const fd_batch_view &B, const fd_hash_consts &C, const float *n_xyz, const float *cb_xyz, const uint32_t *src_perm, void *frames,
                              uint32_t *counts, hipStream_t st) {
    if (!B.n_work) return;
    hipLaunchKernelGGL(k_pair_count_msd, dim3(grid_for(B.n_work)), dim3(FD_WAVE), 0, st, B, C, n_xyz, cb_xyz, src_perm, (fd_frame *)frames, counts);
}
void fd_launch_pair_emit_msd(const fd_batch_view &B, const void *frames, const fd_hash_consts &C, const uint64_t *seg_off, uint32_t *keys,
                             uint16_t *ids, hipStream_t st) {
    if (!B.n_work) return;
    dim3 g(grid_for(B.n_work)), b(FD_WAVE);
    const fd_frame *F = (const fd_frame *)frames;
    if (C.use_tab == 3) hipLaunchKernelGGL((k_pair_emit2<2, true, true, true>), g, b, 0, st, B, F, C, seg_off, (uint32_t *)nullptr, keys, (void *)ids, 0u);
    else if (C.use_tab == 2) hipLaunchKernelGGL((k_pair_emit2<2, true, true>), g, b, 0, st, B, F, C, seg_off, (uint32_t *)nullptr, keys, (void *)ids, 0u);
    else if (C.use_tab) hipLaunchKernelGGL((k_pair_emit2<1, true, true>), g, b, 0, st, B, F, C, seg_off, (uint32_t *)nullptr, keys, (void *)ids, 0u);
    else hipLaunchKernelGGL((k_pair_emit2<0, true, true>), g, b, 0, st, B, F, C, seg_off, (uint32_t *)nullptr, keys, (void *)ids, 0u);
}
void fd_launch_row_count(const fd_batch_view &B, const fd_hash_consts &C, uint32_t *row_cnt, float cutoff, hipStream_t st) {
    if (!B.n_work) return;
    hipLaunchKernelGGL(k_row_count, dim3(grid_for(B.n_work)), dim3(FD_WAVE), 0, st, B, C, row_cnt, cutoff);
}
void fd_launch_row_emit(const fd_batch_view &B, const fd_hash_consts &C, const uint64_t *row_off, uint32_t *keys, float cutoff, uint32_t *ids,
                        uint32_t first_id, hipStream_t st, int ids_partner) {
    if (!B.n_work) return;
    hipLaunchKernelGGL(k_row_emit, dim3(grid_for(B.n_work)), dim3(FD_WAVE), 0, st, B, C, row_off, keys, cutoff, ids, first_id, ids_partner);
}
}
```

### include/fdgpu_debug.h

```cpp
#ifndef FDGPU_DEBUG_H
#define FDGPU_DEBUG_H
#include "fdgpu.h"
#ifdef __cplusplus
extern "C" {
#endif

int fdgpu_debug_merge_gathered(fdgpu_ctx *ctx, uint32_t world, uint64_t n_queries, uint32_t top_n, const uint8_t *messages,
                               fd_count_rec **out, uint64_t **out_off);
int fdgpu_debug_merge_retrieved(fdgpu_ctx *ctx, uint32_t world, uint64_t n_queries, const uint64_t *counts, const fd_match_rec *const *rank_matches,
                                const int32_t *const *rank_residues, const uint64_t *nres_per, fd_match_rec **matches, uint64_t **match_off,
                                int32_t **residues, uint64_t **res_off);
int fdgpu_debug_gunzip(const uint8_t *in, uint64_t n, uint8_t **out, uint64_t *n_out);
int fdgpu_debug_libm(fdgpu_ctx *ctx, int op, const float *a, const float *b, float *out, uint64_t n);

int fdgpu_debug_encode_stream(fdgpu_ctx *ctx, const uint32_t *hashes, const uint32_t *ids, uint64_t n, fdgpu_index **out);
int fdgpu_debug_encode_stream_b24(fdgpu_ctx *ctx, const uint32_t *hashes, const uint32_t *local_ids, uint64_t n, uint64_t first_id, fdgpu_index **out);

int fdgpu_debug_host_components(const uint32_t *edge_i, const uint32_t *edge_j, uint64_t n_edges, uint32_t node_count, uint32_t **residues,
                                uint64_t **comp_off, uint64_t *n_comps);
int fdgpu_debug_hash_is_symmetric(uint32_t hash_type, const uint32_t *hashes, uint64_t n, uint8_t *out);
int fdgpu_debug_host_retrieve_slot(const uint32_t *found_i, const uint32_t *found_j, const uint32_t *found_hash, uint64_t n_found, const uint32_t *cand_qi,
                                   const uint32_t *cand_i, const uint32_t *cand_j, uint64_t n_pairs, uint32_t n_target, const fd_query_map *qm,
                                   uint32_t hash_type, uint32_t node_count, uint32_t two_pass, uint32_t packed, uint64_t *n_recs, float **idf,
                                   uint32_t **same, int32_t **residues);

int fdgpu_debug_match_tables(uint64_t n_queries, const fd_match_query *qs, const uint32_t *cand, const uint64_t *cand_off, const uint64_t *res_off,
                             uint64_t n_struct, uint32_t hash_type, uint32_t dev_items, uint32_t pooled, uint32_t **block, uint64_t *layout,
                             uint64_t *scalars, const char **message);

#define FDGPU_PATH_TILED 1u
#define FDGPU_PATH_SUMS32 2u
#define FDGPU_PATH_STREAM 4u
#define FDGPU_PATH_SLICED 8u
#define FDGPU_PATH_ROWS 16u
#define FDGPU_PATH_PACKED 32u
#define FDGPU_PATH_OVERFLOW 64u
int fdgpu_debug_last_count_path(fdgpu_ctx *ctx, uint32_t *flags);

#define FDGPU_RPATH_DEVICE_TRIED 1u
#define FDGPU_RPATH_DEVICE_DONE 2u
#define FDGPU_RPATH_LIMIT 4u
#define FDGPU_RPATH_CAPACITY 8u
#define FDGPU_RPATH_TWO_PASS 16u
#define FDGPU_RPATH_SPLIT 32u
int fdgpu_debug_last_retrieve_path(fdgpu_ctx *ctx, uint32_t *flags);

#define FDGPU_QMPATH_HOST_EXPAND 1u
#define FDGPU_QMPATH_DEVICE_EXPAND 2u
#define FDGPU_QMPATH_CHAIN 4u
#define FDGPU_QMPATH_CHAIN_LENGTHS 8u
#define FDGPU_QMPATH_SORT_DEDUPE 16u
int fdgpu_debug_last_query_map_path(fdgpu_ctx *ctx, uint32_t *flags);

int fdgpu_debug_qm_pairs(uint64_t n_queries, const uint32_t *q_struct, const uint64_t *q_off, const uint32_t *q_index, const uint64_t *res_off,
                         uint32_t **pair_i, uint32_t **pair_j, uint64_t *pair_off);
int fdgpu_debug_qm_fields(uint32_t hash_type, int32_t *out);
int fdgpu_debug_qm_expand(const float *features, const uint8_t *valid, const uint32_t *pair_i, const uint32_t *pair_j, uint64_t n_pairs, uint64_t r0,
                          const uint32_t *q_index, uint64_t n_q, const uint8_t *const *subs, const uint32_t *n_subs, uint32_t hash_type,
                          const float *dist_thr, uint64_t n_dist, const float *angle_thr_rad, uint64_t n_angle, float **cand_features,
                          uint32_t **cand_recs, uint64_t *n_cands);
int fdgpu_debug_qm_first_insertions(const uint32_t *hashes, uint64_t n_cands, uint32_t n_cfg, uint64_t table_max, uint64_t set_min, uint32_t **keep,
                                    uint64_t *n_keep);
int fdgpu_debug_qm_arena(uint64_t n, uint64_t n_indices, uint64_t n_aad, uint32_t with_post, uint64_t *offsets);
int fdgpu_debug_qm_fill(const uint32_t *keep, uint64_t n, const uint32_t *hashes, uint64_t n_cands, uint32_t n_cfg, uint64_t c0, const uint32_t *cand_recs,
                        const uint32_t *valid_pairs, uint64_t per_pair, const uint32_t *pair_i, const uint32_t *pair_j, uint64_t r0, const float *pair_idf,
                        const uint32_t *pair_primary, const uint64_t *post_len, const uint32_t *post_seg, const long long *post_kidx, uint64_t index_uid,
                        const uint32_t *indices, uint64_t n_indices, const uint8_t *aad_aa1, const uint8_t *aad_aa2, const float *aad_dist,
                        const uint32_t *aad_qi, uint64_t n_aad, uint32_t pooled, fd_query_map **out);

#ifdef __cplusplus
}
#endif
#endif
```

Measured before the change: 1.712 million structures/s.

## Cache pair-filter bitmasks from count pass and replay them in emit pass

The MSD count kernel now stores per-tile 64-bit neighbor-distance masks into a new workspace buffer indexed by per-work-item column offsets. The emit kernel replays these masks instead of recomputing CA distance filters, so the distance pass over all residue pairs runs once instead of twice. In exchange it adds mask write and read traffic plus a large extra allocation, with an OOM fallback that releases the buffer and retries without masks.

```diff
diff --git a/folddisco_amd/_lib.py b/folddisco_amd/_lib.py
--- a/folddisco_amd/_lib.py
+++ b/folddisco_amd/_lib.py
@@ -250,6 +250,7 @@
     ("fdgpu_debug_merge_gathered", C.c_int, [VP, C.c_uint32, C.c_uint64, C.c_uint32, u8p, C.POINTER(C.POINTER(CountRec)), C.POINTER(u64p)]),
     ("fdgpu_debug_libm", C.c_int, [VP, C.c_int, f32p, f32p, f32p, C.c_uint64]),
     ("fdgpu_debug_last_count_path", C.c_int, [VP, u32p]),
+    ("fdgpu_debug_last_build_mask_bytes", C.c_int, [VP, u64p]),
     ("fdgpu_debug_last_retrieve_path", C.c_int, [VP, u32p]),
     ("fdgpu_debug_last_query_map_path", C.c_int, [VP, u32p]),
     ("fdgpu_debug_qm_pairs", C.c_int, [C.c_uint64, u32p, u64p, u32p, u64p, C.POINTER(u32p), C.POINTER(u32p), u64p]),
diff --git a/folddisco_amd/csrc/fd_api_build.hip b/folddisco_amd/csrc/fd_api_build.hip
--- a/folddisco_amd/csrc/fd_api_build.hip
+++ b/folddisco_amd/csrc/fd_api_build.hip
@@ -244,7 +244,11 @@
     StageTimer t(c, "frames", b->n_res * (37 + sizeof(fd_frame)));
     fd_launch_frames(b->view(), b->n_res, c->ws[WS_FRAMES].p, c->stream);
 }
-static int ib_count_msd(fdgpu_ctx *c, const fdgpu_batch *b, const fd_hash_consts &C, fd_batch_view &V, uint64_t *P1) {
+static bool ib_pair_masks_wanted(const fdgpu_ctx *c, const fd_hash_consts &C) {
+    const char *e = getenv("FDGPU_PAIR_MASKS");
+    return !(e && e[0] == '0') && C.use_tab == 3 && !c->pair_masks_crowded;
+}
+static int ib_count_msd(fdgpu_ctx *c, const fdgpu_batch *b, const fd_hash_consts &C, fd_batch_view &V, uint64_t *P1, uint64_t **masks) {
     hipStream_t st = c->stream;
     const uint64_t R1 = std::max<uint64_t>(b->n_res, 1), NS = (uint64_t)IB_BUCKETS * b->n_work;
     HIPCHK(c, c->ws[WS_CA_PERM].ensure(R1 * 12));
@@ -263,9 +267,14 @@
     HIPCHK(c, c->ws[WS_SEGOFF].ensure((NS + 2) * 8));
     HIPCHK(c, c->ws[WS_SCANTMP].ensure(fd_scan_tmp_elems(std::max<uint64_t>(NS, b->n_res)) * 8 + 64));
     HIPCHK(c, c->ws[WS_TOTAL].ensure(64));
+    *masks = nullptr;
+    if (ib_pair_masks_wanted(c, C) && b->wi_col) {
+        if (c->ws[WS_PAIR_MASKS].ensure((b->n_mask_cols + FD_MASK_SLACK_WORDS) * 8) == hipSuccess) *masks = c->ws[WS_PAIR_MASKS].as<uint64_t>();
+        else (void)hipGetLastError();
+    }
     {
         StageTimer t(c, "pair_count", b->n_res * (14 + 28 + sizeof(fd_frame)) + NS * 4);
-        fd_launch_pair_count_msd(V, C, b->n_xyz, b->cb_xyz, c->ws[WS_SRC_PERM].as<uint32_t>(), c->ws[WS_FRAMES].p, c->ws[WS_COUNTS].as<uint32_t>(), st);
+        fd_launch_pair_count_msd(V, C, b->n_xyz, b->cb_xyz, c->ws[WS_SRC_PERM].as<uint32_t>(), c->ws[WS_FRAMES].p, c->ws[WS_COUNTS].as<uint32_t>(), *masks, st);
     }
     int rc = scan_counts(c, NS, P1);
     uint64_t odd = 0;
@@ -277,9 +286,10 @@
     StageTimer t(c, "pair_emit", b->n_res * 37 + P * 8);
     fd_launch_row_emit(b->view(), C, c->ws[WS_MISC1].as<uint64_t>(), K.ka, p->dist_cutoff, (uint32_t *)K.ia, (uint32_t)first_id, c->stream);
 }
-static void ib_emit_msd(fdgpu_ctx *c, const fdgpu_batch *b, const fd_batch_view &V, const fd_hash_consts &C, const ib_keys &K, uint64_t P) {
+static void ib_emit_msd(fdgpu_ctx *c, const fdgpu_batch *b, const fd_batch_view &V, const fd_hash_consts &C, const ib_keys &K, uint64_t P, const uint64_t *masks) {
     StageTimer t(c, "pair_emit", b->n_res * 37 + P * 6);
-    fd_launch_pair_emit_msd(V, c->ws[WS_FRAMES].p, C, c->ws[WS_SEGOFF].as<uint64_t>(), K.ka, (uint16_t *)K.ia, c->stream);
+    c->last_build_mask_bytes = masks ? b->n_mask_cols * 8 : 0;
+    fd_launch_pair_emit_msd(V, c->ws[WS_FRAMES].p, C, c->ws[WS_SEGOFF].as<uint64_t>(), K.ka, (uint16_t *)K.ia, masks, c->stream);
 }
 static int ib_emit_structure_major(fdgpu_ctx *c, const fdgpu_batch *b, const fd_hash_params *p, const ib_form &F, const fd_hash_consts &C, const ib_keys &K, uint64_t P,
                                    uint64_t first_id) {
@@ -314,6 +324,7 @@
     ib_form F;
     int rc = ib_choose_form(c, b, p, first_id, force32, F);
     if (rc) return rc;
+    c->last_build_mask_bytes = 0;
     HIPCHK(c, c->ws[WS_FRAMES].ensure(std::max<uint64_t>(b->n_res, 1) * sizeof(fd_frame)));
     if ((rc = ib_clear_words(c))) return rc;
     fd_hash_consts C = fd_make_consts_cfg(p, 0);
@@ -337,11 +348,13 @@
         if ((rc = ib_reserve_keys(c, F, P, K)) || (rc = ib_emit_structure_major(c, b, p, F, C, K, P, first_id))) return rc;
         cur = ib_sort(c, F, K, P);
         break;
-    case IB_MSD:
-        if ((rc = ib_count_msd(c, b, C, V, &P)) || (rc = ib_reserve_keys(c, F, P, K))) return rc;
-        ib_emit_msd(c, b, V, C, K, P);
+    case IB_MSD: {
+        uint64_t *masks = nullptr;
+        if ((rc = ib_count_msd(c, b, C, V, &P, &masks)) || (rc = ib_reserve_keys(c, F, P, K))) return rc;
+        ib_emit_msd(c, b, V, C, K, P, masks);
         if ((rc = ib_sort_msd(c, b, K, P, &cur))) return rc;
         break;
+    }
     }
     return encode_sorted_stream(c, cur ? K.kb : K.ka, cur ? K.ib : K.ia, F.codec, first_id, P, b->n_struct, F.seg_stride, out);
 }
@@ -350,7 +363,21 @@
     const char *e32 = getenv("FDGPU_IDS32");
     int rc = index_build_impl(c, b, p, first_id, out, e32 && e32[0] == '1');
     if (rc == FDGPU_RETRY_WIDE) rc = index_build_impl(c, b, p, first_id, out, true);
+    if (rc == FDGPU_EHIP && c && c->ws[WS_PAIR_MASKS].p) {
+        (void)hipStreamSynchronize(c->stream);
+        (void)hipGetLastError();
+        c->ws[WS_PAIR_MASKS].release();
+        c->pair_masks_crowded = true;
+        rc = index_build_impl(c, b, p, first_id, out, e32 && e32[0] == '1');
+        if (rc == FDGPU_RETRY_WIDE) rc = index_build_impl(c, b, p, first_id, out, true);
+    }
     return rc;
+}
+
+extern "C" int fdgpu_debug_last_build_mask_bytes(fdgpu_ctx *c, uint64_t *bytes) { FD_LOCK(c);
+    if (!c || !bytes) return FDGPU_EINVAL;
+    *bytes = c->last_build_mask_bytes;
+    return FDGPU_OK;
 }
 
 static int debug_upload_stream(fdgpu_ctx *c, const uint32_t *keys, const void *ids, size_t id_bytes, uint64_t n) {
diff --git a/folddisco_amd/csrc/fd_device.h b/folddisco_amd/csrc/fd_device.h
--- a/folddisco_amd/csrc/fd_device.h
+++ b/folddisco_amd/csrc/fd_device.h
@@ -12,6 +12,7 @@
     const uint32_t *res_off;
     const uint32_t *wi_struct;
     const uint32_t *wi_i0;
+    const uint64_t *wi_col;
     uint32_t n_struct;
     uint32_t n_work;
 };
diff --git a/folddisco_amd/csrc/fd_pair_mask_cols.h b/folddisco_amd/csrc/fd_pair_mask_cols.h
--- /dev/null
+++ b/folddisco_amd/csrc/fd_pair_mask_cols.h
@@ -0,0 +1,29 @@
+#pragma once
+#include <stdint.h>
+
+#define FD_MASK_BLOCK 64ull
+#define FD_MASK_SLACK_WORDS 8ull
+
+static inline uint64_t fd_mask_cols_padded(uint64_t partners) { return (partners + (FD_MASK_BLOCK - 1)) / FD_MASK_BLOCK * FD_MASK_BLOCK; }
+
+static inline uint64_t fd_mask_tiles(uint64_t R) { return (R + (FD_MASK_BLOCK - 1)) / FD_MASK_BLOCK; }
+
+static inline uint64_t fd_mask_cols_of_structure(uint64_t R) {
+    uint64_t n = 0;
+    for (uint64_t t = 0; t < R; t += FD_MASK_BLOCK) n += fd_mask_cols_padded(R - t);
+    return n;
+}
+
+static inline uint64_t fd_mask_col_offsets(const uint64_t *res_off, uint64_t n_struct, uint64_t *wi_col) {
+    uint64_t col = 0, w = 0;
+    for (uint64_t s = 0; s < n_struct; ++s) {
+        const uint64_t R = res_off[s + 1] - res_off[s];
+        for (uint64_t t = 0; t < R; t += FD_MASK_BLOCK) {
+            if (wi_col) wi_col[w] = col;
+            ++w;
+            col += fd_mask_cols_padded(R - t);
+        }
+    }
+    if (wi_col) wi_col[w] = col;
+    return col;
+}
diff --git a/folddisco_amd/csrc/fdgpu_api.hip b/folddisco_amd/csrc/fdgpu_api.hip
--- a/folddisco_amd/csrc/fdgpu_api.hip
+++ b/folddisco_amd/csrc/fdgpu_api.hip
@@ -180,6 +180,7 @@
     if (!c) return FDGPU_EINVAL;
     HIPCHK(c, hipStreamSynchronize(c->stream));
     for (auto &b : c->ws) b.release();
+    c->pair_masks_crowded = false;
     c->pool_drop();
     (void)hipGetLastError();
     return FDGPU_OK;
@@ -285,6 +286,7 @@
 
 int fd_build_work_items(fdgpu_ctx *c, fdgpu_batch *b, bool with_hash_ok) {
     std::vector<uint32_t> ws, wi;
+    std::vector<uint64_t> wc;
     std::vector<uint32_t> ro(b->n_struct + 1);
     for (uint64_t s = 0; s <= b->n_struct; ++s) ro[s] = (uint32_t)b->h_res_off[s];
     for (uint64_t s = 0; s < b->n_struct; ++s) {
@@ -294,7 +296,11 @@
     }
     if (ws.size() > 0xfffffff0ull) FAIL(c, FDGPU_ERANGE, "too many tiles in one batch");
     b->n_work = (uint32_t)ws.size();
+    wc.resize(ws.size() + 1);
+    b->n_mask_cols = fd_mask_col_offsets(b->h_res_off.data(), b->n_struct, wc.data());
     HIPCHK(c, hipMalloc((void **)&b->res_off, ro.size() * 4));
+    HIPCHK(c, hipMalloc((void **)&b->wi_col, wc.size() * 8));
+    HIPCHK(c, hipMemcpyAsync(b->wi_col, wc.data(), wc.size() * 8, hipMemcpyHostToDevice, c->stream));
     HIPCHK(c, hipMalloc((void **)&b->wi_struct, std::max<size_t>(ws.size(), 1) * 4));
     HIPCHK(c, hipMalloc((void **)&b->wi_i0, std::max<size_t>(wi.size(), 1) * 4));
     HIPCHK(c, hipMemcpyAsync(b->res_off, ro.data(), ro.size() * 4, hipMemcpyHostToDevice, c->stream));
@@ -357,6 +363,7 @@
     if (!b) return;
     if (b->owns) { (void)hipFree(b->n_xyz); (void)hipFree(b->ca_xyz); (void)hipFree(b->cb_xyz); (void)hipFree(b->aa); (void)hipFree(b->cb_valid); }
     (void)hipFree(b->hash_ok); (void)hipFree(b->res_off); (void)hipFree(b->wi_struct); (void)hipFree(b->wi_i0);
+    (void)hipFree(b->wi_col);
     delete b;
 }
 extern "C" uint64_t fdgpu_batch_num_structures(const fdgpu_batch *b) { return b ? b->n_struct : 0; }
diff --git a/folddisco_amd/csrc/fdgpu_internal.h b/folddisco_amd/csrc/fdgpu_internal.h
--- a/folddisco_amd/csrc/fdgpu_internal.h
+++ b/folddisco_amd/csrc/fdgpu_internal.h
@@ -13,6 +13,7 @@
 
 #include "fd_host_pool.h"
 #include "fd_match_tables.h"
+#include "fd_pair_mask_cols.h"
 
 struct fd_devbuf {
     void *p = nullptr;
@@ -39,6 +40,7 @@
     WS_CQ_KIDX, WS_CQ_NSEG, WS_CQ_WSTART, WS_CQ_SEGSUM, WS_CQ_TOPN,
     WS_QT_RANGES, WS_QT_COMPACT, WS_QT_COUNT, WS_QT_AUX, WS_RS_PLAN, WS_RS_REC, WS_RS_RECRES, WS_QT_PARTIAL, WS_QT_SURV, WS_QT_ROWBITS, WS_QT_STREAM, WS_QT_STAB, WS_QT_PIECEP, WS_QT_WIN, WS_QT_HEAD, WS_RS_SPLIT, WS_MP_QSET,
     WS_CA_PERM, WS_OK_PERM, WS_AA_PERM, WS_SRC_PERM , WS_SEG_TAB,
+    WS_PAIR_MASKS ,
     WS_RS_TAB, WS_RS_SEG, WS_RS_OUT, WS_RS_RES, WS_RS_KX, WS_RS_KY, WS_RS_KOFF, WS_RS_SOL, WS_RS_CNT, WS_RS_GQ, WS_MP_ACT, WS_MP_Q,
     WS_SG_TAB , WS_SG_TAB_B, WS_SG_PAIRS, WS_SG_CURSOR,
     WS_SG_NB_PART , WS_SG_NB_OUT ,
@@ -66,6 +68,8 @@
     uint32_t last_count_path = 0;
     uint32_t last_query_map_path = 0;
     fd_devbuf ws[WS_COUNT];
+    uint64_t last_build_mask_bytes = 0;
+    bool pair_masks_crowded = false;
     bool timing = false;
     mutable std::recursive_mutex mu;
     int host_libm_matches = -1;
@@ -156,11 +160,13 @@
     float *n_xyz = nullptr, *ca_xyz = nullptr, *cb_xyz = nullptr;
     uint8_t *aa = nullptr, *cb_valid = nullptr, *hash_ok = nullptr;
     uint32_t *res_off = nullptr, *wi_struct = nullptr, *wi_i0 = nullptr;
+    uint64_t *wi_col = nullptr;
+    uint64_t n_mask_cols = 0;
     std::vector<uint64_t> h_res_off;
     fd_batch_view view() const {
         fd_batch_view v;
         v.n_xyz = n_xyz; v.ca_xyz = ca_xyz; v.cb_xyz = cb_xyz; v.aa = aa; v.hash_ok = hash_ok; v.res_off = res_off;
-        v.wi_struct = wi_struct; v.wi_i0 = wi_i0; v.n_struct = (uint32_t)n_struct; v.n_work = n_work;
+        v.wi_struct = wi_struct; v.wi_i0 = wi_i0; v.wi_col = wi_col; v.n_struct = (uint32_t)n_struct; v.n_work = n_work;
         return v;
     }
 };
@@ -255,9 +261,9 @@
                           uint64_t *tot, hipStream_t st, fdgpu_ctx *timing_ctx = nullptr);
 void fd_launch_frames_perm(const fd_batch_view &B, float *ca_perm, uint8_t *ok_perm, uint8_t *aa_perm, uint32_t *src_perm, unsigned long long *wide_flag, hipStream_t st);
 void fd_launch_pair_count_msd(const fd_batch_view &B, const fd_hash_consts &C, const float *n_xyz, const float *cb_xyz, const uint32_t *src_perm, void *frames,
-                              uint32_t *counts, hipStream_t st);
+                              uint32_t *counts, uint64_t *masks, hipStream_t st);
 void fd_launch_pair_emit_msd(const fd_batch_view &B, const void *frames, const fd_hash_consts &C, const uint64_t *seg_off, uint32_t *keys,
-                             uint16_t *ids, hipStream_t st);
+                             uint16_t *ids, const uint64_t *masks, hipStream_t st);
 uint32_t fd_rs_seg_num_tiles(uint64_t n, uint32_t n_seg);
 uint64_t fd_rs_seg_tot_words(uint64_t n, uint32_t n_seg);
 size_t fd_rs_seg_tab_bytes(uint64_t n, uint32_t n_seg);
diff --git a/folddisco_amd/csrc/k_hash.hip b/folddisco_amd/csrc/k_hash.hip
--- a/folddisco_amd/csrc/k_hash.hip
+++ b/folddisco_amd/csrc/k_hash.hip
@@ -98,6 +98,32 @@
 #define FD_NOT_HASHABLE 0x100u
 
 __device__ __forceinline__ bool fd_lane_of(uint64_t m) { return __builtin_amdgcn_inverse_ballot_w64(m); }
+__device__ __forceinline__ uint32_t fd_writelane(uint32_t old, uint32_t val, uint32_t lane) {
+    asm("v_writelane_b32 %0, %1, %2" : "+v"(old) : "s"(val), "{m0}"(lane));
+    return old;
+}
+
+struct fd_block_runs {
+    uint64_t starts;
+    uint32_t nkf;
+    bool last_block;
+};
+__device__ __forceinline__ fd_block_runs fd_runs_of_block(uint32_t kind, uint32_t jb, uint32_t r1) {
+    fd_block_runs R;
+    const uint64_t okm = __ballot(kind != FD_NOT_HASHABLE);
+    R.starts = __ballot(kind != (uint32_t)__shfl_up((int)kind, 1, FD_WAVE)) | 1ull;
+    R.last_block = jb + FD_WAVE >= r1;
+    const uint32_t nk = okm ? 64u - (uint32_t)__builtin_clzll(okm) : 0u;
+    R.nkf = (R.last_block && nk == 0) ? 1u : nk;
+    return R;
+}
+__device__ __forceinline__ void fd_run_at(const fd_block_runs &R, uint32_t kind, uint32_t k, uint32_t &t, uint32_t &ke, bool &run_last) {
+    t = (uint32_t)__builtin_amdgcn_readlane((int)kind, (int)k);
+    const uint64_t rest = (R.starts >> k) >> 1;
+    ke = rest ? k + 1u + (uint32_t)__builtin_ctzll(rest) : (uint32_t)FD_WAVE;
+    ke = ke < R.nkf ? ke : R.nkf;
+    run_last = R.last_block && ke >= R.nkf;
+}
 
 template <bool TYPES, class Step, class RunEnd>
 __device__ __forceinline__ void fd_filter_block(const fd_batch_view &B, float d2_max, const fd_v3 &cai, uint64_t vim, uint32_t i0, uint32_t jb, uint32_t r1,
@@ -113,20 +139,14 @@
     fd_wave_lds_fence();
     s_cj[lane] = cj.x; s_cj[FD_WAVE + lane] = cj.y; s_cj[2 * FD_WAVE + lane] = cj.z;
     fd_wave_lds_fence();
-    const uint64_t okm = __ballot(kind != FD_NOT_HASHABLE);
-    const uint64_t starts = __ballot(kind != (uint32_t)__shfl_up((int)kind, 1, FD_WAVE)) | 1ull;
-    const bool last_block = jb + FD_WAVE >= r1;
-    const uint32_t nk = okm ? 64u - (uint32_t)__builtin_clzll(okm) : 0u;
-    const uint32_t nkf = (last_block && nk == 0) ? 1u : nk;
+    const fd_block_runs R = fd_runs_of_block(kind, jb, r1);
     const bool first = jb == i0;
     const fd_f2 ax = {cai.x, cai.x}, ay = {cai.y, cai.y}, az = {cai.z, cai.z};
     uint32_t k = 0;
-    while (k < nkf) {
-        const uint32_t t = (uint32_t)__builtin_amdgcn_readlane((int)kind, (int)k);
-        const uint64_t rest = (starts >> k) >> 1;
-        uint32_t ke = rest ? k + 1u + (uint32_t)__builtin_ctzll(rest) : (uint32_t)FD_WAVE;
-        ke = ke < nkf ? ke : nkf;
-        const bool run_last = last_block && ke >= nkf;
+    while (k < R.nkf) {
+        uint32_t t, ke;
+        bool run_last;
+        fd_run_at(R, kind, k, t, ke, run_last);
         const bool dead = t == FD_NOT_HASHABLE;
         if (dead && !run_last) { k = ke; continue; }
         const uint64_t vr = dead ? 0ull : vim;
@@ -145,6 +165,30 @@
         } while (k < ke);
         k = ke;
         run_end(t);
+    }
+}
+
+typedef uint64_t fd_u64x2 __attribute__((ext_vector_type(2), aligned(8)));
+template <class Step>
+__device__ __forceinline__ void fd_replay_block(const fd_batch_view &B, const uint64_t *__restrict__ cols, uint32_t jb, uint32_t r1, Step &&step) {
+    const uint32_t jl = jb + threadIdx.x;
+    uint32_t kind = FD_NOT_HASHABLE;
+    if (jl < r1 && B.hash_ok[jl]) kind = (uint32_t)B.aa[jl];
+    const fd_block_runs R = fd_runs_of_block(kind, jb, r1);
+    uint32_t k = 0;
+    while (k < R.nkf) {
+        uint32_t t, ke;
+        bool run_last;
+        fd_run_at(R, kind, k, t, ke, run_last);
+        if (t == FD_NOT_HASHABLE && !run_last) { k = ke; continue; }
+        do {
+            const fd_u64x2 m = *reinterpret_cast<const fd_u64x2 *>(cols + k);
+            const uint64_t m1 = (k + 1u < ke) ? m.y : 0ull;
+            const uint32_t k0 = k;
+            k += 2;
+            step(k0, t, m.x, m1, run_last && k >= ke);
+        } while (k < ke);
+        k = ke;
     }
 }
 
@@ -222,8 +266,10 @@
     }
 }
 
+template <bool STORE>
 __global__ __launch_bounds__(FD_WAVE) void k_pair_count_msd(fd_batch_view B, fd_hash_consts C, const float *__restrict__ n_xyz, const float *__restrict__ cb_xyz,
-                                                            const uint32_t *__restrict__ src_perm, fd_frame *__restrict__ frames, uint32_t *__restrict__ counts) {
+                                                            const uint32_t *__restrict__ src_perm, fd_frame *__restrict__ frames, uint32_t *__restrict__ counts,
+                                                            uint64_t *__restrict__ masks) {
     __shared__ uint32_t s_cnt[FD_WAVE];
     __shared__ float s_cj[3 * FD_WAVE + 1];
     uint32_t w = fd_xcd_remap(blockIdx.x, B.n_work);
@@ -249,14 +295,27 @@
     const uint64_t vim = __ballot(vi);
     uint32_t c_lo = 0, c_hi = 0, run = 0;
     const uint32_t hi_i = aai >> 4;
-    for (uint32_t jb = i0; jb < r1; jb += FD_WAVE)
+    uint2 *mrow = STORE ? reinterpret_cast<uint2 *>(masks + B.wi_col[w]) + lane : nullptr;
+    for (uint32_t jb = i0; jb < r1; jb += FD_WAVE) {
+        uint32_t c_x = 0, c_y = 0;
         fd_filter_block<true>(B, C.d2_max, cai, vim, i0, jb, r1, s_cj,
-                              [&](uint32_t, uint32_t, uint64_t m0, uint64_t m1, bool) { run += (fd_lane_of(m0) ? 1u : 0u) + (fd_lane_of(m1) ? 1u : 0u); },
+                              [&](uint32_t k, uint32_t, uint64_t m0, uint64_t m1, bool) {
+                                  run += (fd_lane_of(m0) ? 1u : 0u) + (fd_lane_of(m1) ? 1u : 0u);
+                                  if (STORE) {
+                                      const uint32_t k1 = k + 1u < FD_WAVE ? k + 1u : FD_WAVE - 1u;
+                                      c_x = fd_writelane(c_x, (uint32_t)m1, k1);
+                                      c_y = fd_writelane(c_y, (uint32_t)(m1 >> 32), k1);
+                                      c_x = fd_writelane(c_x, (uint32_t)m0, k);
+                                      c_y = fd_writelane(c_y, (uint32_t)(m0 >> 32), k);
+                                  }
+                              },
                               [&](uint32_t t) {
                                   if (t >= 16u) c_hi += run; else c_lo += run;
                                   if (run) atomicAdd(&s_cnt[(t * 2u + hi_i) & (FD_WAVE - 1u)], run);
                                   run = 0;
                               });
+        if (STORE) { *mrow = make_uint2(c_x, c_y); mrow += FD_WAVE; }
+    }
     if (c_lo) atomicAdd(&s_cnt[aai * 2u], c_lo);
     if (c_hi) atomicAdd(&s_cnt[aai * 2u + 1u], c_hi);
     __syncthreads();
@@ -369,12 +428,14 @@
     }
 }
 
-template <int TAB, bool IDS16, bool MSD, bool DT = false>
+template <int TAB, bool IDS16, bool MSD, bool DT = false, bool MASKS = false>
 __global__ __launch_bounds__(FD_WAVE, FD_EMIT_WAVES) void k_pair_emit2(fd_batch_view B, const fd_frame *__restrict__ frames, fd_hash_consts C,
                                                         const uint64_t *__restrict__ seg_off, uint32_t *__restrict__ cursor,
-                                                        uint32_t *__restrict__ keys, void *__restrict__ ids, uint32_t first_id) {
+                                                        uint32_t *__restrict__ keys, void *__restrict__ ids, uint32_t first_id,
+                                                        const uint64_t *__restrict__ masks) {
+    static_assert(!MASKS || MSD, "the mask table belongs to the MSD build");
     __shared__ uint32_t q[3 * FD_WAVE];
-    __shared__ float s_cj[3 * FD_WAVE + 1];
+    __shared__ float s_cj[MASKS ? 1 : 3 * FD_WAVE + 1];
     __shared__ uint32_t tab[DT ? 64 + FD_DIST_NTHR + 1 : 64];
     uint32_t w = fd_xcd_remap(blockIdx.x, B.n_work);
     if (w >= B.n_work) return;
@@ -393,9 +454,6 @@
     const uint32_t i0 = B.wi_i0[w];
     const uint32_t lane = threadIdx.x;
     const uint32_t i = i0 + lane;
-    const bool vi = i < r1 && B.hash_ok[i];
-    fd_v3 cai = {0.f, 0.f, 0.f};
-    if (vi) cai = fd_load3(B.ca_xyz, i);
     __shared__ float4 s_fi[4 * FD_WAVE];
     if (TAB == 2 && i < r1) {
         const float4 *fp = reinterpret_cast<const float4 *>(frames + i);
@@ -406,31 +464,36 @@
     __shared__ uint64_t s_boff[MSD ? FD_MSD_BUCKETS : 1];
     if (MSD && lane < FD_MSD_BUCKETS) s_boff[lane] = seg_off[(uint64_t)lane * B.n_work + w];
     __syncthreads();
-    const uint64_t vim = __ballot(vi);
     const uint32_t lane16 = lane << 16;
     uint32_t qn = 0;
-    for (uint32_t jb = i0; jb < r1; jb += FD_WAVE) {
-        const uint32_t jrel = jb - r0;
-        fd_filter_block<MSD>(B, C.d2_max, cai, vim, i0, jb, r1, s_cj,
-            [&](uint32_t k, uint32_t t, uint64_t m0, uint64_t m1, bool last) {
-                const uint32_t tag = (MSD ? t << 22 : 0u) | (jrel + k);
-                if (m0) {
-                    if (fd_lane_of(m0)) q[__builtin_amdgcn_mbcnt_hi((uint32_t)(m0 >> 32), __builtin_amdgcn_mbcnt_lo((uint32_t)m0, qn))] = lane16 | tag;
-                    qn += (uint32_t)__popcll(m0);
-                }
-                if (m1) {
-                    if (fd_lane_of(m1)) q[__builtin_amdgcn_mbcnt_hi((uint32_t)(m1 >> 32), __builtin_amdgcn_mbcnt_lo((uint32_t)m1, qn))] = lane16 | (tag + 1u);
-                    qn += (uint32_t)__popcll(m1);
-                }
-                while (qn >= FD_WAVE || (last && qn)) {
-                    fd_wave_lds_fence();
-                    uint32_t n = qn < FD_WAVE ? qn : FD_WAVE;
-                    qn -= n;
-                    drain2<TAB, IDS16, MSD, DT>(B, frames, C, tab, q + qn, n, i0, r0, s, first_id + s, seg_off, cursor, keys, ids, s_fi, s_bc, s_boff);
-                    fd_wave_lds_fence();
-                }
-            },
-            [](uint32_t) {});
+    uint32_t jrel = i0 - r0;
+    auto step = [&](uint32_t k, uint32_t t, uint64_t m0, uint64_t m1, bool last) {
+        const uint32_t tag = (MSD ? t << 22 : 0u) | (jrel + k);
+        if (m0) {
+            if (fd_lane_of(m0)) q[__builtin_amdgcn_mbcnt_hi((uint32_t)(m0 >> 32), __builtin_amdgcn_mbcnt_lo((uint32_t)m0, qn))] = lane16 | tag;
+            qn += (uint32_t)__popcll(m0);
+        }
+        if (m1) {
+            if (fd_lane_of(m1)) q[__builtin_amdgcn_mbcnt_hi((uint32_t)(m1 >> 32), __builtin_amdgcn_mbcnt_lo((uint32_t)m1, qn))] = lane16 | (tag + 1u);
+            qn += (uint32_t)__popcll(m1);
+        }
+        while (qn >= FD_WAVE || (last && qn)) {
+            fd_wave_lds_fence();
+            uint32_t n = qn < FD_WAVE ? qn : FD_WAVE;
+            qn -= n;
+            drain2<TAB, IDS16, MSD, DT>(B, frames, C, tab, q + qn, n, i0, r0, s, first_id + s, seg_off, cursor, keys, ids, s_fi, s_bc, s_boff);
+            fd_wave_lds_fence();
+        }
+    };
+    if constexpr (MASKS) {
+        const uint64_t *cols = masks + B.wi_col[w];
+        for (uint32_t jb = i0; jb < r1; jb += FD_WAVE, jrel += FD_WAVE, cols += FD_WAVE) fd_replay_block(B, cols, jb, r1, step);
+    } else {
+        const bool vi = i < r1 && B.hash_ok[i];
+        fd_v3 cai = {0.f, 0.f, 0.f};
+        if (vi) cai = fd_load3(B.ca_xyz, i);
+        const uint64_t vim = __ballot(vi);
+        for (uint32_t jb = i0; jb < r1; jb += FD_WAVE, jrel += FD_WAVE) fd_filter_block<MSD>(B, C.d2_max, cai, vim, i0, jb, r1, s_cj, step, [](uint32_t) {});
     }
 }
 
@@ -559,31 +622,35 @@
     if (!B.n_work) return;
     dim3 g(grid_for(B.n_work)), b(FD_WAVE);
     const fd_frame *F = (const fd_frame *)frames;
-    if (C.use_tab >= 2 && ids16) hipLaunchKernelGGL((k_pair_emit2<2, true, false>), g, b, 0, st, B, F, C, seg_off, cursor, keys, ids, first_id);
-    else if (C.use_tab >= 2) hipLaunchKernelGGL((k_pair_emit2<2, false, false>), g, b, 0, st, B, F, C, seg_off, cursor, keys, ids, first_id);
-    else if (C.use_tab && ids16) hipLaunchKernelGGL((k_pair_emit2<1, true, false>), g, b, 0, st, B, F, C, seg_off, cursor, keys, ids, first_id);
-    else if (C.use_tab) hipLaunchKernelGGL((k_pair_emit2<1, false, false>), g, b, 0, st, B, F, C, seg_off, cursor, keys, ids, first_id);
-    else if (ids16) hipLaunchKernelGGL((k_pair_emit2<0, true, false>), g, b, 0, st, B, F, C, seg_off, cursor, keys, ids, first_id);
-    else hipLaunchKernelGGL((k_pair_emit2<0, false, false>), g, b, 0, st, B, F, C, seg_off, cursor, keys, ids, first_id);
+    if (C.use_tab >= 2 && ids16) hipLaunchKernelGGL((k_pair_emit2<2, true, false>), g, b, 0, st, B, F, C, seg_off, cursor, keys, ids, first_id, (const uint64_t *)nullptr);
+    else if (C.use_tab >= 2) hipLaunchKernelGGL((k_pair_emit2<2, false, false>), g, b, 0, st, B, F, C, seg_off, cursor, keys, ids, first_id, (const uint64_t *)nullptr);
+    else if (C.use_tab && ids16) hipLaunchKernelGGL((k_pair_emit2<1, true, false>), g, b, 0, st, B, F, C, seg_off, cursor, keys, ids, first_id, (const uint64_t *)nullptr);
+    else if (C.use_tab) hipLaunchKernelGGL((k_pair_emit2<1, false, false>), g, b, 0, st, B, F, C, seg_off, cursor, keys, ids, first_id, (const uint64_t *)nullptr);
+    else if (ids16) hipLaunchKernelGGL((k_pair_emit2<0, true, false>), g, b, 0, st, B, F, C, seg_off, cursor, keys, ids, first_id, (const uint64_t *)nullptr);
+    else hipLaunchKernelGGL((k_pair_emit2<0, false, false>), g, b, 0, st, B, F, C, seg_off, cursor, keys, ids, first_id, (const uint64_t *)nullptr);
 }
 void fd_launch_frames_perm(const fd_batch_view &B, float *ca_perm, uint8_t *ok_perm, uint8_t *aa_perm, uint32_t *src_perm, unsigned long long *wide_flag, hipStream_t st) {
     if (!B.n_struct) return;
     hipLaunchKernelGGL(k_frames_perm, dim3(B.n_struct), dim3(256), 0, st, B, ca_perm, ok_perm, aa_perm, src_perm, wide_flag);
 }
 void fd_launch_pair_count_msd(const fd_batch_view &B, const fd_hash_consts &C, const float *n_xyz, const float *cb_xyz, const uint32_t *src_perm, void *frames,
-                              uint32_t *counts, hipStream_t st) {
-    if (!B.n_work) return;
-    hipLaunchKernelGGL(k_pair_count_msd, dim3(grid_for(B.n_work)), dim3(FD_WAVE), 0, st, B, C, n_xyz, cb_xyz, src_perm, (fd_frame *)frames, counts);
+                              uint32_t *counts, uint64_t *masks, hipStream_t st) {
+    if (!B.n_work) return;
+    dim3 g(grid_for(B.n_work)), b(FD_WAVE);
+    if (masks) hipLaunchKernelGGL(k_pair_count_msd<true>, g, b, 0, st, B, C, n_xyz, cb_xyz, src_perm, (fd_frame *)frames, counts, masks);
+    else hipLaunchKernelGGL(k_pair_count_msd<false>, g, b, 0, st, B, C, n_xyz, cb_xyz, src_perm, (fd_frame *)frames, counts, (uint64_t *)nullptr);
 }
 void fd_launch_pair_emit_msd(const fd_batch_view &B, const void *frames, const fd_hash_consts &C, const uint64_t *seg_off, uint32_t *keys,
-                             uint16_t *ids, hipStream_t st) {
+                             uint16_t *ids, const uint64_t *masks, hipStream_t st) {
     if (!B.n_work) return;
     dim3 g(grid_for(B.n_work)), b(FD_WAVE);
     const fd_frame *F = (const fd_frame *)frames;
-    if (C.use_tab == 3) hipLaunchKernelGGL((k_pair_emit2<2, true, true, true>), g, b, 0, st, B, F, C, seg_off, (uint32_t *)nullptr, keys, (void *)ids, 0u);
-    else if (C.use_tab == 2) hipLaunchKernelGGL((k_pair_emit2<2, true, true>), g, b, 0, st, B, F, C, seg_off, (uint32_t *)nullptr, keys, (void *)ids, 0u);
-    else if (C.use_tab) hipLaunchKernelGGL((k_pair_emit2<1, true, true>), g, b, 0, st, B, F, C, seg_off, (uint32_t *)nullptr, keys, (void *)ids, 0u);
-    else hipLaunchKernelGGL((k_pair_emit2<0, true, true>), g, b, 0, st, B, F, C, seg_off, (uint32_t *)nullptr, keys, (void *)ids, 0u);
+    const uint64_t *no = nullptr;
+    if (C.use_tab == 3 && masks) hipLaunchKernelGGL((k_pair_emit2<2, true, true, true, true>), g, b, 0, st, B, F, C, seg_off, (uint32_t *)nullptr, keys, (void *)ids, 0u, masks);
+    else if (C.use_tab == 3) hipLaunchKernelGGL((k_pair_emit2<2, true, true, true>), g, b, 0, st, B, F, C, seg_off, (uint32_t *)nullptr, keys, (void *)ids, 0u, no);
+    else if (C.use_tab == 2) hipLaunchKernelGGL((k_pair_emit2<2, true, true>), g, b, 0, st, B, F, C, seg_off, (uint32_t *)nullptr, keys, (void *)ids, 0u, no);
+    else if (C.use_tab) hipLaunchKernelGGL((k_pair_emit2<1, true, true>), g, b, 0, st, B, F, C, seg_off, (uint32_t *)nullptr, keys, (void *)ids, 0u, no);
+    else hipLaunchKernelGGL((k_pair_emit2<0, true, true>), g, b, 0, st, B, F, C, seg_off, (uint32_t *)nullptr, keys, (void *)ids, 0u, no);
 }
 void fd_launch_row_count(const fd_batch_view &B, const fd_hash_consts &C, uint32_t *row_cnt, float cutoff, hipStream_t st) {
     if (!B.n_work) return;
diff --git a/include/fdgpu_debug.h b/include/fdgpu_debug.h
--- a/include/fdgpu_debug.h
+++ b/include/fdgpu_debug.h
@@ -37,6 +37,8 @@
 #define FDGPU_PATH_OVERFLOW 64u
 int fdgpu_debug_last_count_path(fdgpu_ctx *ctx, uint32_t *flags);
 
+int fdgpu_debug_last_build_mask_bytes(fdgpu_ctx *ctx, uint64_t *bytes);
+
 #define FDGPU_RPATH_DEVICE_TRIED 1u
 #define FDGPU_RPATH_DEVICE_DONE 2u
 #define FDGPU_RPATH_LIMIT 4u
```

Measured after the change: 1.749 million structures/s, median of 6. +2.1%, better.
